# emonosuke/emoASR

Hardware: AMD Instinct MI355X
Metric: train frames/sec + decode RTF, Conformer-CTC 23M, 80-mel, 1/2/4/8 GPU (higher is better)
Workload: dtype bf16; 1 GPU; CTC(Conformer) 23M `L2`, bf16, SpecAugment on-GPU, synthetic LibriSpeech-shaped batches (2000 utts, lognormal lengths, ASRBatchSampler packing 30000 frames/50 utts per GPU), one step = accum_grad 5 micro-batches (the reference's accum_grad: 5, asr/train_asr.py:106-128, stacked through the engine in one pass) fwd+bwd, then all-reduce+clip+Adam; dropout 0.1; accum_grad=5, stacked_micro_batches=True, parallelism=dp1

## Files before the change

emoasr_amd/csrc/convfused.hip:

```cpp
#include <algorithm>
#include "common.h"
#include "../../include/emoasr_hip.h"

namespace {

constexpr int CF_TT = 32;
constexpr int CF_MAXK = 31;
constexpr int CF_CB = 256;
constexpr int CF_ROWS_P = 64;

typedef __attribute__((ext_vector_type(2))) float f2;
__device__ __forceinline__ f2 unpack2(unsigned u) { return f2{__uint_as_float(u << 16), __uint_as_float(u & 0xffff0000u)}; }
__device__ __forceinline__ unsigned pack2(f2 v) {
  const bf16 lo = (bf16)v[0], hi = (bf16)v[1];
  return (unsigned)__builtin_bit_cast(unsigned short, lo) | ((unsigned)__builtin_bit_cast(unsigned short, hi) << 16);
}
__device__ __forceinline__ unsigned lds_pair(const bf16* base, int row, int pair) {
  return *reinterpret_cast<const unsigned*>(base + row * CF_CB + 2 * pair);
}

__device__ __forceinline__ int ring_row(int u) { return (u & (CF_ROWS_P - 1)) * CF_CB; }

template <bool GLU>
__global__ __launch_bounds__(CF_CB) void cf_dwconv_kernel(int Tn, int C, int K, const bf16* __restrict__ x,
// ... 354 lines not shown
}

extern "C" int emoasr_conv_bwd_fused(int dtype, int B, int Tn, int C, int K, const void* ds, const void* cv,
                                     const float* mean, const float* var, const float* gamma, const float* beta, float eps,
                                     const float* tot, const void* g, const float* w, void* dg, float* dw, float* dbias,
                                     float* scratch, void* stream) {
  EMO_CHECK(dtype == EMO_BF16, "conv_bwd_fused: bf16 only");
  EMO_CHECK(K <= CF_MAXK && (K & 1) && C % 8 == 0, "conv_bwd_fused: K=%d (odd, <= %d), C=%d (multiple of 8)", K, CF_MAXK, C);
  EMO_CHECK((long)Tn * 2 * C * 2 < (1L << 32), "conv_bwd_fused: utterance larger than 4 GiB");
  EMO_CHECK(scratch != nullptr && tot != nullptr, "conv_bwd_fused: scratch and tot are required");
  if (B * Tn == 0) return 0;
  hipStream_t s = (hipStream_t)stream;
  if (bwd_lds_attr()) return 1;
  const int S = strip_tiles(1, &B, &Tn, cdiv(C, CF_CB));
  dim3 grid(cdiv(cdiv(Tn, CF_TT), S), cdiv(C, CF_CB), B);
  cf_conv_bwd_kernel<<<grid, CF_CB, CF_BWD_LDS, s>>>(Tn, C, K, (const bf16*)ds, (const bf16*)cv, mean, var, gamma, beta, eps, tot,
                                                   (const bf16*)g, w, (bf16*)dg, scratch, S, 1, RowSegs{});
  EMO_LAUNCH_CHECK();
  return emo_dwconv_bwd_w_reduce(cdiv(Tn, CF_TT) * B, C, K, scratch, dw, dbias, s);
}

int emo_bn_stats_finalize_seg(const RowSegs& sg, int C, float* part, float* mean, float* var, float* running_mean,
                              float* running_var, float momentum, long long* nbt, hipStream_t s);
int emo_bn_swish_fwd_seg(const RowSegs& sg, int C, const void* y, const float* mean, const float* var, const float* gamma,
                         const float* beta, float eps, void* z, hipStream_t s);
int emo_bn_swish_bwd_sums_seg(const RowSegs& sg, int C, const void* dz, const void* y, const float* mean, const float* var,
                              const float* gamma, const float* beta, float eps, float* dgamma, float* dbeta, float* scratch,
                              float** tot_out, hipStream_t s);

namespace {
bool row_segs(const emoasr_segments_t* seg, int C, RowSegs* out, int* tmax) {
  if (!seg || seg->n < 1 || seg->n > EMOASR_MAX_SEGMENTS) return false;
  RowSegs sg{};
  sg.n = seg->n;
  *tmax = 0;
  for (int i = 0; i < seg->n; ++i) {
    if (seg->B[i] <= 0 || seg->T[i] <= 0) return false;
    sg.b0[i + 1] = sg.b0[i] + seg->B[i];
    sg.T[i] = seg->T[i];
    sg.row[i + 1] = sg.row[i] + (long)seg->B[i] * seg->T[i];
    sg.part[i + 1] = sg.part[i] + emoasr_dwconv_stats_floats(seg->B[i], seg->T[i], C);
    sg.sums[i + 1] = sg.sums[i] + (emoasr_bn_swish_bwd_scratch_floats(seg->B[i] * seg->T[i], C) / (2 * C) - 1);
    *tmax = std::max(*tmax, seg->T[i]);
  }
  *out = sg;
  return true;
}
}

extern "C" int emoasr_conv_module_fwd_seg(int dtype, const emoasr_segments_t* seg, int C, int K, const void* g, const float* w,
                                          const float* bias, void* c, float* part, float* bmean, float* bvar, float* running_mean,
                                          float* running_var, float momentum, long long* num_batches_tracked, const float* gamma,
                                          const float* beta, float eps, void* z, int training, void* stream) {
  EMO_CHECK(dtype == EMO_BF16, "conv_module_fwd_seg: bf16 only");
  EMO_CHECK(K <= CF_MAXK && (K & 1) && C % 8 == 0, "conv_module_fwd_seg: K=%d (odd, <= %d), C=%d (multiple of 8)", K, CF_MAXK, C);
  RowSegs sg;
  int tmax = 0;
  EMO_CHECK(row_segs(seg, C, &sg, &tmax), "conv_module_fwd_seg: bad segment description");
  EMO_CHECK((long)tmax * 2 * C * 2 < (1L << 32) && sg.row[sg.n] * 2 * C * 2 < (1L << 46), "conv_module_fwd_seg: batch too large");
  EMO_CHECK(!training || (part && bmean && bvar), "conv_module_fwd_seg: training needs the BatchNorm buffers");
  hipStream_t s = (hipStream_t)stream;
  EmoTimerScope timer_(EMO_TIMER_CONV_MODULE, s, 0.0, 5.0 * (double)sg.row[sg.n] * C * 2.0);
  const int S = strip_tiles(seg->n, seg->B, seg->T, cdiv(C, CF_CB));
  dim3 grid(cdiv(cdiv(tmax, CF_TT), S), cdiv(C, CF_CB), sg.b0[sg.n]);
  cf_dwconv_kernel<true><<<grid, CF_CB, 0, s>>>(tmax, C, K, (const bf16*)g, w, bias, (bf16*)c, 0, training ? part : nullptr, S, sg);
  EMO_LAUNCH_CHECK();
  if (training) {
    if (emo_bn_stats_finalize_seg(sg, C, part, bmean, bvar, running_mean, running_var, momentum, num_batches_tracked, s)) return 1;
    return emo_bn_swish_fwd_seg(sg, C, c, bmean, bvar, gamma, beta, eps, z, s);
  }
  RowSegs one{};
  one.n = 1; one.b0[1] = sg.b0[sg.n]; one.row[1] = sg.row[sg.n];
  return emo_bn_swish_fwd_seg(one, C, c, running_mean, running_var, gamma, beta, eps, z, s);
}

extern "C" long emoasr_conv_module_bwd_seg_scratch_floats(const emoasr_segments_t* seg, int C, int K, int which) {
  RowSegs sg;
  int tmax = 0;
  if (!row_segs(seg, C, &sg, &tmax)) return 0;
  if (which == 0) return (sg.sums[sg.n] + 2 * sg.n) * 2 * C;
  return emoasr_dwconv_bwd_w_scratch_floats(sg.b0[sg.n], tmax, C, K);
}

extern "C" int emoasr_conv_module_bwd_seg(int dtype, const emoasr_segments_t* seg, int C, int K, const void* dz, const void* c,
                                          const float* bmean, const float* bvar, const float* gamma, const float* beta, float eps,
                                          float* dgamma, float* dbeta, const void* g, const float* w, void* dg, float* dw,
                                          float* dbias, float* bn_scratch, float* dw_scratch, void* stream) {
  EMO_CHECK(dtype == EMO_BF16, "conv_module_bwd_seg: bf16 only");
  EMO_CHECK(K <= CF_MAXK && (K & 1) && C % 8 == 0, "conv_module_bwd_seg: K=%d (odd, <= %d), C=%d (multiple of 8)", K, CF_MAXK, C);
  EMO_CHECK(bn_scratch && dw_scratch, "conv_module_bwd_seg: scratch required");
  RowSegs sg;
  int tmax = 0;
  EMO_CHECK(row_segs(seg, C, &sg, &tmax), "conv_module_bwd_seg: bad segment description");
  hipStream_t s = (hipStream_t)stream;
  EmoTimerScope timer_(EMO_TIMER_CONV_MODULE, s, 0.0, 8.0 * (double)sg.row[sg.n] * C * 2.0);
  float* tot = nullptr;
  if (emo_bn_swish_bwd_sums_seg(sg, C, dz, c, bmean, bvar, gamma, beta, eps, dgamma, dbeta, bn_scratch, &tot, s)) return 1;
  if (bwd_lds_attr()) return 1;
  const int S = strip_tiles(seg->n, seg->B, seg->T, cdiv(C, CF_CB));
  dim3 grid(cdiv(cdiv(tmax, CF_TT), S), cdiv(C, CF_CB), sg.b0[sg.n]);
  cf_conv_bwd_kernel<<<grid, CF_CB, CF_BWD_LDS, s>>>(tmax, C, K, (const bf16*)dz, (const bf16*)c, bmean, bvar, gamma, beta, eps, tot,
                                                   (const bf16*)g, w, (bf16*)dg, dw_scratch, S, 0, sg);
  EMO_LAUNCH_CHECK();
  return emo_dwconv_bwd_w_reduce((int)live_strips(seg->n, seg->B, seg->T, S), C, K, dw_scratch, dw, dbias, s);
}
```

emoasr_amd/csrc/convmodule.hip:

```cpp
#include <algorithm>
#include "common.h"
#include "../../include/emoasr_hip.h"

namespace {

constexpr int DW_TT = 32;
constexpr int DW_MAXK = 31;
constexpr int DW_WCHUNKS = 1;

template <typename T>
__global__ __launch_bounds__(256) void dwconv_kernel(int Tn, int C, int K, const T* __restrict__ x,
                                                     const float* __restrict__ w,
                                                     const float* __restrict__ bias, T* __restrict__ y,
                                                     int flip, float* __restrict__ part, const RowSegs sg) {
  const int c = blockIdx.y * 256 + threadIdx.x;
  if (c >= C) return;
  int b = blockIdx.z;
  if (sg.n > 1) {
    const int si = rowsegs_of_utt(sg, b);
    Tn = sg.T[si];
    x += sg.row[si] * C; y += sg.row[si] * C;
    if (part) part += sg.part[si];
    b -= sg.b0[si];
    if ((int)blockIdx.x * DW_TT >= Tn) return;
// ... 122 lines not shown
    tickets[blockIdx.x] = 0u;
    if (num_batches_tracked && blockIdx.x == 0) *num_batches_tracked += ns;
  }
}

template <typename T>
__global__ __launch_bounds__(256) void dwconv_bwd_w_kernel(int Tn, int C, int K, const T* __restrict__ dy,
                                                           const T* __restrict__ x, float* __restrict__ part, const RowSegs sg) {
  const int c = blockIdx.y * 256 + threadIdx.x;
  if (c >= C) return;
  int b = blockIdx.z;
  const int pad = (K - 1) / 2;
  if (sg.n > 1) {
    const int si = rowsegs_of_utt(sg, b);
    Tn = sg.T[si];
    x += sg.row[si] * C; dy += sg.row[si] * C;
    b -= sg.b0[si];
  }
  float acc[DW_MAXK];
#pragma unroll
  for (int j = 0; j < DW_MAXK; ++j) acc[j] = 0.f;
  float sb = 0.f;
  const __amdgpu_buffer_rsrc_t rsx = make_rsrc(x + (long)b * Tn * C), rsd = make_rsrc(dy + (long)b * Tn * C);
  for (int cc = 0; cc < DW_WCHUNKS; ++cc) {
    const int t0 = (blockIdx.x * DW_WCHUNKS + cc) * DW_TT;
    if (t0 >= Tn) break;
    float win[DW_TT + DW_MAXK - 1];
#pragma unroll
    for (int i = 0; i < DW_TT + DW_MAXK - 1; ++i) {
      const int t = t0 + i - pad;
      const bool ok = i < DW_TT + K - 1 && t >= 0 && t < Tn;
      win[i] = buf_load_f32<T>(rsx, ok ? (unsigned)(((long)t * C + c) * sizeof(T)) : EMO_OOB);
    }
    float dv[DW_TT];
#pragma unroll
    for (int i = 0; i < DW_TT; ++i)
      dv[i] = buf_load_f32<T>(rsd, t0 + i < Tn ? (unsigned)(((long)(t0 + i) * C + c) * sizeof(T)) : EMO_OOB);
#pragma unroll
    for (int i = 0; i < DW_TT; ++i) {
      const float d = dv[i];
      sb += d;
#pragma unroll
      for (int j = 0; j < DW_MAXK; ++j) acc[j] = emo_mac(d, win[i + j], acc[j]);
    }
  }
  const long blk = ((long)blockIdx.z * gridDim.x + blockIdx.x);
  float* p = part + blk * (K + 1) * C + c;
#pragma unroll
  for (int j = 0; j < DW_MAXK; ++j)
    if (j < K) p[(long)j * C] = acc[j];
  p[(long)K * C] = sb;
}

__global__ __launch_bounds__(256) void dwconv_bwd_w_reduce_kernel(int nblk, int C, int K,
                                                                  const float* __restrict__ part,
                                                                  float* __restrict__ dw,
                                                                  float* __restrict__ dbias) {
  __shared__ float red[4][64];
  const int lane = threadIdx.x & 63, wave = threadIdx.x >> 6;
  const int i = blockIdx.x * 64 + lane;
  const int n = (K + 1) * C;
  const int per = (nblk + gridDim.y - 1) / gridDim.y;
  const int b0 = blockIdx.y * per, b1 = min(nblk, b0 + per);
  float s = 0.f;
  if (i < n) {
#pragma unroll 8
    for (int b = b0 + wave; b < b1; b += 4) s += part[(long)b * n + i];
  }
  red[wave][lane] = s;
  __syncthreads();
  if (wave == 0 && i < n) {
    s = red[0][lane] + red[1][lane] + red[2][lane] + red[3][lane];
    const int j = i / C, c = i % C;
    if (gridDim.y == 1) {
      if (j < K) dw[c * K + j] += s;
      else if (dbias) dbias[c] += s;
    } else {
      if (j < K) atomicAdd(&dw[c * K + j], s);
      else if (dbias) atomicAdd(&dbias[c], s);
    }
  }
}

constexpr int BN_ROWS = 16;
constexpr int BN_STAT_ROWS = 64;
template <typename T>
__global__ __launch_bounds__(256) void bn_sum_kernel(int M, int C, const T* __restrict__ y,
                                                     float* __restrict__ sum) {
  const int c = blockIdx.x * 256 + threadIdx.x;
  if (c >= C) return;
  const int r0 = blockIdx.y * BN_STAT_ROWS, r1 = min(M, r0 + BN_STAT_ROWS);
  float s = 0.f;
  for (int r = r0; r < r1; ++r) s += to_f32(y[(long)r * C + c]);
  atomicAdd(&sum[c], s);
}
template <typename T>
__global__ __launch_bounds__(256) void bn_var_kernel(int M, int C, const T* __restrict__ y,
                                                     const float* __restrict__ sum,
                                                     float* __restrict__ sq) {
  const int c = blockIdx.x * 256 + threadIdx.x;
  if (c >= C) return;
  const float mu = sum[c] / M;
  const int r0 = blockIdx.y * BN_STAT_ROWS, r1 = min(M, r0 + BN_STAT_ROWS);
  float s = 0.f;
  for (int r = r0; r < r1; ++r) { const float d = to_f32(y[(long)r * C + c]) - mu; s += d * d; }
  atomicAdd(&sq[c], s);
}
__global__ void bn_finalize_kernel(int M, int C, float* mean, float* var, float* running_mean,
                                   float* running_var, float momentum) {
  const int c = blockIdx.x * 256 + threadIdx.x;
  if (c >= C) return;
  const float mu = mean[c] / M, vb = var[c] / M;
  mean[c] = mu; var[c] = vb;
  if (running_mean) running_mean[c] = (1.f - momentum) * running_mean[c] + momentum * mu;
  if (running_var) {
    const float vu = M > 1 ? var[c] * M / (M - 1) : vb;
    running_var[c] = (1.f - momentum) * running_var[c] + momentum * vu;
  }
}

template <typename T>
__global__ __launch_bounds__(256) void bn_swish_fwd_kernel(long n, int C, const T* __restrict__ y,
                                                           const float* __restrict__ mean,
                                                           const float* __restrict__ var,
                                                           const float* __restrict__ gamma,
                                                           const float* __restrict__ beta, float eps,
                                                           T* __restrict__ z, const RowSegs sg) {
  for (long i = (long)blockIdx.x * 256 + threadIdx.x; i < n; i += (long)gridDim.x * 256) {
    const int c = i % C;
    const long so = sg.n > 1 ? (long)rowsegs_of_row(sg, i / C) * C : 0;
    const float xh = (to_f32(y[i]) - mean[so + c]) * rsqrtf(var[so + c] + eps);
    z[i] = from_f32<T>(swish_t<T>(gamma[c] * xh + beta[c]));
  }
}
template <typename T>
__global__ __launch_bounds__(256) void bn_swish_fwd8_kernel(long n8, int C, const T* __restrict__ y,
                                                            const float* __restrict__ mean,
                                                            const float* __restrict__ var,
                                                            const float* __restrict__ gamma,
                                                            const float* __restrict__ beta, float eps,
                                                            T* __restrict__ z, const RowSegs sg) {
  const int cg = C / 8;
  for (long i = (long)blockIdx.x * 256 + threadIdx.x; i < n8; i += (long)gridDim.x * 256) {
    const long row = i / cg;
    const int c = (int)(i - row * cg) * 8;
    const long so = sg.n > 1 ? (long)rowsegs_of_row(sg, row) * C : 0;
    float v[8];
    load8<T>(y + i * 8, v);
#pragma unroll
    for (int j = 0; j < 8; ++j) {
      const float xh = (v[j] - mean[so + c + j]) * rsqrtf(var[so + c + j] + eps);
      v[j] = swish_t<T>(gamma[c + j] * xh + beta[c + j]);
    }
    store8<T>(z + i * 8, v);
  }
}

constexpr int BN_SUM_ROWS = 64;
constexpr int BN_APPLY_ROWS = 16;

template <typename T>
__global__ __launch_bounds__(256) void bn_bwd_sums_kernel(int M, int C, const T* __restrict__ dz,
                                                          const T* __restrict__ y,
                                                          const float* __restrict__ mean,
                                                          const float* __restrict__ var,
                                                          const float* __restrict__ gamma,
// ... 83 lines not shown
      raw[C + c] = b;
    }
  }
  if (ns == 1 || (!dbeta && !dgamma)) return;
  __syncthreads();
  if (threadIdx.x == 0) {
    __threadfence();
    s_last = atomicAdd(&tickets[64 + blockIdx.x], 1u) == (unsigned)ns - 1;
  }
  __syncthreads();
  if (!s_last) return;
  __threadfence();
  if (grp == 0 && c < C) {
    float da = 0.f, db = 0.f;
    const float* r0 = tot_ + (long)ns * 2 * C;
    for (int k = 0; k < ns; ++k) {
      da += __hip_atomic_load(r0 + (long)k * 2 * C + c, __ATOMIC_RELAXED, __HIP_MEMORY_SCOPE_AGENT);
      db += __hip_atomic_load(r0 + (long)k * 2 * C + C + c, __ATOMIC_RELAXED, __HIP_MEMORY_SCOPE_AGENT);
    }
    if (dbeta) dbeta[c] += da;
    if (dgamma) dgamma[c] += db;
  }
  if (threadIdx.x == 0) tickets[64 + blockIdx.x] = 0u;
}
template <typename T>
__global__ __launch_bounds__(256) void bn_bwd_apply_kernel(int M, int C, const T* __restrict__ dz,
                                                           const T* __restrict__ y,
                                                           const float* __restrict__ mean,
                                                           const float* __restrict__ var,
                                                           const float* __restrict__ gamma,
                                                           const float* __restrict__ beta, float eps,
                                                           const float* __restrict__ tot,
                                                           T* __restrict__ dy, const RowSegs sg) {
  const int hl = threadIdx.x & 31, rl = threadIdx.x >> 5;
  const int c = blockIdx.x * 256 + hl * 8;
  if (c >= C) return;
  if (sg.n > 1) {
    const int si = blockIdx.z;
    M = (int)(sg.row[si + 1] - sg.row[si]);
    if ((int)blockIdx.y * BN_APPLY_ROWS >= M) return;
    dz += sg.row[si] * C; y += sg.row[si] * C; dy += sg.row[si] * C;
    mean += (long)si * C; var += (long)si * C; tot += (long)si * 2 * C;
  }
  float mu[8], is[8], g[8], bt[8], m1[8], m2[8];
#pragma unroll
  for (int j = 0; j < 8; ++j) {
    mu[j] = mean[c + j]; is[j] = rsqrtf(var[c + j] + eps); g[j] = gamma[c + j]; bt[j] = beta[c + j];
    m1[j] = tot[c + j]; m2[j] = tot[C + c + j];
  }
  const __amdgpu_buffer_rsrc_t rsy = make_rsrc(y), rsd = make_rsrc(dz);
  const int r0 = blockIdx.y * BN_APPLY_ROWS;
#pragma unroll
  for (int it = 0; it < BN_APPLY_ROWS / 8; ++it) {
    const int r = r0 + rl + 8 * it;
    const bool ok = r < M;
    float yv[8], dv[8], o[8];
    buf_load8<T>(rsy, (long)r * C + c, ok, yv);
    buf_load8<T>(rsd, (long)r * C + c, ok, dv);
#pragma unroll
    for (int j = 0; j < 8; ++j) {
      const float xh = (yv[j] - mu[j]) * is[j];
      const float dbn = dv[j] * dswish_t<T>(g[j] * xh + bt[j]);
      o[j] = g[j] * is[j] * (dbn - m1[j] - xh * m2[j]);
    }
    if (ok) store8<T>(dy + (long)r * C + c, o);
  }
}

inline int ew_grid(long n) { long b = (n + 255) / 256; return (int)(b > 8192 ? 8192 : (b < 1 ? 1 : b)); }

}

int emo_dwconv_lds(int B, int Tn, int C, int K, const void* x, const float* w, const float* bias, void* y, int flip,
                   float* part, hipStream_t s);
static bool use_lds(int dtype, int Tn, int C) {
  return g_opt.dwconv_lds && dtype == EMO_BF16 && C % 8 == 0 && (long)Tn * C * 2 < (1L << 32);
}
int emo_dwconv_bwd_w_reduce(int nblk, int C, int K, const float* part, float* dw, float* dbias, hipStream_t s) {
  dwconv_bwd_w_reduce_kernel<<<dim3(cdiv((K + 1) * C, 64), nblk >= 1024 ? 4 : 1), 256, 0, s>>>(nblk, C, K, part, dw, dbias);
  EMO_LAUNCH_CHECK();
  return 0;
}

extern "C" int emoasr_dwconv_fwd(int dtype, int B, int Tn, int C, int K, const void* x, const float* w,
                                 const float* bias, void* y, void* stream) {
  EMO_CHECK(K <= DW_MAXK && (K & 1), "dwconv: K=%d unsupported (odd, <= %d)", K, DW_MAXK);
  if (B * Tn == 0) return 0;
  if (use_lds(dtype, Tn, C)) return emo_dwconv_lds(B, Tn, C, K, x, w, bias, y, 0, nullptr, (hipStream_t)stream);
  dim3 grid(cdiv(Tn, DW_TT), cdiv(C, 256), B);
  EMO_DISPATCH(dtype, (dwconv_kernel<T><<<grid, 256, 0, (hipStream_t)stream>>>(Tn, C, K, (const T*)x, w,
                                                                              bias, (T*)y, 0, nullptr, RowSegs{})));
  EMO_LAUNCH_CHECK();
  return 0;
}

extern "C" long emoasr_dwconv_stats_floats(int B, int Tn, int C) { return (long)B * cdiv(Tn, DW_TT) * 2 * C; }

extern "C" int emoasr_dwconv_fwd_stats(int dtype, int B, int Tn, int C, int K, const void* x, const float* w,
                                       const float* bias, void* y, float* part, void* stream) {
  EMO_CHECK(K <= DW_MAXK && (K & 1), "dwconv: K=%d unsupported", K);
  EMO_CHECK(part != nullptr && B * Tn > 0, "dwconv_fwd_stats: needs a non-empty batch and the partials buffer");
  if (use_lds(dtype, Tn, C)) return emo_dwconv_lds(B, Tn, C, K, x, w, bias, y, 0, part, (hipStream_t)stream);
  dim3 grid(cdiv(Tn, DW_TT), cdiv(C, 256), B);
  EMO_DISPATCH(dtype, (dwconv_kernel<T><<<grid, 256, 0, (hipStream_t)stream>>>(Tn, C, K, (const T*)x, w,
                                                                              bias, (T*)y, 0, part, RowSegs{})));
  EMO_LAUNCH_CHECK();
  return 0;
}

extern "C" int emoasr_bn_stats_finalize(int B, int Tn, int C, const float* part, float* mean, float* var,
                                        float* running_mean, float* running_var, float momentum,
                                        long long* num_batches_tracked, void* stream) {
  EMO_CHECK(B * Tn > 0, "bn_stats_finalize: empty batch");
  EMO_CHECK(cdiv(C, BNF_CH) <= 64, "bn_stats_finalize: C=%d too wide for the ticket table", C);
  EMO_BN_TICKETS(stream);
  bn_stats_finalize_kernel<<<cdiv(C, BNF_CH), 1024, 0, (hipStream_t)stream>>>(B, Tn, C, const_cast<float*>(part), mean, var, running_mean,
                                                                          running_var, momentum, num_batches_tracked, RowSegs{}, tickets_);
  EMO_LAUNCH_CHECK();
  return 0;
}
extern "C" int emoasr_dwconv_bwd_x(int dtype, int B, int Tn, int C, int K, const void* dy, const float* w,
                                   void* dx, void* stream) {
  EMO_CHECK(K <= DW_MAXK && (K & 1), "dwconv: K=%d unsupported", K);
  if (B * Tn == 0) return 0;
  if (use_lds(dtype, Tn, C)) return emo_dwconv_lds(B, Tn, C, K, dy, w, nullptr, dx, 1, nullptr, (hipStream_t)stream);
  dim3 grid(cdiv(Tn, DW_TT), cdiv(C, 256), B);
  EMO_DISPATCH(dtype, (dwconv_kernel<T><<<grid, 256, 0, (hipStream_t)stream>>>(Tn, C, K, (const T*)dy, w,
                                                                              nullptr, (T*)dx, 1, nullptr, RowSegs{})));
  EMO_LAUNCH_CHECK();
  return 0;
}
extern "C" long emoasr_dwconv_bwd_w_scratch_floats(int B, int Tn, int C, int K) {
  return (long)B * cdiv(Tn, DW_TT * DW_WCHUNKS) * (K + 1) * C;
}

extern "C" int emoasr_dwconv_bwd_w(int dtype, int B, int Tn, int C, int K, const void* dy, const void* x,
                                   float* dw, float* dbias, int accumulate, float* scratch, void* stream) {
  EMO_CHECK(K <= DW_MAXK && (K & 1), "dwconv: K=%d unsupported", K);
  hipStream_t s = (hipStream_t)stream;
  if (!accumulate) {
    hipMemsetAsync(dw, 0, sizeof(float) * C * K, s);
    if (dbias) hipMemsetAsync(dbias, 0, sizeof(float) * C, s);
  }
  if (B * Tn == 0) return 0;
  EMO_CHECK(scratch != nullptr, "dwconv_bwd_w: scratch of emoasr_dwconv_bwd_w_scratch_floats() floats required");
  dim3 grid(cdiv(Tn, DW_TT * DW_WCHUNKS), cdiv(C, 256), B);
  EMO_DISPATCH(dtype, (dwconv_bwd_w_kernel<T><<<grid, 256, 0, s>>>(Tn, C, K, (const T*)dy, (const T*)x, scratch, RowSegs{})));
  const int nblk = grid.x * B;
  dwconv_bwd_w_reduce_kernel<<<cdiv((K + 1) * C, 64), 256, 0, s>>>(nblk, C, K, scratch, dw, dbias);
  EMO_LAUNCH_CHECK();
  return 0;
}

extern "C" int emoasr_bn_stats(int dtype, int M, int C, const void* y, float* mean, float* var,
                               float* running_mean, float* running_var, float momentum, void* stream) {
  EMO_CHECK(M > 0, "bn_stats: empty batch");
  hipStream_t s = (hipStream_t)stream;
  hipMemsetAsync(mean, 0, sizeof(float) * C, s);
  hipMemsetAsync(var, 0, sizeof(float) * C, s);
  dim3 grid(cdiv(C, 256), cdiv(M, BN_STAT_ROWS));
  EMO_DISPATCH(dtype, (bn_sum_kernel<T><<<grid, 256, 0, s>>>(M, C, (const T*)y, mean)));
  EMO_DISPATCH(dtype, (bn_var_kernel<T><<<grid, 256, 0, s>>>(M, C, (const T*)y, mean, var)));
  bn_finalize_kernel<<<cdiv(C, 256), 256, 0, s>>>(M, C, mean, var, running_mean, running_var, momentum);
  EMO_LAUNCH_CHECK();
  return 0;
}
// ... 152 lines not shown
```

emoasr_amd/csrc/gemm.hip:

```cpp
#include <algorithm>
#include <type_traits>
#include <vector>
#include "mma.h"
#include "../../include/emoasr_hip.h"
#include "gemm_big_tn.h"

namespace {

struct ConvGeom {
  int T1, F1, T2, F2, C;
};
__device__ __forceinline__ long conv_row_base(const ConvGeom& g, int m) {
  const int per_b = g.T2 * g.F2;
  const int b = m / per_b, r = m - b * per_b;
  const int t2 = r / g.F2, f2 = r - t2 * g.F2;
  return (((long)b * g.T1 + 2 * t2) * g.F1 + 2 * f2) * g.C;
}
__device__ __forceinline__ int conv_k_off(const ConvGeom& g, int k) {
  const int p = k / g.C, c = k - p * g.C;
  const int kh = p / 3, kw = p - kh * 3;
  return (kh * g.F1 + kw) * g.C + c;
}

struct DgradGeom {
// ... 606 lines not shown
      }
    } else {
#pragma unroll
    for (int kk = 0; kk < BK; kk += M_::KSTEP) {
      typename M_::Frag af[TM], bfr[TN];
#pragma unroll
      for (int i = 0; i < TM; ++i) af[i] = M_::template load_km<TR>(As[buf], LDA, kk, w1 + i * 32, lane);
#pragma unroll
      for (int j = 0; j < TN; ++j) bfr[j] = M_::template load_km<TR>(Bs[buf], LDB, kk, w2 + j * 32, lane);
#pragma unroll
      for (int i = 0; i < TM; ++i)
#pragma unroll
        for (int j = 0; j < TN; ++j) acc[i][j] = M_::mma(af[i], bfr[j], acc[i][j]);
    }
    }
    store_tile(nxt, buf ^ 1);
    __syncthreads();
  };
  for (int kt = kt_begin; kt < kt_end; kt += 3) {
    step(kt, s1, s2);
    if (kt + 1 < kt_end) step(kt + 1, s2, s0);
    if (kt + 2 < kt_end) step(kt + 2, s0, s1);
  }

#pragma unroll
  for (int i = 0; i < TM; ++i)
#pragma unroll
    for (int j = 0; j < TN; ++j) {
      const int col = n2_0 + w2 + j * 32 + c_col(lane);
      if (col >= g.N2) continue;
#pragma unroll
      for (int r = 0; r < 16; ++r) {
        const int row = n1_0 + w1 + i * 32 + c_row(r, lane);
        if (row >= g.N1) continue;
        atomicAdd(&g.C[(long)row * g.ldc + col], g.alpha * acc[i][j][r]);
      }
    }
  if (do_colsum && n1_0 + tid < g.N1) atomicAdd(&g.colsum[n1_0 + tid], g.colsum_scale * csum);
}

template <typename T, int BN1, int BN2, int BMODE, bool TR, int KB, bool SP = false>
__global__ __launch_bounds__(256) void gemm_tn_kernel(const TnArgs g) {
  const int gx = gridDim.x, gy = gridDim.y;
  const int lin = xcd_remap((blockIdx.z * gy + blockIdx.y) * gx + blockIdx.x, gx * gy * gridDim.z);
  tn_block<T, BN1, BN2, BMODE, TR, KB, SP>(g, lin % gx, (lin / gx) % gy, lin / (gx * gy), gx);
}

constexpr int TN_PLACE_MAX = 24;
struct TnPlace {
  unsigned short start[8][TN_PLACE_MAX + 1];
  unsigned char prob[8][TN_PLACE_MAX], split[8][TN_PLACE_MAX];
  unsigned char cnt[8];
};
struct TnGroup {
  int n;
  int xcd;
  int start[EMOASR_TN_GROUP_MAX + 1];
  TnArgs p[EMOASR_TN_GROUP_MAX];
  TnPlace place;
};
template <typename T, bool TR, int KB, int BT, bool SP = false>
__global__ __launch_bounds__(256) void gemm_tn_grouped_kernel(const TnGroup G) {
  if (G.xcd == 1) {
    const int x = blockIdx.x & 7, slot = blockIdx.x >> 3, cnt = G.place.cnt[x];
    if (slot >= G.place.start[x][cnt]) return;
    int e = 0;
    while (e + 1 < cnt && slot >= G.place.start[x][e + 1]) ++e;
    const TnArgs& g = G.p[G.place.prob[x][e]];
    const int local = slot - G.place.start[x][e];
    const int tx = (g.N2 + BT - 1) / BT;
    tn_block<T, BT, BT, 0, TR, KB, SP>(g, local % tx, local / tx, G.place.split[x][e], tx);
    return;
  }
  const int bid = G.xcd ? xcd_remap(blockIdx.x, gridDim.x) : (int)blockIdx.x;
  int p = 0;
  while (p + 1 < G.n && bid >= G.start[p + 1]) ++p;
  const TnArgs& g = G.p[p];
  const int local = bid - G.start[p];
  const int tx = (g.N2 + BT - 1) / BT, ty = (g.N1 + BT - 1) / BT;
  tn_block<T, BT, BT, 0, TR, KB, SP>(g, local % tx, (local / tx) % ty, local / (tx * ty), tx);
}

template <typename T, int AMODE, bool BKM, bool TR, bool SP = false>
int launch_nt_(const NtArgs& a_in, hipStream_t s, int nz = 1) {
  NtArgs a = a_in;
  a.xcd = g_opt.gemm_xcd;
  if constexpr (SP) {
    const long t12864 = (long)cdiv(a.M, 128) * cdiv(a.N, 64) * nz, t128 = (long)cdiv(a.M, 128) * cdiv(a.N, 128) * nz;
    (void)t12864;
    int tile = (t128 >= g_opt.split_min128 && a.N % 128 == 0) ? 1 : 3;
    if (g_opt.split_tile == 1 && a.N % 128 == 0) tile = 1;
    else if (g_opt.split_tile >= 2) tile = g_opt.split_tile;
    const int kb = (g_opt.split_kb == 2 && a.K >= 512) ? 2 : 1;
#define EMO_SP_LAUNCH(BM_, BN_)                                                            \
  do {                                                                                     \
    dim3 grid(cdiv(a.N, BN_), cdiv(a.M, BM_), nz);                                         \
    if (kb == 2) gemm_nt_kernel<T, BM_, BN_, AMODE, BKM, TR, 2, true><<<grid, 256, 0, s>>>(a); \
    else gemm_nt_kernel<T, BM_, BN_, AMODE, BKM, TR, 1, true><<<grid, 256, 0, s>>>(a);      \
  } while (0)
    if (tile == 1) EMO_SP_LAUNCH(128, 128);
    else if (tile == 2) EMO_SP_LAUNCH(128, 64);
    else EMO_SP_LAUNCH(64, 64);
#undef EMO_SP_LAUNCH
    EMO_LAUNCH_CHECK();
    return 0;
  }
  const long t12864 = (long)cdiv(a.M, 128) * cdiv(a.N, 64) * nz;
  const bool stacked64 = AMODE == 0 && a.M >= 16384 && !(a.N >= (g_opt.gemm_wide128 ? 512 : 768));
  const int tile = g_opt.gemm_tile ? g_opt.gemm_tile : (stacked64 ? 3 : (t12864 >= 384 ? 2 : 3));
  const int kb = sizeof(T) == 2 ? (g_opt.gemm_kb ? g_opt.gemm_kb : (a.K >= 512 ? 2 : 1)) : 1;
#define EMO_NT_LAUNCH(BM_, BN_)                                                           \
  do {                                                                                    \
    dim3 grid(cdiv(a.N, BN_), cdiv(a.M, BM_), nz);                                        \
    if constexpr (sizeof(T) == 2) {                                                       \
      if (kb == 2) gemm_nt_kernel<T, BM_, BN_, AMODE, BKM, TR, 2><<<grid, 256, 0, s>>>(a); \
      else gemm_nt_kernel<T, BM_, BN_, AMODE, BKM, TR, 1><<<grid, 256, 0, s>>>(a);         \
    } else {                                                                              \
      gemm_nt_kernel<T, BM_, BN_, AMODE, BKM, TR, 1><<<grid, 256, 0, s>>>(a);              \
    }                                                                                     \
  } while (0)
  if constexpr (sizeof(T) == 2 && AMODE == 0 && !BKM) {
    if (g_opt.gemm_wholek && a.M <= 2048 && a.K % 256 == 0 && nz == 1) {
      dim3 grid(cdiv(a.N, 64), cdiv(a.M, 64), 1);
      gemm_nt_kernel<T, 64, 64, AMODE, BKM, TR, 8><<<grid, 256, 0, s>>>(a);
      EMO_LAUNCH_CHECK();
      return 0;
    }
  }
  if (tile == 1) EMO_NT_LAUNCH(128, 128);
  else if (tile == 2) EMO_NT_LAUNCH(128, 64);
  else EMO_NT_LAUNCH(64, 64);
#undef EMO_NT_LAUNCH
  EMO_LAUNCH_CHECK();
  return 0;
}
template <typename T> constexpr bool is_f32 = sizeof(T) == 4;
template <typename T, int AMODE>
int launch_nt(const NtArgs& a, hipStream_t s) {
  if constexpr (is_f32<T>) { if (t_f32_split) return launch_nt_<T, AMODE, false, true, true>(a, s); }
  return launch_nt_<T, AMODE, false, true>(a, s);
}
template <typename T>
int launch_nn(const NtArgs& a, hipStream_t s, int nz = 1) {
  if constexpr (is_f32<T>) { if (t_f32_split) return launch_nt_<T, 0, true, true, true>(a, s, nz); }
  return g_opt.tr_read ? launch_nt_<T, 0, true, true>(a, s, nz) : launch_nt_<T, 0, true, false>(a, s, nz);
}

inline int tn_split_cap(long N1, long N2, long K) {
  const long out_bytes = N1 * N2 * 4;
  const double est_s = 2.0 * (double)N1 * (double)N2 * (double)K / 300e12;
  const long cap_work = (long)(0.25 * est_s * 1.3e12 / (double)out_bytes);
  return (int)std::max(std::max(1L, (8L << 20) / out_bytes), cap_work);
}

template <typename T, int BMODE, bool SP = false>
int launch_tn(TnArgs a, hipStream_t s) {
  if constexpr (is_f32<T> && !SP) { if (t_f32_split) return launch_tn<T, BMODE, true>(a, s); }
  const bool big = (long)cdiv(a.N1, 128) * cdiv(a.N2, 128) >= 32 && a.N1 >= 128 && a.N2 >= 128;
  const int kb = sizeof(T) == 2 ? (g_opt.gemm_kb ? g_opt.gemm_kb : (a.K >= 512 && !big ? 2 : 1)) : 1;
  const int BK = (SP ? 32 : TileCfg<T>::BK) * kb;
  const int nk = cdiv(a.K, BK);
  const int bn = big ? 128 : 64;
  const long tiles = (long)cdiv(a.N1, bn) * cdiv(a.N2, bn);
  const long slots_ = g_opt.tn_group_blocks > 0 ? g_opt.tn_group_blocks : ((big && kb == 2) || (big && SP) ? 512 : 768);
  int splits = (int)std::max(1L, slots_ / tiles);
  const int cap = tn_split_cap(a.N1, a.N2, a.K);
  const int floor_splits = (int)std::min((long)splits, (128 + tiles - 1) / tiles);
  splits = std::max(floor_splits, std::min(splits, cap));
  splits = std::max(1, std::min(splits, nk / 4 > 0 ? nk / 4 : 1));
  a.k_tiles_per_split = cdiv(nk, splits);
  splits = cdiv(nk, a.k_tiles_per_split);
  dim3 grid(cdiv(a.N2, bn), cdiv(a.N1, bn), splits);
#define EMO_TN_LAUNCH(BN_, TR_)                                                     \
  do {                                                                              \
    if constexpr (sizeof(T) == 2) {                                                 \
      if (kb == 2) gemm_tn_kernel<T, BN_, BN_, BMODE, TR_, 2><<<grid, 256, 0, s>>>(a); \
      else gemm_tn_kernel<T, BN_, BN_, BMODE, TR_, 1><<<grid, 256, 0, s>>>(a);         \
    } else {                                                                        \
      gemm_tn_kernel<T, BN_, BN_, BMODE, TR_, 1, SP><<<grid, 256, 0, s>>>(a);          \
    }                                                                               \
  } while (0)
  if constexpr (SP) {
    if (big) EMO_TN_LAUNCH(128, true);
    else EMO_TN_LAUNCH(64, true);
  } else {
  if (big) {
    if (g_opt.tr_read) EMO_TN_LAUNCH(128, true);
    else EMO_TN_LAUNCH(128, false);
  } else {
    if (g_opt.tr_read) EMO_TN_LAUNCH(64, true);
    else EMO_TN_LAUNCH(64, false);
  }
  }
#undef EMO_TN_LAUNCH
  EMO_LAUNCH_CHECK();
  return 0;
}

}

bool emo_gemm_nt_big_wants(int M, int N, int K, long lda, long ldb, long ldc, const emoasr_epilogue_t& ep);
int emo_gemm_nt_big_ep(int M, int N, int K, const void* A, long lda, const void* B, long ldb, void* C, long ldc,
                       const emoasr_epilogue_t& ep, hipStream_t s);
int emo_conv2_fwd_big(int B, int T1, int F1, int C, const void* y1, const void* w, void* y2, const float* bias,
                      int relu, hipStream_t s);


static int check_vec(long ld, int dtype, const char* what) {
  const int vec = dtype == EMO_BF16 ? 8 : 4;
  if (ld % vec != 0) { emo_set_error("gemm: %s=%ld must be a multiple of %d elements", what, ld, vec); return 1; }
  return 0;
}

extern "C" int emoasr_gemm_nt(int dtype, int M, int N, int K, const void* A, long lda, const void* B,
                              long ldb, void* C, long ldc, const emoasr_epilogue_t* ep, void* stream) {
  SplitScope split_scope(dtype);
  EMO_CHECK(M > 0 && N > 0 && K > 0, "gemm_nt: empty problem %d %d %d", M, N, K);
  if (check_vec(lda, dtype, "lda") || check_vec(ldb, dtype, "ldb") || check_vec(K, dtype, "K")) return 1;
  NtArgs a{};
  a.M = M; a.N = N; a.K = K; a.A = A; a.lda = lda; a.B = B; a.ldb = ldb; a.C = C; a.ldc = ldc;
  if (ep) a.ep = *ep; else { a.ep = emoasr_epilogue_t{}; a.ep.alpha = 1.f; }
  const double esz_ = dtype == EMO_BF16 ? 2.0 : 4.0;
  EmoTimerScope timer_(EMO_TIMER_GEMM_NT_NN, (hipStream_t)stream, 2.0 * M * N * K,
                       ((double)M * K + (double)N * K + (double)M * N * (1 + (a.ep.residual ? 1 : 0) + (a.ep.pre_out ? 1 : 0))) * esz_);
  if (dtype == EMO_BF16 && emo_gemm_nt_big_wants(M, N, K, lda, ldb, ldc, a.ep))
    return emo_gemm_nt_big_ep(M, N, K, A, lda, B, ldb, C, ldc, a.ep, (hipStream_t)stream);
  EMO_DISPATCH(dtype, return (launch_nt<T, 0>(a, (hipStream_t)stream)));
}

extern "C" int emoasr_gemm_nn(int dtype, int M, int N, int K, const void* A, long lda, const void* B,
                              long ldb, void* C, long ldc, const emoasr_epilogue_t* ep, void* stream) {
  SplitScope split_scope(dtype);
  EMO_CHECK(M > 0 && N > 0 && K > 0, "gemm_nn: empty problem %d %d %d", M, N, K);
  if (check_vec(lda, dtype, "lda") || check_vec(ldb, dtype, "ldb") || check_vec(K, dtype, "K") ||
      check_vec(N, dtype, "N")) return 1;
  NtArgs a{};
  a.M = M; a.N = N; a.K = K; a.A = A; a.lda = lda; a.B = B; a.ldb = ldb; a.C = C; a.ldc = ldc;
  if (ep) a.ep = *ep; else { a.ep = emoasr_epilogue_t{}; a.ep.alpha = 1.f; }
  const double esz_ = dtype == EMO_BF16 ? 2.0 : 4.0;
  EmoTimerScope timer_(EMO_TIMER_GEMM_NT_NN, (hipStream_t)stream, 2.0 * M * N * K,
                       ((double)M * K + (double)N * K + (double)M * N * (1 + (a.ep.residual ? 1 : 0) + (a.ep.dact_pre ? 1 : 0))) * esz_);
  EMO_DISPATCH(dtype, return (launch_nn<T>(a, (hipStream_t)stream)));
  return 0;
}

extern "C" int emoasr_gemm_nn_batched(int dtype, int M, int N, int K, const void* A, long lda, long sa_b,
                                      long sa_h, const void* B, long ldb, long sb_b, long sb_h, void* C,
                                      long ldc, long sc_b, long sc_h, int nb, int nh, float alpha,
                                      int accumulate, void* stream) {
  SplitScope split_scope(dtype);
  EMO_CHECK(M > 0 && N > 0 && K > 0 && nb > 0 && nh > 0, "gemm_nn_batched: empty problem");
  if (check_vec(lda, dtype, "lda") || check_vec(ldb, dtype, "ldb") ||
      check_vec(N, dtype, "N") || check_vec(sa_b, dtype, "sa_b") || check_vec(sa_h, dtype, "sa_h") ||
      check_vec(sb_b, dtype, "sb_b") || check_vec(sb_h, dtype, "sb_h")) return 1;
  NtArgs a{};
  a.M = M; a.N = N; a.K = K; a.A = A; a.lda = lda; a.B = B; a.ldb = ldb; a.C = C; a.ldc = ldc;
  a.ep = emoasr_epilogue_t{}; a.ep.alpha = alpha;
  if (accumulate) { a.ep.residual = C; a.ep.ldr = (int)ldc; a.ep.res_scale = 1.f; }
  a.nh = nh; a.sa_b = sa_b; a.sa_h = sa_h; a.sb_b = sb_b; a.sb_h = sb_h; a.sc_b = sc_b; a.sc_h = sc_h;
  EMO_DISPATCH(dtype, return (launch_nn<T>(a, (hipStream_t)stream, nb * nh)));
  return 0;
}

static bool tn_big_takes(int dtype, int N1, int N2, int K, long lda, long ldb);
static void tn_big_splits(int n, const BigTnProblem* q, int* splits);

extern "C" int emoasr_gemm_tn(int dtype, int N1, int N2, int K, const void* A, long lda, const void* B,
                              long ldb, float* C, long ldc, float alpha, int accumulate, float* colsum,
                              float colsum_scale, void* stream) {
  SplitScope split_scope(dtype);
  EMO_CHECK(N1 > 0 && N2 > 0 && K > 0, "gemm_tn: empty problem");
  if (check_vec(lda, dtype, "lda") || check_vec(ldb, dtype, "ldb") || check_vec(N2, dtype, "N2")) return 1;
  EMO_CHECK(N1 % (dtype == EMO_BF16 ? 8 : 4) == 0 || lda >= (N1 + 7) / 8 * 8, "gemm_tn: ragged N1 needs padded lda");
  if (!accumulate) {
    if (ldc == N2) hipMemsetAsync(C, 0, sizeof(float) * (size_t)N1 * N2, (hipStream_t)stream);
    else hipMemset2DAsync(C, sizeof(float) * ldc, 0, sizeof(float) * N2, N1, (hipStream_t)stream);
    if (colsum) hipMemsetAsync(colsum, 0, sizeof(float) * N1, (hipStream_t)stream);
  }
  TnArgs a{};
  a.N1 = N1; a.N2 = N2; a.K = K; a.A = A; a.lda = lda; a.B = B; a.ldb = ldb; a.C = C; a.ldc = ldc;
  a.alpha = alpha; a.colsum = colsum; a.colsum_scale = colsum_scale;
  EmoTimerScope timer_(EMO_TIMER_GEMM_TN, (hipStream_t)stream, 2.0 * N1 * N2 * K,
                       ((double)K * N1 + (double)K * N2) * (dtype == EMO_BF16 ? 2.0 : 4.0) + 4.0 * N1 * N2);
  if (tn_big_takes(dtype, N1, N2, K, lda, ldb)) {
    const BigTnProblem q{N1, N2, K, A, lda, B, ldb, C, ldc, alpha, 0, colsum, colsum_scale};
    int splits = 1;
    tn_big_splits(1, &q, &splits);
    return emo_tn_big_launch(1, &q, &splits, (hipStream_t)stream);
  }
  EMO_DISPATCH(dtype, return (launch_tn<T, 0>(a, (hipStream_t)stream)));
}

static int tn_group_plan(int dtype, int n, const emoasr_tn_problem_t* probs, TnGroup& G, int& bt, int& kb) {
  EMO_CHECK(n > 0 && n <= EMOASR_TN_GROUP_MAX, "gemm_tn_grouped: n=%d outside 1..%d", n, EMOASR_TN_GROUP_MAX);
  G.n = n;
  long tiles = 0;
  bt = 128;
  for (int i = 0; i < n; ++i)
    if (probs[i].N1 < 128 || probs[i].N2 < 128) bt = 64;
  if (g_opt.gemm_tile == 3) bt = 64;
  kb = dtype == EMO_BF16 ? (g_opt.tn_group_kb ? g_opt.tn_group_kb : g_opt.gemm_kb ? g_opt.gemm_kb : (bt == 128 ? 1 : 2)) : 1;
  const bool split = dtype == EMO_F32X3;
  const int BK = (dtype == EMO_BF16 || split ? 32 : 16) * kb;
  for (int i = 0; i < n; ++i) {
    const emoasr_tn_problem_t& q = probs[i];
    EMO_CHECK(q.N1 > 0 && q.N2 > 0 && q.K > 0, "gemm_tn_grouped: empty problem %d", i);
    if (check_vec(q.lda, dtype, "lda") || check_vec(q.ldb, dtype, "ldb") || check_vec(q.N2, dtype, "N2")) return 1;
    EMO_CHECK(q.N1 % (dtype == EMO_BF16 ? 8 : 4) == 0 || q.lda >= (q.N1 + 7) / 8 * 8,
              "gemm_tn_grouped: ragged N1 needs padded lda");
    tiles += (long)cdiv(q.N1, bt) * cdiv(q.N2, bt);
  }
  const long slots = g_opt.tn_group_blocks > 0 ? g_opt.tn_group_blocks : ((bt == 128 && kb == 2) || (bt == 128 && split) ? 512 : 768);
// ... 223 lines not shown
```

emoasr_amd/csrc/layer.hip:

```cpp
#include <math.h>
#include <algorithm>
#include <map>
#include <mutex>
#include <utility>
#include "common.h"
#include "../../include/emoasr_hip.h"

void emo_attn_bwd_fused_extras(float* zero, long zn, const float* cast_src, void* cast_dst, long cn);
void emo_attn_bwd_defer_join(int v);
void emo_attn_bwd_join(void* stream);
int emo_attn_bwd_prelaunch(int dtype, const emoasr_attn_t* a, void* ws, size_t ws_bytes, float* zero, long zn, void* stream);

int emo_bn_stats_finalize_seg(const RowSegs& sg, int C, float* part, float* mean, float* var, float* running_mean,
                              float* running_var, float momentum, long long* nbt, hipStream_t s);
int emo_bn_swish_fwd_seg_dt(int dtype, const RowSegs& sg, int C, const void* y, const float* mean, const float* var,
                            const float* gamma, const float* beta, float eps, void* z, hipStream_t s);
int emo_bn_swish_bwd_sums_seg_dt(int dtype, const RowSegs& sg, int C, const void* dz, const void* y, const float* mean, const float* var,
                                 const float* gamma, const float* beta, float eps, float* dgamma, float* dbeta, float* scratch,
                                 float** tot_out, hipStream_t s);
int emo_bn_bwd_apply_seg(int dtype, const RowSegs& sg, int C, const void* dz, const void* y, const float* mean, const float* var,
                         const float* gamma, const float* beta, float eps, const float* tot, void* dy, hipStream_t s);
int emo_dwconv_seg(int dtype, const RowSegs& sg, int tmax, int C, int K, const void* x, const float* w, const float* bias, void* y,
                   int flip, float* part, hipStream_t s);
int emo_dwconv_bwd_w_seg(int dtype, const RowSegs& sg, int tmax, int C, int K, const void* dy, const void* x, float* dw, float* dbias,
                         float* scratch, hipStream_t s);

namespace {

emoasr_epilogue_t plain_ep() {
  emoasr_epilogue_t e{};
  e.alpha = 1.f;
  e.res_scale = 1.f;
  return e;
}

bool conv_fused_ok(int dtype, int d) { return g_opt.conv_fused && dtype == EMO_BF16 && d % 8 == 0; }

struct WgSide {
  hipStream_t side = nullptr;
  hipEvent_t fork = nullptr, done[2] = {nullptr, nullptr};
  bool pending[2] = {false, false};
  unsigned n = 0;
};
std::mutex g_wg_mu;
std::map<std::pair<int, hipStream_t>, WgSide> g_wg;

WgSide* wg_side_of(hipStream_t s, bool create) {
  hipStreamCaptureStatus cap = hipStreamCaptureStatusNone;
  if (hipStreamIsCapturing(s, &cap) != hipSuccess || cap != hipStreamCaptureStatusNone) return nullptr;
  int dev = 0;
  if (hipGetDevice(&dev) != hipSuccess) return nullptr;
  std::lock_guard<std::mutex> lk(g_wg_mu);
  auto it = g_wg.find({dev, s});
  if (it != g_wg.end()) return &it->second;
  if (!create) return nullptr;
  WgSide w;
  if (hipStreamCreateWithFlags(&w.side, hipStreamNonBlocking) != hipSuccess) return nullptr;
  if (hipEventCreateWithFlags(&w.fork, hipEventDisableTiming) != hipSuccess ||
      hipEventCreateWithFlags(&w.done[0], hipEventDisableTiming) != hipSuccess ||
      hipEventCreateWithFlags(&w.done[1], hipEventDisableTiming) != hipSuccess)
    return nullptr;
  return &(g_wg[{dev, s}] = w);
}

int ffn_fwd(int dtype, int M, int d, int F, const emoasr_ffn_params_t& p, const void* x, float res_scale,
            float p_enc, uint64_t s_in, uint64_t s_out, const emoasr_ffn_stash_t& st, void* stream) {
  if (emoasr_layernorm_fwd(dtype, M, d, x, p.ln_g, p.ln_b, 1e-5f, st.h, st.mean, st.rstd, stream)) return 1;
  emoasr_epilogue_t e1 = plain_ep();
  e1.bias = p.b1; e1.act = EMOASR_ACT_SWISH | (g_opt.ffn_save_dact ? EMOASR_ACT_SAVE_DACT : 0); e1.pre_out = st.u; e1.drop_p = p_enc; e1.seed = s_in;
  if (emoasr_gemm_nt(dtype, M, F, d, st.h, d, p.w1, d, st.a, F, &e1, stream)) return 1;
  emoasr_epilogue_t e2 = plain_ep();
  e2.bias = p.b2; e2.residual = x; e2.ldr = d; e2.res_scale = res_scale; e2.drop_p = p_enc; e2.seed = s_out;
  return emoasr_gemm_nt(dtype, M, d, F, st.a, F, p.w2, F, st.y, d, &e2, stream);
}

struct SegView {
  int n = 0, Btot = 0;
  int B[EMOASR_MAX_SEGMENTS], T[EMOASR_MAX_SEGMENTS], b0[EMOASR_MAX_SEGMENTS];
  long row[EMOASR_MAX_SEGMENTS + 1], prow[EMOASR_MAX_SEGMENTS + 1], part[EMOASR_MAX_SEGMENTS + 1];
  long M() const { return row[n]; }
  long R() const { return prow[n]; }
};

bool seg_view(const emoasr_conformer_fwd_t* io, int d, SegView* v) {
  const emoasr_segments_t& s = io->seg;
  if (s.n < 0 || s.n > EMOASR_MAX_SEGMENTS) return false;
  v->n = s.n > 0 ? s.n : 1;
  v->row[0] = v->prow[0] = v->part[0] = 0;
  v->Btot = 0;
  for (int i = 0; i < v->n; ++i) {
    v->B[i] = s.n > 0 ? s.B[i] : io->B;
    v->T[i] = s.n > 0 ? s.T[i] : io->T;
    if (v->B[i] <= 0 || v->T[i] <= 0) return false;
    v->b0[i] = v->Btot;
    v->Btot += v->B[i];
    v->row[i + 1] = v->row[i] + (long)v->B[i] * v->T[i];
    v->prow[i + 1] = v->prow[i] + 2L * v->T[i] - 1;
    v->part[i + 1] = v->part[i] + emoasr_dwconv_stats_floats(v->B[i], v->T[i], d);
  }
  return true;
}

RowSegs row_segs_of(const SegView& sv, int C) {
  RowSegs sg{};
  sg.n = sv.n;
  for (int i = 0; i < sv.n; ++i) {
    sg.b0[i + 1] = sg.b0[i] + sv.B[i];
    sg.T[i] = sv.T[i];
// ... 13 lines not shown
  a.B = nb; a.H = H; a.DK = d / H; a.Tq = tmax; a.Tk = tmax;
  a.ldq = a.ldk = a.ldv = 3 * d; a.ldo = d; a.ldp = d;
  a.q = base; a.k = base + (size_t)d * esz; a.v = base + (size_t)2 * d * esz;
  a.pos = (const char*)pp + (size_t)sv.prow[s0] * d * esz;
  a.klens = klens ? klens + sv.b0[s0] : nullptr;
  a.causal = 0; a.scale = 1.f / sqrtf((float)(d / H));
  a.seed = seed + 0x9E3779B97F4A7C15ull * (uint64_t)s0;
  a.nseg = 0;
  if (s1 - s0 > 1) {
    a.nseg = s1 - s0;
    for (int k = s0; k <= s1; ++k) {
      a.seg_b0[k - s0] = k < s1 ? sv.b0[k] - sv.b0[s0] : nb;
      a.seg_row[k - s0] = sv.row[k] - sv.row[s0];
      a.seg_prow[k - s0] = sv.prow[k] - sv.prow[s0];
      if (k < s1) a.seg_T[k - s0] = sv.T[k];
    }
  }
}

}

extern "C" int emoasr_wgrad_side_join(int keep, void* stream) {
  hipStream_t s = (hipStream_t)stream;
  WgSide* w = wg_side_of(s, false);
  if (!w) return 0;
  for (int back = 2; back > (keep > 0 ? 1 : 0); --back) {
    if (w->n < (unsigned)back) continue;
    const int slot = (w->n - back) & 1;
    if (!w->pending[slot]) continue;
    if (hipStreamWaitEvent(s, w->done[slot], 0) != hipSuccess) { emo_set_error("wgrad_side_join: hipStreamWaitEvent failed"); return 1; }
    w->pending[slot] = false;
  }
  return 0;
}

extern "C" int emoasr_conformer_attn_masks(int dtype, int nl, const emoasr_segments_t* seg, int B, int T, int H, int d, const int* klens,
                                           float p_att, const uint64_t* seeds, unsigned* masks, long layer_stride_words, int nw,
                                           void* stream) {
  EMO_CHECK(seg && seeds && masks && nl >= 0 && H > 0 && d % H == 0, "conformer_attn_masks: bad arguments");
  if (p_att <= 0.f) return 0;
  emoasr_conformer_fwd_t io{};
  io.B = B; io.T = T; io.seg = *seg;
  SegView sv;
  EMO_CHECK(seg_view(&io, d, &sv), "conformer_attn_masks: bad batch / segment shapes");
  const size_t esz = dtype == EMO_BF16 ? 2 : 4;
  const int astep = g_opt.stack_launch ? sv.n : 1;
  for (int l = 0; l < nl; ++l)
    for (int si = 0; si < sv.n; si += astep) {
      emoasr_attn_t am{};
      attn_args_for(am, sv, si, si + astep, H, d, esz, nullptr, nullptr, klens, seeds[l]);
      am.drop_p = p_att;
      if (emoasr_attn_dropmask(dtype, &am, masks + (size_t)l * layer_stride_words + (size_t)sv.row[si] * H * nw, nw, stream)) return 1;
    }
  return 0;
}

extern "C" int emoasr_conformer_layer_fwd(int dtype, const emoasr_conformer_layer_t* L,
                                          const emoasr_conformer_fwd_t* io, void* stream) {
  EMO_CHECK(L && io && io->x && io->pos_t, "conformer_layer_fwd: missing arguments");
  const int d = L->d, H = L->H, F = L->F;
  EMO_CHECK(d > 0 && H > 0 && d % H == 0, "conformer_layer_fwd: bad dims d=%d H=%d", d, H);
  SegView sv;
  EMO_CHECK(seg_view(io, d, &sv), "conformer_layer_fwd: bad batch / segment shapes (B=%d T=%d segments=%d)", io->B, io->T, io->seg.n);
  const int M = (int)sv.M(), R = (int)sv.R();
  const size_t esz = dtype == EMO_BF16 ? 2 : 4;
  const float p_enc = io->p_enc;
  const bool att_bits = g_opt.attn_mask_bits && io->att_mask && io->training && io->p_att > 0.f && dtype == EMO_BF16;
  const int astep_m = g_opt.stack_launch ? sv.n : 1;
  for (int si = 0; si < sv.n && att_bits && !io->att_mask_ready; si += astep_m) {
    emoasr_attn_t am{};
    attn_args_for(am, sv, si, si + astep_m, H, d, esz, io->qkv, io->pp, io->klens, io->seed[2]);
    am.drop_p = io->p_att;
    if (emoasr_attn_dropmask(dtype, &am, io->att_mask + (size_t)sv.row[si] * H * io->att_mask_nw, io->att_mask_nw, stream)) return 1;
  }
  if (ffn_fwd(dtype, M, d, F, L->ffm, io->x, 0.5f, p_enc, io->seed[0], io->seed[1], io->ffm, stream)) return 1;
  const void* x1 = io->ffm.y;
  if (emoasr_layernorm_fwd(dtype, M, d, x1, L->att_ln_g, L->att_ln_b, 1e-5f, io->at_h, io->at_mean, io->at_rstd, stream))
    return 1;
  {
    emoasr_epilogue_t e = plain_ep();
    e.bias = L->bqkv;
    if (emoasr_gemm_nt(dtype, M, 3 * d, d, io->at_h, d, L->wqkv, d, io->qkv, 3 * d, &e, stream)) return 1;
    emoasr_epilogue_t ep = plain_ep();
    if (emoasr_gemm_nt(dtype, R, d, d, io->pos_t, d, L->wpos, d, io->pp, d, &ep, stream)) return 1;
    const int astep = g_opt.stack_launch ? sv.n : 1;
    for (int si = 0; si < sv.n; si += astep) {
      const size_t ro = (size_t)sv.row[si];
      emoasr_attn_t a{};
      attn_args_for(a, sv, si, si + astep, H, d, esz, io->qkv, io->pp, io->klens, io->seed[2]);
      a.bias_u = L->bias_u; a.bias_v = L->bias_v; a.drop_p = io->p_att;
      a.out = (char*)io->o + ro * d * esz; a.lse = io->lse + ro * H;
      if (att_bits) { a.keep_mask = io->att_mask + ro * H * io->att_mask_nw; a.keep_nw = io->att_mask_nw; }
      if (emoasr_attn_fwd(dtype, &a, stream)) return 1;
    }
    emoasr_epilogue_t eo = plain_ep();
    eo.bias = L->bout; eo.residual = x1; eo.ldr = d; eo.drop_p = p_enc; eo.seed = io->seed[3];
    if (emoasr_gemm_nt(dtype, M, d, d, io->o, d, L->wout, d, io->at_y, d, &eo, stream)) return 1;
  }
  const void* x2 = io->at_y;
  if (emoasr_layernorm_fwd(dtype, M, d, x2, L->cv_ln_g, L->cv_ln_b, 1e-5f, io->cv_h, io->cv_mean, io->cv_rstd, stream))
    return 1;
  {
    emoasr_epilogue_t e = plain_ep();
    e.bias = L->pw1_b;
    if (emoasr_gemm_nt(dtype, M, 2 * d, d, io->cv_h, d, L->pw1, d, io->g, 2 * d, &e, stream)) return 1;
    const bool fused = conv_fused_ok(dtype, d);
    if (!fused && emoasr_glu_fwd(dtype, M, d, io->g, io->gl, stream)) return 1;
    if (io->training) EMO_CHECK(io->bn_part && io->bmean && io->bvar, "conformer_layer_fwd: training needs the BatchNorm buffers");
    const bool conv_one_launch = fused && sv.n > 1 && g_opt.stack_launch;
    if (conv_one_launch &&
        emoasr_conv_module_fwd_seg(dtype, &io->seg, d, L->K, io->g, L->dw_w, L->dw_b, io->c, io->bn_part, io->bmean, io->bvar,
                                   L->bn_rm, L->bn_rv, 0.1f, L->bn_nbt, L->bn_g, L->bn_b, 1e-5f, io->z, io->training, stream))
      return 1;
    const bool bn_one_launch = !fused && io->training && sv.n > 1 && g_opt.stack_launch;
    if (bn_one_launch) {
      const RowSegs sg = row_segs_of(sv, d);
      int tmax = 0;
      for (int si = 0; si < sv.n; ++si) tmax = std::max(tmax, sv.T[si]);
      if (emo_dwconv_seg(dtype, sg, tmax, d, L->K, io->gl, L->dw_w, L->dw_b, io->c, 0, io->bn_part, (hipStream_t)stream)) return 1;
      if (emo_bn_stats_finalize_seg(sg, d, io->bn_part, io->bmean, io->bvar, L->bn_rm, L->bn_rv, 0.1f, L->bn_nbt, (hipStream_t)stream))
        return 1;
      if (emo_bn_swish_fwd_seg_dt(dtype, sg, d, io->c, io->bmean, io->bvar, L->bn_g, L->bn_b, 1e-5f, io->z, (hipStream_t)stream)) return 1;
    }
    for (int si = 0; si < sv.n && !conv_one_launch && !bn_one_launch; ++si) {
      const size_t ro = (size_t)sv.row[si];
      const int B = sv.B[si], T = sv.T[si];
      const char* g = (const char*)io->g + ro * 2 * d * esz;
      const char* gl = io->gl ? (const char*)io->gl + ro * d * esz : nullptr;
      char* c = (char*)io->c + ro * d * esz;
      const float *bmean = L->bn_rm, *bvar = L->bn_rv;
      if (io->training) {
        float* part = io->bn_part + sv.part[si];
        if (fused) {
          if (emoasr_glu_dwconv_fwd(dtype, B, T, d, L->K, g, L->dw_w, L->dw_b, c, part, stream)) return 1;
        } else if (emoasr_dwconv_fwd_stats(dtype, B, T, d, L->K, gl, L->dw_w, L->dw_b, c, part, stream)) {
          return 1;
        }
        if (emoasr_bn_stats_finalize(B, T, d, part, io->bmean + (size_t)si * d, io->bvar + (size_t)si * d, L->bn_rm, L->bn_rv, 0.1f,
                                     L->bn_nbt, stream))
          return 1;
        bmean = io->bmean + (size_t)si * d; bvar = io->bvar + (size_t)si * d;
      } else if (fused) {
        if (emoasr_glu_dwconv_fwd(dtype, B, T, d, L->K, g, L->dw_w, L->dw_b, c, nullptr, stream)) return 1;
      } else if (emoasr_dwconv_fwd(dtype, B, T, d, L->K, gl, L->dw_w, L->dw_b, c, stream)) {
        return 1;
      }
      if (emoasr_bn_swish_fwd(dtype, B * T, d, c, bmean, bvar, L->bn_g, L->bn_b, 1e-5f, (char*)io->z + ro * d * esz, stream)) return 1;
    }
    emoasr_epilogue_t eo = plain_ep();
    eo.bias = L->pw2_b; eo.residual = x2; eo.ldr = d; eo.drop_p = p_enc; eo.seed = io->seed[4];
    if (emoasr_gemm_nt(dtype, M, d, d, io->z, d, L->pw2, d, io->cv_y, d, &eo, stream)) return 1;
  }
  if (ffn_fwd(dtype, M, d, F, L->ff, io->cv_y, 0.5f, p_enc, io->seed[5], io->seed[6], io->ff, stream)) return 1;
  return emoasr_layernorm_fwd(dtype, M, d, io->ff.y, L->fin_ln_g, L->fin_ln_b, 1e-5f, io->y, io->fin_mean, io->fin_rstd, stream);
}

namespace {

struct BwdLayout {
  size_t off = 0;
  size_t take(size_t bytes) { const size_t o = off; off += (bytes + 255) / 256 * 256; return o; }
};

struct BwdBufs {
  size_t dx1, dx2, dx3, dx4, pre1, pre2, pre3, pre4, dh, du_ff, du_ffm, dz, dc, dgl, dg, dout, dqkv, dpos_t;
  size_t dpos, delta, bn_scr, dw_scr, attn_ws, attn_ws_bytes, total;
  size_t img[EMOASR_MAX_SEGMENTS + 1];
};

BwdBufs bwd_layout(int dtype, const SegView& sv, int d, int H, int F, int K) {
  const size_t esz = dtype == EMO_BF16 ? 2 : 4, M = (size_t)sv.M(), R = (size_t)sv.R();
  BwdLayout L;
  BwdBufs b{};
  b.dx1 = L.take(M * d * esz); b.dx2 = L.take(M * d * esz); b.dx3 = L.take(M * d * esz); b.dx4 = L.take(M * d * esz);
  b.pre1 = L.take(M * d * esz); b.pre2 = L.take(M * d * esz); b.pre3 = L.take(M * d * esz); b.pre4 = L.take(M * d * esz);
  b.dh = L.take(M * d * esz);
  b.du_ff = L.take(M * F * esz); b.du_ffm = L.take(M * F * esz);
  b.dz = L.take(M * d * esz); b.dc = L.take(M * d * esz); b.dgl = L.take(M * d * esz); b.dg = L.take(M * 2 * d * esz);
  b.dout = L.take(M * d * esz); b.dqkv = L.take(M * 3 * d * esz); b.dpos_t = L.take(R * d * esz);
  b.dpos = L.take(R * d * 4); b.delta = L.take(M * H * 4);
  size_t bn_scr = 0, dw_scr = 0, attn_ws = 0;
  int tmax = 0;
  for (int i = 0; i < sv.n; ++i) {
    bn_scr = std::max(bn_scr, (size_t)emoasr_bn_swish_bwd_scratch_floats(sv.B[i] * sv.T[i], d) * 4);
    dw_scr = std::max(dw_scr, (size_t)emoasr_dwconv_bwd_w_scratch_floats(sv.B[i], sv.T[i], d, K) * 4);
    attn_ws = std::max(attn_ws, dtype == EMO_BF16 ? emoasr_attn_bwd_fused_ws_bytes(dtype, sv.B[i], H, sv.T[i], sv.T[i], 1)
                                                  : emoasr_attn_bwd_mat_bytes(dtype, sv.B[i], H, sv.T[i], sv.T[i], 1, 1));
    tmax = std::max(tmax, sv.T[i]);
    b.img[i + 1] = b.img[i] + (dtype == EMO_BF16 ? 0 : emoasr_attn_bwd_mat_bytes(dtype, sv.B[i], H, sv.T[i], sv.T[i], 1, 0));
  }
  if (dtype == EMO_BF16)
    attn_ws = std::max(attn_ws, emoasr_attn_bwd_fused_ws_bytes_rows(dtype, (long)M, H, tmax, 1));
  if (sv.n > 1) {
    emoasr_segments_t sg{};
    sg.n = sv.n;
    for (int i = 0; i < sv.n; ++i) { sg.B[i] = sv.B[i]; sg.T[i] = sv.T[i]; }
    bn_scr = std::max(bn_scr, (size_t)emoasr_conv_module_bwd_seg_scratch_floats(&sg, d, K, 0) * 4);
    dw_scr = std::max(dw_scr, (size_t)emoasr_conv_module_bwd_seg_scratch_floats(&sg, d, K, 1) * 4);
  }
  b.bn_scr = L.take(bn_scr);
  b.dw_scr = L.take(dw_scr);
  b.attn_ws_bytes = attn_ws;
  b.attn_ws = L.take(b.attn_ws_bytes);
  b.total = L.off;
  return b;
}

}

extern "C" size_t emoasr_conformer_layer_bwd_ws_bytes_seg(int dtype, const emoasr_segments_t* seg, int d, int H, int F, int K) {
  emoasr_conformer_fwd_t io{};
  if (!seg) return 0;
  io.seg = *seg;
  SegView sv;
  if (seg->n < 1 || !seg_view(&io, d, &sv)) return 0;
  return bwd_layout(dtype, sv, d, H, F, K).total;
}

extern "C" size_t emoasr_conformer_layer_bwd_img_bytes_seg(int dtype, const emoasr_segments_t* seg, int d, int H) {
  emoasr_conformer_fwd_t io{};
  if (!seg || dtype == EMO_BF16) return 0;
  io.seg = *seg;
  SegView sv;
  if (seg->n < 1 || !seg_view(&io, d, &sv)) return 0;
  return bwd_layout(dtype, sv, d, H, 4 * d, 1).img[sv.n];
}

extern "C" size_t emoasr_conformer_layer_bwd_ws_bytes(int dtype, int B, int T, int d, int H, int F, int K) {
  emoasr_segments_t seg{};
  seg.n = 1; seg.B[0] = B; seg.T[0] = T;
  return emoasr_conformer_layer_bwd_ws_bytes_seg(dtype, &seg, d, H, F, K);
}

extern "C" int emoasr_conformer_layer_bwd(int dtype, const emoasr_conformer_layer_t* L, const emoasr_conformer_layer_t* G,
                                          const emoasr_conformer_fwd_t* st, const emoasr_conformer_bwd_t* io, void* stream) {
  EMO_CHECK(L && G && st && io && io->dy && io->dx && io->ws && io->ln_part, "conformer_layer_bwd: missing arguments");
  const int d = L->d, H = L->H, F = L->F, K = L->K;
  SegView sv;
  EMO_CHECK(seg_view(st, d, &sv), "conformer_layer_bwd: bad batch / segment shapes");
  const int M = (int)sv.M(), R = (int)sv.R();
  const BwdBufs bb = bwd_layout(dtype, sv, d, H, F, K);
  EMO_CHECK(io->ws_bytes >= bb.total, "conformer_layer_bwd: workspace %zu < %zu bytes", io->ws_bytes, bb.total);
  char* ws = static_cast<char*>(io->ws);
  const size_t esz = dtype == EMO_BF16 ? 2 : 4;
  EMO_CHECK(dtype == EMO_BF16 || (io->attn_img && io->attn_img_bytes >= bb.img[sv.n]),
            "conformer_layer_bwd: f32 needs the zero-filled attention image area (%zu bytes, emoasr_conformer_layer_bwd_img_bytes_seg)",
            bb.img[sv.n]);
  const float p = st->p_enc;
  hipStream_t s = (hipStream_t)stream;
  emoasr_tn_problem_t pr[EMOASR_TN_GROUP_MAX];
  int npr = 0;
  WgSide* wgs = g_opt.wgrad_side ? wg_side_of(s, true) : nullptr;
  if (wgs && wgs->pending[wgs->n & 1]) {
    if (hipStreamWaitEvent(s, wgs->done[wgs->n & 1], 0) != hipSuccess) return 1;
    wgs->pending[wgs->n & 1] = false;
  }
  auto wgrad = [&](const void* dy, long lddy, int N1, const void* x, long ldx, int N2, int Kred, const void* gw, float alpha,
                   const void* gb) {
    pr[npr++] = emoasr_tn_problem_t{N1, N2, Kred, dy, lddy, x, ldx, (float*)gw, (long)N2, alpha, (float*)gb, alpha};
  };
  auto ln_bwd = [&](int slot, const void* dh, const void* x, const float* gamma, const float* mean, const float* rstd,
                    const void* dres, void* dx, const void* ggam, const void* gbet, void* pre, float scale, uint64_t seed) {
    emoasr_ln_bwd_opts_t o{};
    if (pre && p > 0.f) { o.dy2 = pre; o.scale2 = scale; o.drop_p2 = p; o.seed2 = seed; }
    o.defer_finalize = 1;
    return emoasr_layernorm_bwd_ex(dtype, M, d, dh, x, gamma, mean, rstd, dres, dx, (float*)ggam, (float*)gbet,
                                   io->ln_part + (long)slot * io->ln_part_stride, &o, stream);
  };
  auto dgrad = [&](int n_out, const void* dy_, const void* W, const void* Wt, void* dx_) {
    emoasr_epilogue_t e_ = plain_ep();
    if (Wt) return emoasr_gemm_nt(dtype, M, d, n_out, dy_, n_out, Wt, n_out, dx_, d, &e_, stream);
    return emoasr_gemm_nn(dtype, M, d, n_out, dy_, n_out, W, d, dx_, d, &e_, stream);
  };
  auto ffn_bwd = [&](const emoasr_ffn_params_t& P, const emoasr_ffn_params_t& Gp, const emoasr_ffn_stash_t& S, const void* x_in,
                     const void* dx_in, const void* pre_in, void* du, uint64_t s_in, const void* w1t, const void* w2t) {
    const void* dy = p > 0.f ? pre_in : dx_in;
    const float alpha = p > 0.f ? 1.f : 0.5f;
    wgrad(dy, d, d, S.a, F, F, M, Gp.w2, alpha, Gp.b2);
    emoasr_epilogue_t e = plain_ep();
    e.alpha = alpha; e.dact_pre = S.u; e.seed = s_in;
    if (g_opt.ffn_save_dact) { e.dact = EMOASR_DACT_MUL; e.drop_p = 0.f; }
    else { e.dact = EMOASR_ACT_SWISH; e.drop_p = p; }
    if (w2t ? emoasr_gemm_nt(dtype, M, F, d, dy, d, w2t, d, du, F, &e, stream)
            : emoasr_gemm_nn(dtype, M, F, d, dy, d, P.w2, F, du, F, &e, stream)) return 1;
    wgrad(du, F, F, S.h, d, d, M, Gp.w1, 1.f, Gp.b1);
    return dgrad(F, du, P.w1, w1t, ws + bb.dh);
  };

  if (g_opt.stack_launch && dtype == EMO_BF16) {
    emoasr_attn_t am{};
    attn_args_for(am, sv, 0, sv.n, H, d, esz, st->qkv, st->pp, st->klens, st->seed[2]);
    am.bias_u = L->bias_u; am.bias_v = L->bias_v; am.drop_p = st->p_att;
    if (g_opt.attn_mask_bits && st->att_mask && st->p_att > 0.f) { am.keep_mask = st->att_mask; am.keep_nw = st->att_mask_nw; }
    if (emo_attn_bwd_prelaunch(dtype, &am, ws + bb.attn_ws, bb.attn_ws_bytes, (float*)(ws + bb.dpos), (long)sv.R() * d, stream)) return 1;
  }
  if (ln_bwd(0, io->dy, st->ff.y, L->fin_ln_g, st->fin_mean, st->fin_rstd, nullptr, ws + bb.dx1, G->fin_ln_g, G->fin_ln_b,
             ws + bb.pre1, 0.5f, st->seed[6])) return 1;
  if (ffn_bwd(L->ff, G->ff, st->ff, st->cv_y, ws + bb.dx1, ws + bb.pre1, ws + bb.du_ff, st->seed[5], L->ff_w1t, L->ff_w2t)) return 1;
  if (ln_bwd(1, ws + bb.dh, st->cv_y, L->ff.ln_g, st->ff.mean, st->ff.rstd, ws + bb.dx1, ws + bb.dx2, G->ff.ln_g, G->ff.ln_b,
             ws + bb.pre2, 1.f, st->seed[4])) return 1;
  {
    const void* dy = p > 0.f ? ws + bb.pre2 : ws + bb.dx2;
    wgrad(dy, d, d, st->z, d, d, M, G->pw2, 1.f, G->pw2_b);
    emoasr_epilogue_t e = plain_ep();
    if (L->pw2_t ? emoasr_gemm_nt(dtype, M, d, d, dy, d, L->pw2_t, d, ws + bb.dz, d, &e, stream)
                 : emoasr_gemm_nn(dtype, M, d, d, dy, d, L->pw2, d, ws + bb.dz, d, &e, stream)) return 1;
    if (conv_fused_ok(dtype, d)) {
      const bool conv_one_launch = sv.n > 1 && g_opt.stack_launch;
      if (conv_one_launch &&
          emoasr_conv_module_bwd_seg(dtype, &st->seg, d, K, ws + bb.dz, st->c, st->bmean, st->bvar, L->bn_g, L->bn_b, 1e-5f,
                                     (float*)G->bn_g, (float*)G->bn_b, st->g, L->dw_w, ws + bb.dg, (float*)G->dw_w, (float*)G->dw_b,
                                     (float*)(ws + bb.bn_scr), (float*)(ws + bb.dw_scr), stream))
        return 1;
      for (int si = 0; si < sv.n && !conv_one_launch; ++si) {
        const size_t ro = (size_t)sv.row[si];
        const float *bmean = st->bmean + (size_t)si * d, *bvar = st->bvar + (size_t)si * d;
        const char* c = (const char*)st->c + ro * d * esz;
        float* tot = nullptr;
        if (emoasr_bn_swish_bwd_sums(dtype, sv.B[si] * sv.T[si], d, ws + bb.dz + ro * d * esz, c, bmean, bvar, L->bn_g, L->bn_b, 1e-5f,
                                     (float*)G->bn_g, (float*)G->bn_b, (float*)(ws + bb.bn_scr), &tot, stream)) return 1;
        if (emoasr_conv_bwd_fused(dtype, sv.B[si], sv.T[si], d, K, ws + bb.dz + ro * d * esz, c, bmean, bvar, L->bn_g, L->bn_b, 1e-5f,
                                  tot, (const char*)st->g + ro * 2 * d * esz, L->dw_w, ws + bb.dg + ro * 2 * d * esz, (float*)G->dw_w,
                                  (float*)G->dw_b, (float*)(ws + bb.dw_scr), stream)) return 1;
      }
    } else {
      const bool bn_one_launch = sv.n > 1 && g_opt.stack_launch;
      if (bn_one_launch) {
        const RowSegs sg = row_segs_of(sv, d);
        int tmax = 0;
        for (int si = 0; si < sv.n; ++si) tmax = std::max(tmax, sv.T[si]);
        float* tot = nullptr;
        if (emo_bn_swish_bwd_sums_seg_dt(dtype, sg, d, ws + bb.dz, st->c, st->bmean, st->bvar, L->bn_g, L->bn_b, 1e-5f, (float*)G->bn_g,
                                         (float*)G->bn_b, (float*)(ws + bb.bn_scr), &tot, s)) return 1;
        if (emo_bn_bwd_apply_seg(dtype, sg, d, ws + bb.dz, st->c, st->bmean, st->bvar, L->bn_g, L->bn_b, 1e-5f, tot, ws + bb.dc, s)) return 1;
        if (emo_dwconv_seg(dtype, sg, tmax, d, K, ws + bb.dc, L->dw_w, nullptr, ws + bb.dgl, 1, nullptr, s)) return 1;
        if (emo_dwconv_bwd_w_seg(dtype, sg, tmax, d, K, ws + bb.dc, st->gl, (float*)G->dw_w, (float*)G->dw_b, (float*)(ws + bb.dw_scr), s))
          return 1;
      }
      for (int si = 0; si < sv.n && !bn_one_launch; ++si) {
        const size_t ro = (size_t)sv.row[si];
        const int B = sv.B[si], T = sv.T[si];
        const float *bmean = st->bmean + (size_t)si * d, *bvar = st->bvar + (size_t)si * d;
        if (emoasr_bn_swish_bwd(dtype, B * T, d, ws + bb.dz + ro * d * esz, (const char*)st->c + ro * d * esz, bmean, bvar, L->bn_g,
                                L->bn_b, 1e-5f, ws + bb.dc + ro * d * esz, (float*)G->bn_g, (float*)G->bn_b,
                                (float*)(ws + bb.bn_scr), stream)) return 1;
        if (emoasr_dwconv_bwd_x(dtype, B, T, d, K, ws + bb.dc + ro * d * esz, L->dw_w, ws + bb.dgl + ro * d * esz, stream)) return 1;
        if (emoasr_dwconv_bwd_w(dtype, B, T, d, K, ws + bb.dc + ro * d * esz, (const char*)st->gl + ro * d * esz, (float*)G->dw_w,
                                (float*)G->dw_b, 1, (float*)(ws + bb.dw_scr), stream)) return 1;
      }
      if (emoasr_glu_bwd(dtype, M, d, st->g, ws + bb.dgl, ws + bb.dg, stream)) return 1;
    }
    wgrad(ws + bb.dg, 2 * d, 2 * d, st->cv_h, d, d, M, G->pw1, 1.f, G->pw1_b);
    if (dgrad(2 * d, ws + bb.dg, L->pw1, L->pw1_t, ws + bb.dh)) return 1;
    if (ln_bwd(2, ws + bb.dh, st->at_y, L->cv_ln_g, st->cv_mean, st->cv_rstd, ws + bb.dx2, ws + bb.dx3, G->cv_ln_g, G->cv_ln_b,
               ws + bb.pre3, 1.f, st->seed[3])) return 1;
  }
  {
    const void* dy = p > 0.f ? ws + bb.pre3 : ws + bb.dx3;
    wgrad(dy, d, d, st->o, d, d, M, G->wout, 1.f, G->bout);
    emoasr_epilogue_t e = plain_ep();
    if (L->wout_t ? emoasr_gemm_nt(dtype, M, d, d, dy, d, L->wout_t, d, ws + bb.dout, d, &e, stream)
                  : emoasr_gemm_nn(dtype, M, d, d, dy, d, L->wout, d, ws + bb.dout, d, &e, stream)) return 1;
    if (dtype != EMO_BF16) {
      if (hipMemsetAsync(ws + bb.dpos, 0, (size_t)R * d * 4, s) != hipSuccess) return 1;
      for (int si = 0; si < sv.n; ++si) {
        const size_t ro = (size_t)sv.row[si], po = (size_t)sv.prow[si];
        char* dqkv = ws + bb.dqkv + ro * 3 * d * esz;
        emoasr_attn_t a{};
        attn_args_for(a, sv, si, si + 1, H, d, esz, st->qkv, st->pp, st->klens, st->seed[2]);
        a.bias_u = L->bias_u; a.bias_v = L->bias_v; a.drop_p = st->p_att;
        a.out = (char*)st->o + ro * d * esz; a.lse = st->lse + ro * H;
        a.dout = ws + bb.dout + ro * d * esz; a.delta = (float*)(ws + bb.delta) + ro * H;
        a.dq = dqkv; a.dk = dqkv + (size_t)d * esz; a.dv = dqkv + (size_t)2 * d * esz;
        a.dpos = (float*)(ws + bb.dpos) + po * d; a.dbias_u = (float*)G->bias_u; a.dbias_v = (float*)G->bias_v;
        if (emoasr_attn_bwd_mat_bind(dtype, &a, (char*)io->attn_img + bb.img[si], ws + bb.attn_ws)) return 1;
        if (emoasr_attn_bwd(dtype, &a, stream)) return 1;
      }
    }
    const int astep = g_opt.stack_launch ? sv.n : 1;
    for (int si = 0; si < sv.n && dtype == EMO_BF16; si += astep) {
      const size_t ro = (size_t)sv.row[si], po = (size_t)sv.prow[si];
      const long Rs = sv.prow[si + astep] - sv.prow[si];
      char* dqkv = ws + bb.dqkv + ro * 3 * d * esz;
      emoasr_attn_t a{};
      attn_args_for(a, sv, si, si + astep, H, d, esz, st->qkv, st->pp, st->klens, st->seed[2]);
      a.bias_u = L->bias_u; a.bias_v = L->bias_v; a.drop_p = st->p_att;
      a.out = (char*)st->o + ro * d * esz; a.lse = st->lse + ro * H;
      if (g_opt.attn_mask_bits && st->att_mask && st->p_att > 0.f) { a.keep_mask = st->att_mask + ro * H * st->att_mask_nw; a.keep_nw = st->att_mask_nw; }
      a.dout = ws + bb.dout + ro * d * esz; a.delta = (float*)(ws + bb.delta) + ro * H;
      a.dq = dqkv; a.dk = dqkv + (size_t)d * esz; a.dv = dqkv + (size_t)2 * d * esz;
      float* dpos = (float*)(ws + bb.dpos) + po * d;
      a.dpos = dpos; a.dbias_u = (float*)G->bias_u; a.dbias_v = (float*)G->bias_v;
      emo_attn_bwd_fused_extras(dpos, Rs * d, dpos, ws + bb.dpos_t + po * d * esz, Rs * d);
      emo_attn_bwd_defer_join(astep == sv.n);
      if (emoasr_attn_bwd_fused(dtype, &a, ws + bb.attn_ws, bb.attn_ws_bytes, stream)) return 1;
// ... 24 lines not shown
```

emoasr_amd/engine/encoder.py:

```python
import math
import os

import torch

from .. import ops
from ..ops import ACT_RELU, ACT_SWISH
from .arena import AttnStash, ConvStash, FFNStash, LayerRecord, ParamArena, _Stash, _cfg, h2d_i32, h2d_pack, sinusoid
from .las import LASDecoder
from .rnn_encoder import RNNEncoder
from .rnnt import RNNTDecoder
from .transformer_decoder import TransformerDecoder


class CTCEngine(TransformerDecoder, RNNTDecoder, RNNEncoder, LASDecoder):

    def __init__(self, cfg, module, compute_dtype=torch.bfloat16, bn_buffers=None, f32_split=False, arena=None):
        self.cfg = cfg
        self.split = bool(f32_split) and compute_dtype == torch.float32
        self.d = cfg.enc_hidden_size
        self.h = _cfg(cfg, "enc_num_attention_heads", 0)
        self.nl = cfg.enc_num_layers
        self.conformer = cfg.encoder_type == "conformer"
        self.rnn_enc = cfg.encoder_type == "rnn"
        self.rel = _cfg(cfg, "pos_encode_type", "abs") == "rel"
        self.embed_in = _cfg(cfg, "input_layer", "conv2d") == "embed"
        inter_on = (_cfg(cfg, "mtl_inter_ctc_weight", 0) or 0) > 0 or (_cfg(cfg, "mtl_phone_ctc_weight", 0) or 0) > 0
        self.inter_layer = int(cfg.inter_ctc_layer_id) if inter_on else 0
        self.eouts_inter = None
        self._implicit_dgrad = os.environ.get("EMOASR_CONV2_DGRAD", "implicit") == "implicit"
        self._conv1_fold = os.environ.get("EMOASR_CONV1_FOLD", "1") != "0"
        from .. import lib as _lib
        self._conv_fused = _lib.get_option("conv_fused") != 0
        self._ffn_save_dact = _lib.get_option("ffn_save_dact") != 0
        self._conv_big = _lib.get_option("conv_big") != 0
        self.p_enc = float(_cfg(cfg, "dropout_enc_rate", 0.0))
        self.p_att = float(_cfg(cfg, "dropout_attn_rate", 0.0))
        self.dtype = compute_dtype
        self.module = module
        self._own_arena = arena is None
        self.arena = ParamArena(module, compute_dtype) if arena is None else arena
        self._tables = {}
        self._scratch_cache = {}
        self._group_wgrads = os.environ.get("EMOASR_WGRAD_GROUP", "1") != "0"
        self._defer_wgrads = False
        self._wq = []
        self._ln_deferred = []
        self.grad_hook = None
        self._layer_lo = None
        self._cpp_layers = os.environ.get("EMOASR_CPP_LAYER", "1") != "0"
        self._layer_rt = None
        self.mask_padding = False
        self._conv_lens = None
        self._side_wgrads = os.environ.get("EMOASR_WGRAD_SIDE", "0") != "0"
        self._side, self._inflight = None, []
        self.attn_store_scores = os.environ.get("EMOASR_ATTN_STORED", "0") == "1"
        self.attn_fused = os.environ.get("EMOASR_ATTN_FUSED", "1") != "0"
        self._bufs = {}
        self.f32_head = os.environ.get("EMOASR_F32_HEAD", "1") != "0"
        self.seed = 0x5EED
        if _cfg(cfg, "decoder_type", "ctc") == "transformer":
            self._dec_init()
        if _cfg(cfg, "decoder_type", "ctc") == "rnn_transducer":
            self._rnnt_init()
        if _cfg(cfg, "decoder_type", "ctc") == "las":
            self._las_init()
        self.step_count = 0

    def ensure_bound(self):
        if not self.arena.bound():
            assert self._own_arena, "emoasr_amd: the parameters left the shared arena; its owner re-binds them and rebuilds this engine"
            self.arena = ParamArena(self.module, self.dtype)
            self._layer_lo = None
            self._layer_rt = None
            self._bufs = {}
            self._scratch_cache = {}

    def _pos_table(self, T, device, max_len=5000):
        max_len = max(max_len, T)
        key = (self.rel, max_len, str(device))
        if key not in self._tables:
            if self.rel:
                tab = sinusoid(torch.arange(max_len - 1, -max_len, -1), self.d, device)
            else:
                tab = sinusoid(torch.arange(max_len), self.d, device)
            self._tables[key] = tab
        tab = self._tables[key]
        if self.rel:
            return tab[max_len - T: max_len - 1 + T]
        return tab[:T]

    def _seed(self, site):
        return (self.seed * 1000003 + self.step_count * 4099 + site) & 0xFFFFFFFFFFFF

    def _apply_mode(self):
        ops.split_products(self.split)

    def _scope(self):
        return ops.stream_scope(self.split)

    def _buffers(self, name):
        b = self._bufs.get(name)
        if b is None or not b.is_cuda:
            self._bufs = dict(self.module.named_buffers())
            b = self._bufs[name]
        return b

    def forward(self, xs, xlens_host, training, stash=None):
        with self._scope():
            if self.rnn_enc:
                return self._rnn_enc_forward(xs, xlens_host, training, stash)
            return self._forward(xs, xlens_host, training, stash)

    def _forward(self, xs, xlens_host, training, stash):
        self.ensure_bound()
        A, d, dt = self.arena, self.d, self.dtype
        A.refresh_shadow()
        stash = training if stash is None else stash
        self._keep = stash
        st = _Stash() if stash else None
        p_enc = self.p_enc if training else 0.0
        p_att = self.p_att if training else 0.0
        B, T = xs.shape[:2]
        dev = xs.device
        xlens_host = [int(v) for v in xlens_host]
        if self.embed_in:
            return self._forward_embed(xs, xlens_host, training, stash, st)
        elens_host = [((v - 1) // 2 - 1) // 2 for v in xlens_host]
        elens = h2d_i32(elens_host, dev)
        x, y1, y2, w2r, wlr = self._frontend_fwd(xs)
        T2, F2 = y2.shape[1], y2.shape[2]
        M = B * T2
        tab = self._pos_table(T2, dev)
        scale = math.sqrt(d)
# ... 150 lines not shown
    def _layer_fwd(self, li, x, B, T, elens, pos_t, p_enc, p_att, training):
        name = f"encoder.transformers.{li}"
        site = 100 + li * 20
        A = self.arena
        if self.conformer:
            x, s_ffm = self._ffn_fwd(name + ".feed_forward_macaron", x, 0.5, ACT_SWISH, name + ".norm_ff_macaron", 1e-5,
                                     p_enc, site, training)
            if self.rel:
                x, s_att = self._attn_fwd(name + ".self_attn", x, B, T, elens, pos_t, name + ".norm_self_attn", 1e-5,
                                          p_enc, p_att, site + 2, training)
                x, s_conv = self._conv_fwd(name + ".conv", x, B, T, name + ".norm_conv", p_enc, site + 4, training)
            else:
                x, s_conv = self._conv_fwd(name + ".conv", x, B, T, name + ".norm_conv", p_enc, site + 4, training)
                x, s_att = self._attn_fwd(name + ".self_attn", x, B, T, elens, None, name + ".norm_self_attn", 1e-5,
                                          p_enc, p_att, site + 2, training)
            x, s_ff = self._ffn_fwd(name + ".feed_forward", x, 0.5, ACT_SWISH, name + ".norm_ff", 1e-5, p_enc, site + 6,
                                    training)
            y, mean, rstd = ops.layernorm_fwd(x, A.p(name + ".norm_final.weight"), A.p(name + ".norm_final.bias"), 1e-5,
                                              self._keep)
            return y, LayerRecord(s_ffm, s_att, s_conv, s_ff, (x, mean, rstd))
        x, s_att = self._attn_fwd(name + ".self_attn", x, B, T, elens, None, name + ".norm1", 1e-12, p_enc, p_att,
                                  site + 2, training)
        x, s_ff = self._ffn_fwd(name + ".feed_forward", x, 1.0, ACT_RELU, name + ".norm2", 1e-12, p_enc, site + 6, training)
        return x, LayerRecord(None, s_att, None, s_ff, None)

    def head_logits(self, eouts, head="decoder.output", out_f32=False):
        self._apply_mode()
        B, T, d = eouts.shape
        A = self.arena
        w = A.w(head + ".weight")
        V = w.shape[0]
        out = None
        if V % 8:
            out = torch.empty(B * T, (V + 7) // 8 * 8, device=eouts.device, dtype=eouts.dtype)[:, :V]
            out_f32 = False
        if out_f32 and eouts.dtype != torch.float32:
            logits = ops.gemm_nt(eouts.reshape(B * T, d), w, bias=A.p(head + ".bias"), out_f32=True)
        else:
            logits = ops.gemm_nt(eouts.reshape(B * T, d), w, out=out, bias=A.p(head + ".bias"))
        return logits.view(B, T, V)

    def ctc_loss(self, logits, elens, ys_host, ylens_host, blank, want_grad, gscale_over_b=None):
        self._apply_mode()
        B, T, V = logits.shape
        dev = logits.device
        ylens_host = [int(v) for v in ylens_host]
        Lmax = max(max(ylens_host), 1)
        labels = torch.as_tensor(ys_host)[:, :Lmax].to(torch.int32)
        if labels.shape[1] < Lmax:
            labels = torch.nn.functional.pad(labels, (0, Lmax - labels.shape[1]))
        labels = h2d_i32(labels.contiguous(), dev)
        ylens = h2d_i32(ylens_host, dev)
        lse = ops.row_lse(logits.view(B * T, V))
        lp, alpha, beta, nll = ops.ctc_forward(logits, lse, labels, elens, ylens, blank)
        loss = torch.where(torch.isfinite(nll), nll, torch.zeros_like(nll)).sum() / B
        ctx = (logits, lse, labels, elens, ylens, blank, lp, alpha, beta, nll) if want_grad else None
        return loss, ctx

    def ctc_grad(self, ctx, gscale, gscale_dev=None):
        self._apply_mode()
        logits, lse, labels, elens, ylens, blank, lp, alpha, beta, nll = ctx
        return ops.ctc_grad(logits, lse, labels, elens, ylens, blank, lp, alpha, beta, nll, gscale / logits.shape[0],
                            gscale_dev)

    def greedy(self, logits, elens, blank):
        best, hyp, hyplen = ops.ctc_greedy(logits, elens, blank)
        return best, hyp, hyplen

    def stacked_ok(self):
        cfg = self.cfg
        return (self.encoder_stacked_ok() and _cfg(cfg, "decoder_type", "ctc") == "ctc"
                and not (_cfg(cfg, "kd_weight", 0) or 0) > 0)

    def ctc_train_stacked(self, batches, blank, scales=None, head="decoder.output"):
        assert self.stacked_ok(), "ctc_train_stacked: unsupported configuration (see stacked_ok)"
        self._defer_wgrads = self._group_wgrads
        try:
            with self._scope():
                return self._ctc_train_stacked(batches, blank, scales, head)
        finally:
            self._defer_wgrads = False
            self._wq = []
            self._ln_deferred = []

    def _stack_dtype_ok(self, single=False):
        if self.dtype == torch.bfloat16:
            return True
        if os.environ.get("EMOASR_F32_CPP_BWD", "1") == "0":
            return False
        return single or os.environ.get("EMOASR_F32_STACKED", "1") != "0"

    def encoder_stacked_ok(self):
        return (self.conformer and self.rel and self._stack_dtype_ok() and self._cpp_layers and self.attn_fused
                and not self.attn_store_scores and not self._side_wgrads and self.inter_layer == 0
                and os.environ.get("EMOASR_CPP_BWD", "1") != "0" and self._implicit_dgrad and self._conv_big
                and self.d % 256 == 0 and os.environ.get("EMOASR_STACKED", "1") != "0")

    def _encoder_fwd_stacked(self, xs_list, xlens_list, elens_dev=None):
        from .. import lib
        self.ensure_bound()
        A, d, dt = self.arena, self.d, self.dtype
        A.refresh_shadow()
        A.attach_grads()
        self.step_count += 1
        self._keep = True
        n = len(xs_list)
        assert 1 <= n <= lib.MAX_SEGMENTS
        dev = xs_list[0].device
        p_enc, p_att = self.p_enc, self.p_att
        pre = "encoder.conv."
        C = d
        w1 = A.p(pre + "conv.0.weight").view(C, 9)
        w2r = ops.strided_copy(A.p(pre + "conv.2.weight").permute(0, 2, 3, 1), out_dtype=dt).view(C, 9 * C)
        y1s, segs, xlens_all = [], [], []
        for xs, xlens in zip(xs_list, xlens_list):
            B, T, Fd = xs.shape
            T1, F1 = (T - 3) // 2 + 1, (Fd - 3) // 2 + 1
            T2, F2 = (T1 - 3) // 2 + 1, (F1 - 3) // 2 + 1
            segs.append((B, T2))
            xlens_all += [int(v) for v in xlens]
        rows = [0]
        for b, t in segs:
            rows.append(rows[-1] + b * t)
        M = rows[-1]
        elens_host = [((v - 1) // 2 - 1) // 2 for v in xlens_all]
        elens = elens_dev if elens_dev is not None else h2d_i32(elens_host, dev)
        if self._layer_rt is None:
            from ..layer_rt import ConformerLayerRuntime
            self._layer_rt = ConformerLayerRuntime(self)
        Btot, Tmax = sum(b for b, _ in segs), max(t for _, t in segs)
        masks = None
        if p_att > 0 and dt == torch.bfloat16 and os.environ.get("EMOASR_MASKS_UPFRONT", "1") != "0":
            masks = self._layer_rt.hash_attn_masks(self.nl, Btot, Tmax, elens, p_att, tuple(segs))
        y2 = torch.empty(M, F2 * C, device=dev, dtype=dt)
        for k, xs in enumerate(xs_list):
            y1 = ops.conv1_fwd(xs, w1, A.p(pre + "conv.0.bias"), dt)
            ops.conv2_fwd(y1, w2r, out=y2[rows[k]:rows[k + 1]], bias=A.p(pre + "conv.2.bias"), act=ACT_RELU)
            y1s.append(y1)
        wl = A.p(pre + "output.weight")
        wlr = ops.strided_copy(wl.view(d, C, F2).permute(0, 2, 1), out_dtype=dt).view(d, F2 * C)
        x = ops.gemm_nt(y2, wlr, bias=A.p(pre + "output.bias"))
        s_pe = self._seed(1)
        x = ops.posenc(x.view(1, M, d), None, math.sqrt(d), p_enc, s_pe).view(M, d)
        tab = torch.cat([self._pos_table(t, dev) for _, t in segs], 0)
        pos_t = ops.strided_copy(tab, out_dtype=dt)
        if p_enc > 0:
            pos_t = ops.scale_dropout(pos_t, 1.0, p_enc, self._seed(2))
        cur, layers = x, []
        for li in range(self.nl):
            cur = self._layer_rt.forward(li, cur, Btot, Tmax, elens, pos_t, p_enc, p_att, True, True, segs=tuple(segs),
                                         att_mask=None if masks is None else masks[li])
            layers.append(cur)
        x_final = cur.tv("y")
        eouts, fin_mean, fin_rstd = ops.layernorm_fwd(x_final, A.p("encoder.norm.weight"), A.p("encoder.norm.bias"), 1e-12, True)
        st = _Stash()
        st.xs_list, st.y1s, st.y2, st.wlr, st.segs, st.rows, st.M, st.F2 = xs_list, y1s, y2, wlr, segs, rows, M, F2
        st.elens, st.elens_host, st.s_pe, st.layers = elens, elens_host, s_pe, layers
        st.pos_t = pos_t
        st.att_masks = masks
        st.x_final, st.fin_mean, st.fin_rstd, st.Btot, st.Tmax = x_final, fin_mean, fin_rstd, Btot, Tmax
        return eouts, st

    def _encoder_bwd_stacked(self, st, deouts):
        A, d, dt = self.arena, self.d, self.dtype
        dev = deouts.device
        M, F2, C, rows = st.M, st.F2, self.d, st.rows
        pre = "encoder.conv."
        dx, _ = self._ln_bwd(deouts, st.x_final, "encoder.norm", st.fin_mean, st.fin_rstd, None, None)
        lnf = ops.lib.size_query("emoasr_layernorm_bwd_scratch_floats", d)
        ln_parts = torch.empty(self.nl, 5, lnf, device=dev, dtype=torch.float32)
        dx_bufs = [torch.empty(M, d, device=dev, dtype=dt) for _ in range(2)]
        for li in reversed(range(self.nl)):
            out = dx_bufs[li & 1]
            self._layer_rt.backward(li, st.layers[li], dx, out, ln_parts[li], self._ln_deferred)
            dx = out
            if self.grad_hook is not None:
                self._flush_wgrads()
                ops.layernorm_bwd_finalize(self._ln_deferred)
                self._hook_after_layer(li)
        self._flush_wgrads()
        self._layer_rt.join_wgrads()
        ops.layernorm_bwd_finalize(self._ln_deferred)
        if self.grad_hook is not None and self._layer_rt.wgrad_side:
            self.grad_hook(self._layer_offset(0))
        dlin = ops.scale_dropout(dx, math.sqrt(d), self.p_enc, st.s_pe)
        dwl = torch.zeros(d, F2 * C, device=dev, dtype=torch.float32)
        ops.gemm_tn(dlin, st.y2, out=dwl, accumulate=True, colsum=A.g(pre + "output.bias"))
        ops.strided_copy(dwl.view(d, F2, C).permute(0, 2, 1), out=A.g(pre + "output.weight").view(d, C, F2), accumulate=True)
        dy2 = ops.gemm_nn(dlin, st.wlr, dact_pre=st.y2, dact=ACT_RELU)
        dw2 = torch.zeros(C, 9 * C, device=dev, dtype=torch.float32)
        kc = dt == torch.bfloat16
        if kc:
            wt = ops.strided_copy(A.p(pre + "conv.2.weight").permute(1, 2, 3, 0), out_dtype=dt).view(C, 9 * C)
        else:
            w2r = ops.strided_copy(A.p(pre + "conv.2.weight").permute(0, 2, 3, 1), out_dtype=dt).view(C, 9 * C)
        dw1, db1 = A.g(pre + "conv.0.weight").view(C, 9), A.g(pre + "conv.0.bias")
        seg_wgrad = kc and C % 256 == 0 and len(st.xs_list) <= ops.lib.CONV2_WGRAD_SEGMENTS
        if seg_wgrad:
            ops.conv2_wgrad_seg([(dy2[rows[k]:rows[k + 1]].view(-1, C), st.y1s[k]) for k in range(len(st.xs_list))], dw2,
                                dbias=A.g(pre + "conv.2.bias"))
        for k, xs in enumerate(st.xs_list):
            dy2_k = dy2[rows[k]:rows[k + 1]].view(-1, C)
            if not seg_wgrad:
                ops.conv2_wgrad(dy2_k, st.y1s[k], dw2, dbias=A.g(pre + "conv.2.bias"), accumulate=True)
            if kc and self._conv1_fold:
                ops.conv2_dgrad_w1(dy2_k, wt, st.y1s[k], xs, dw1, db1, accumulate=True)
                continue
            dy1 = ops.conv2_dgrad_kc(dy2_k, wt, st.y1s[k]) if kc else ops.conv2_dgrad(dy2_k, w2r, st.y1s[k])
            ops.conv1_wgrad(xs, dy1, dw1, db1, accumulate=True)
        ops.strided_copy(dw2.view(C, 3, 3, C).permute(0, 3, 1, 2), out=A.g(pre + "conv.2.weight"), accumulate=True)

    def encoder_forward_stacked(self, xs_list, xlens_list):
        assert self.encoder_stacked_ok(), "encoder_forward_stacked: unsupported configuration (see encoder_stacked_ok)"
        with self._scope():
            return self._encoder_fwd_stacked(xs_list, xlens_list)

    def encoder_backward_stacked(self, st, deouts):
        self._defer_wgrads = self._group_wgrads
        try:
            with self._scope():
                self._encoder_bwd_stacked(st, deouts)
        finally:
            self._defer_wgrads = False
            self._wq = []
            self._ln_deferred = []

    def _ctc_train_stacked(self, batches, blank, scales, head):
        A = self.arena
        n = len(batches)
        scales = [1.0 / n] * n if scales is None else [float(v) for v in scales]
        dev = batches[0][0].device
        segs_h, rows_h = [], [0]
        for xs, _, _, _ in batches:
            Bk, Tk, Fd = xs.shape
            T1 = (Tk - 3) // 2 + 1
            segs_h.append((Bk, (T1 - 3) // 2 + 1))
            rows_h.append(rows_h[-1] + Bk * segs_h[-1][1])
        elens_h = [((int(v) - 1) // 2 - 1) // 2 for b in batches for v in b[1]]
        ylens_all = [int(v) for _, _, _, yl in batches for v in yl]
        Lmax = max(max(ylens_all), 1)
        lab = torch.zeros(sum(b for b, _ in segs_h), Lmax, dtype=torch.int32)
        row0, tpad, uscale, b0 = [], [], [], 0
        segw = torch.zeros(n, sum(b for b, _ in segs_h), dtype=torch.float32)
        for k, (_, _, ys, ylens) in enumerate(batches):
            B, T2 = segs_h[k]
            yk = torch.as_tensor(ys)[:, :Lmax].to(torch.int32)
            lab[b0:b0 + B, : yk.shape[1]] = yk
            row0 += [rows_h[k] + b * T2 for b in range(B)]
            tpad += [T2] * B
            uscale += [scales[k] / B] * B
            segw[k, b0:b0 + B] = 1.0 / B
            b0 += B
        elens_d, labels, yl, row0_d, tpad_d, uscale_d, segw_d = h2d_pack(
            [torch.tensor(elens_h, dtype=torch.int32), lab, torch.tensor(ylens_all, dtype=torch.int32),
             torch.tensor(row0, dtype=torch.int64), torch.tensor(tpad, dtype=torch.int32),
             torch.tensor(uscale, dtype=torch.float32), segw], dev)
        eouts, st = self._encoder_fwd_stacked([b[0] for b in batches], [b[1] for b in batches], elens_dev=elens_d)
        segs, rows, elens, Btot, Tmax = st.segs, st.rows, st.elens, st.Btot, st.Tmax
        assert list(segs) == segs_h and list(rows) == rows_h
        w = A.w(head + ".weight")
        V = w.shape[0]
        assert V % 8 == 0, "ctc_train_stacked: vocabulary must be a multiple of 8"
        logits, lse = ops.gemm_nt_lse(eouts, w, A.p(head + ".bias"))
        Vp = (V + 63) // 64 * 64
        dlp = torch.empty(logits.shape[0], Vp, device=dev, dtype=logits.dtype)
        if Vp > V:
            dlp[:, V:].zero_()
        dlogits = dlp[:, :V]
        lp, alpha, beta, nll = ops.ctc_forward_rows(logits, lse, labels, elens, yl, blank, row0_d, Tmax)
        losses = (segw_d * torch.nan_to_num(nll, nan=0.0, posinf=0.0, neginf=0.0)).sum(1)
        ops.ctc_grad_rows(logits, lse, labels, elens, yl, blank, lp, alpha, beta, nll, 1.0, row0_d, tpad_d, uscale_d, dlogits)
        if self.dtype == torch.bfloat16 and os.environ.get("EMOASR_HEAD_NT", "1") != "0":
            self._wgrad(dlogits, eouts, A.g(head + ".weight", tuple(w.shape)), 1.0, A.g(head + ".bias"), 1.0)
            w_t = torch.zeros(w.shape[1], Vp, device=dev, dtype=w.dtype)
            w_t[:, :V].copy_(w.t())
            deouts = ops.gemm_nt(dlp, w_t)
        else:
            deouts = self._lin_bwd(dlogits, eouts, head + ".weight", head + ".bias")
        if self.grad_hook is not None:
            self._flush_wgrads()
            self.grad_hook(A.offsets[head + ".weight"])
        self._encoder_bwd_stacked(st, deouts)
        return losses

    def _lin_bwd(self, dy, x_in, wname, bname, alpha=1.0, **epi):
        A = self.arena
        w = A.w(wname)
        w2 = w.view(w.shape[0], -1)
        self._wgrad(dy, x_in, A.g(wname, tuple(w2.shape)), alpha, A.g(bname), alpha)
        return ops.gemm_nn(dy, w2, alpha=alpha, **epi)

    def _wgrad(self, dy, x_in, out, alpha=1.0, colsum=None, colsum_scale=1.0):
        if self._defer_wgrads:
            self._wq.append((dy, x_in, out, alpha, colsum, colsum_scale))
        else:
            ops.gemm_tn(dy, x_in, out=out, alpha=alpha, accumulate=True, colsum=colsum, colsum_scale=colsum_scale)

    def _hook_after_layer(self, li):
        if not self._layer_rt.wgrad_side:
            self.grad_hook(self._layer_offset(li))
            return
        self._layer_rt.join_wgrads(keep=1)
        if li + 1 < self.nl:
            self.grad_hook(self._layer_offset(li + 1))

    def _layer_offset(self, li):
        if self._layer_lo is None:
            lo = {}
# ... 275 lines not shown
```

emoasr_amd/layer_rt.py:

```python
import ctypes
import os

import torch

from . import lib, ops
from .engine.arena import AttnStash, ConvStash, FFNStash, LayerRecord

_ALIGN_T, _ALIGN_F = 64, 16


def _round(n, a):
    return (n + a - 1) // a * a


class _Layout:

    def __init__(self, B, T, d, H, F, segs=None):
        self.segs = segs
        if segs is None:
            M, R = B * T, 2 * T - 1
            qkv_shape, o_shape, lse_shape, nstat = (B, T, 3 * d), (B, T, d), (B, H, T), 1
            npart = lib.size_query("emoasr_dwconv_stats_floats", B, T, d)
        else:
            M, R = sum(b * t for b, t in segs), sum(2 * t - 1 for _, t in segs)
            qkv_shape, o_shape, lse_shape, nstat = (M, 3 * d), (M, d), (H * M,), len(segs)
            npart = sum(lib.size_query("emoasr_dwconv_stats_floats", b, t, d) for b, t in segs)
        self.M, self.R = M, R
        self.mask_nw = lib.size_query("emoasr_attn_dropmask_words", T if segs is None else max(t for _, t in segs))
        t_fields = [("ffm_h", (M, d)), ("ffm_u", (M, F)), ("ffm_a", (M, F)), ("ffm_y", (M, d)),
                    ("at_h", (M, d)), ("qkv", qkv_shape), ("pp", (R, d)), ("o", o_shape), ("at_y", (M, d)),
                    ("cv_h", (M, d)), ("g", (M, 2 * d)), ("gl", (M, d)), ("c", (M, d)), ("z", (M, d)), ("cv_y", (M, d)),
                    ("ff_h", (M, d)), ("ff_u", (M, F)), ("ff_a", (M, F)), ("ff_y", (M, d)), ("y", (M, d))]
        f_fields = [("ffm_mean", (M,)), ("ffm_rstd", (M,)), ("lse", lse_shape), ("at_mean", (M,)), ("at_rstd", (M,)),
                    ("bmean", (nstat * d,)), ("bvar", (nstat * d,)), ("bn_part", (npart,)),
                    ("cv_mean", (M,)), ("cv_rstd", (M,)), ("ff_mean", (M,)), ("ff_rstd", (M,)),
                    ("fin_mean", (M,)), ("fin_rstd", (M,)), ("att_mask", (M * H * self.mask_nw,))]
        self.t, self.f = {}, {}
        off = 0
        for name, shape in t_fields:
            n = 1
            for s in shape:
                n *= s
            self.t[name] = (off, n, shape)
            off += _round(n, _ALIGN_T)
        self.nt = off
        off = 0
        for name, shape in f_fields:
            n = 1
            for s in shape:
                n *= s
            self.f[name] = (off, n, shape)
            off += _round(n, _ALIGN_F)
        self.nf = off


class LayerStash:
    __slots__ = ("wt", "wf", "lay", "x_in", "seeds", "_tup", "io", "B", "T", "sweep")

    def __init__(self, wt, wf, lay, x_in, seeds):
        self.wt, self.wf, self.lay, self.x_in, self.seeds, self._tup = wt, wf, lay, x_in, seeds, None
        self.io = None

    def tv(self, name):
        o, n, shape = self.lay.t[name]
        return self.wt[o:o + n].view(shape)

    def fv(self, name):
        o, n, shape = self.lay.f[name]
        return self.wf[o:o + n].view(shape)

    def input(self):
        x = self.x_in
        if isinstance(x, LayerStash):
            x = self.x_in = x.tv("y")
        return x

    def __iter__(self):
        if self.lay.segs is not None:
            raise RuntimeError("a stacked layer pass is differentiated by emoasr_conformer_layer_bwd only (no per-kernel path)")
        if self._tup is None:
            tv, fv, s = self.tv, self.fv, self.seeds
            x0 = self.input()
            x1, x2, x3, x4 = tv("ffm_y"), tv("at_y"), tv("cv_y"), tv("ff_y")
            s_ffm = FFNStash(x0, fv("ffm_mean"), fv("ffm_rstd"), tv("ffm_h"), tv("ffm_u"), tv("ffm_a"), s[0], s[1])
            s_att = AttnStash(x1, fv("at_mean"), fv("at_rstd"), tv("at_h"), tv("qkv"), tv("pp"), tv("o"), fv("lse"), s[2], s[3],
                              None)
            s_conv = ConvStash(x2, fv("cv_mean"), fv("cv_rstd"), tv("cv_h"), tv("g"), tv("gl"), tv("c"), fv("bmean"), fv("bvar"),
                               tv("z"), s[4])
            s_ff = FFNStash(x3, fv("ff_mean"), fv("ff_rstd"), tv("ff_h"), tv("ff_u"), tv("ff_a"), s[5], s[6])
            self._tup = LayerRecord(s_ffm, s_att, s_conv, s_ff, (x4, fv("fin_mean"), fv("fin_rstd")))
        return iter(self._tup)

    def __getitem__(self, i):
        return tuple(self)[i]


class ConformerLayerRuntime:
    def __init__(self, eng):
        self.eng = eng
        self.params = {}
        self.grads = {}
        self.layouts = {}
        self.bwd_ws = [None, None]
        self.wgrad_side = os.environ.get("EMOASR_CPP_WGRAD_SIDE", "0") != "0"
        lib.set_option("wgrad_side", int(self.wgrad_side))
        self.calls = 0
        self.attn_img, self.attn_img_key = None, None
        self.sweeps = 0

    def _layer_params(self, li):
        eng, A = self.eng, self.eng.arena
        name = f"encoder.transformers.{li}"
        bn = name + ".conv.batch_norm"
        rm = eng._buffers(bn + ".running_mean")
        guard = (A.flat.data_ptr(), A.shadow.data_ptr(), rm.data_ptr())
        hit = self.params.get(li)
        if hit is not None and hit[1] == guard:
            return hit[0]
        d = eng.d
        L = lib.ConformerLayer()
        L.d, L.H = d, eng.h
        w1 = A.w(name + ".feed_forward.w1.weight")
        L.F = w1.shape[0]
        wd = A.p(name + ".conv.depthwise_conv.weight")
        L.K = wd.shape[-1]

        def ffn(dst, pre, norm):
            dst.ln_g, dst.ln_b = A.p(norm + ".weight").data_ptr(), A.p(norm + ".bias").data_ptr()
            dst.w1, dst.b1 = A.w(pre + ".w1.weight").data_ptr(), A.p(pre + ".w1.bias").data_ptr()
            dst.w2, dst.b2 = A.w(pre + ".w2.weight").data_ptr(), A.p(pre + ".w2.bias").data_ptr()

        ffn(L.ffm, name + ".feed_forward_macaron", name + ".norm_ff_macaron")
        ffn(L.ff, name + ".feed_forward", name + ".norm_ff")
        sa = name + ".self_attn"
        L.att_ln_g, L.att_ln_b = A.p(name + ".norm_self_attn.weight").data_ptr(), A.p(name + ".norm_self_attn.bias").data_ptr()
        L.wqkv = A.w_span(sa + ".linear_q.weight", sa + ".linear_v.weight", (3 * d, d)).data_ptr()
        L.bqkv = A.p_span(sa + ".linear_q.bias", sa + ".linear_v.bias", (3 * d,)).data_ptr()
        L.wpos = A.w(sa + ".linear_pos.weight").data_ptr()
        L.bias_u, L.bias_v = A.p(sa + ".pos_bias_u").data_ptr(), A.p(sa + ".pos_bias_v").data_ptr()
        L.wout, L.bout = A.w(sa + ".linear_out.weight").data_ptr(), A.p(sa + ".linear_out.bias").data_ptr()
        cv = name + ".conv"
        L.cv_ln_g, L.cv_ln_b = A.p(name + ".norm_conv.weight").data_ptr(), A.p(name + ".norm_conv.bias").data_ptr()
        L.pw1, L.pw1_b = A.w(cv + ".pointwise_conv1.weight", (2 * d, d)).data_ptr(), A.p(cv + ".pointwise_conv1.bias").data_ptr()
        L.dw_w, L.dw_b = wd.data_ptr(), A.p(cv + ".depthwise_conv.bias").data_ptr()
        L.bn_g, L.bn_b = A.p(bn + ".weight").data_ptr(), A.p(bn + ".bias").data_ptr()
        L.bn_rm, L.bn_rv = rm.data_ptr(), eng._buffers(bn + ".running_var").data_ptr()
        L.bn_nbt = eng._buffers(bn + ".num_batches_tracked").data_ptr()
        L.pw2, L.pw2_b = A.w(cv + ".pointwise_conv2.weight", (d, d)).data_ptr(), A.p(cv + ".pointwise_conv2.bias").data_ptr()
        L.fin_ln_g, L.fin_ln_b = A.p(name + ".norm_final.weight").data_ptr(), A.p(name + ".norm_final.bias").data_ptr()
        if A.shadow.dtype == torch.bfloat16 and os.environ.get("EMOASR_DGRAD_NT", "1") != "0":
            L.ffm_w1t = A.transposed(name + ".feed_forward_macaron.w1.weight").data_ptr()
            L.ff_w1t = A.transposed(name + ".feed_forward.w1.weight").data_ptr()
            L.wqkv_t = A.transposed(sa + ".linear_q.weight", sa + ".linear_v.weight", (3 * d, d)).data_ptr()
            L.pw1_t = A.transposed(cv + ".pointwise_conv1.weight", None, (2 * d, d)).data_ptr()
            if os.environ.get("EMOASR_DGRAD_NT2", "0") != "0":
                L.ffm_w2t = A.transposed(name + ".feed_forward_macaron.w2.weight").data_ptr()
                L.ff_w2t = A.transposed(name + ".feed_forward.w2.weight").data_ptr()
                L.wout_t = A.transposed(sa + ".linear_out.weight").data_ptr()
                L.pw2_t = A.transposed(cv + ".pointwise_conv2.weight", None, (d, d)).data_ptr()
        self.params[li] = (L, guard)
        return L

    def hash_attn_masks(self, nl, B, T, elens, p_att, segs):
        eng = self.eng
        lay = self._layout(B, T, self._layer_params(0).F, segs)
        masks = torch.empty(nl, lay.M * eng.h * lay.mask_nw, device=elens.device, dtype=torch.int32)
        seeds = (ctypes.c_uint64 * nl)(*[eng._seed(100 + li * 20 + 2) for li in range(nl)])
        seg = lib.Segments()
        seg.n = len(segs)
        for k, (sb, stt) in enumerate(segs):
            seg.B[k], seg.T[k] = sb, stt
        lib.call("emoasr_conformer_attn_masks", lib.BF16, nl, ctypes.byref(seg), B, T, eng.h, eng.d, elens.data_ptr(), p_att, seeds,
                 masks.data_ptr(), masks.stride(0), lay.mask_nw, ops._stream())
        return masks

    def _layout(self, B, T, F, segs):
        key = (B, T) if segs is None else tuple(segs)
        lay = self.layouts.get(key)
        if lay is None:
            if len(self.layouts) > 64:
                self.layouts.clear()
            lay = self.layouts[key] = _Layout(B, T, self.eng.d, self.eng.h, F, segs)
        return lay

    def forward(self, li, x, B, T, elens, pos_t, p_enc, p_att, training, keep, segs=None, att_mask=None):
        eng = self.eng
        L = self._layer_params(li)
        lay = self._layout(B, T, L.F, segs)
        dev = pos_t.device
        wt = torch.empty(lay.nt, device=dev, dtype=eng.dtype)
        wf = torch.empty(lay.nf, device=dev, dtype=torch.float32)
        site = 100 + li * 20
        seeds = tuple(eng._seed(site + k) for k in (0, 1, 2, 3, 4, 6, 7))
        st = LayerStash(wt, wf, lay, x, seeds)
        if isinstance(x, LayerStash):
            st.sweep = x.sweep
        else:
            self.sweeps += 1
            st.sweep = self.sweeps
        esz = wt.element_size()
        tb, fb = wt.data_ptr(), wf.data_ptr()
        t, f = lay.t, lay.f
        io = lib.ConformerFwd()
        io.B, io.T = B, T
        if segs is not None:
            assert len(segs) <= lib.MAX_SEGMENTS, f"at most {lib.MAX_SEGMENTS} stacked micro-batches"
            io.seg.n = len(segs)
            for k, (sb, stt) in enumerate(segs):
                io.seg.B[k], io.seg.T[k] = sb, stt
        io.x = tb_prev(x, esz)
        io.pos_t, io.klens = pos_t.data_ptr(), elens.data_ptr()
        io.training, io.p_enc, io.p_att = int(training), p_enc, p_att
        io.seed[:] = seeds
        io.ffm.h, io.ffm.u, io.ffm.a, io.ffm.y = (tb + t["ffm_h"][0] * esz, tb + t["ffm_u"][0] * esz if keep else None,
                                                  tb + t["ffm_a"][0] * esz, tb + t["ffm_y"][0] * esz)
        io.ff.h, io.ff.u, io.ff.a, io.ff.y = (tb + t["ff_h"][0] * esz, tb + t["ff_u"][0] * esz if keep else None,
                                              tb + t["ff_a"][0] * esz, tb + t["ff_y"][0] * esz)
        for k in ("at_h", "qkv", "pp", "o", "at_y", "cv_h", "g", "gl", "c", "z", "cv_y", "y"):
            setattr(io, k, tb + t[k][0] * esz)
        io.lse = fb + f["lse"][0] * 4
        if training and p_att > 0 and wt.dtype == torch.bfloat16:
            if att_mask is not None:
                io.att_mask, io.att_mask_nw, io.att_mask_ready = att_mask.data_ptr(), lay.mask_nw, 1
            else:
                io.att_mask, io.att_mask_nw = fb + f["att_mask"][0] * 4, lay.mask_nw
        io.bmean, io.bvar, io.bn_part = fb + f["bmean"][0] * 4, fb + f["bvar"][0] * 4, fb + f["bn_part"][0] * 4
        if keep:
            io.ffm.mean, io.ffm.rstd = fb + f["ffm_mean"][0] * 4, fb + f["ffm_rstd"][0] * 4
            io.ff.mean, io.ff.rstd = fb + f["ff_mean"][0] * 4, fb + f["ff_rstd"][0] * 4
            io.at_mean, io.at_rstd = fb + f["at_mean"][0] * 4, fb + f["at_rstd"][0] * 4
            io.cv_mean, io.cv_rstd = fb + f["cv_mean"][0] * 4, fb + f["cv_rstd"][0] * 4
            io.fin_mean, io.fin_rstd = fb + f["fin_mean"][0] * 4, fb + f["fin_rstd"][0] * 4
        lib.call("emoasr_conformer_layer_fwd", ops.dt(wt), ctypes.byref(L), ctypes.byref(io), ops._stream())
        st.io, st.B, st.T = io, B, T
        return st

    def _layer_grads(self, li):
        eng, A = self.eng, self.eng.arena
        guard = A.grad.data_ptr()
        hit = self.grads.get(li)
        if hit is not None and hit[1] == guard:
            return hit[0]
        name = f"encoder.transformers.{li}"
        d = eng.d
        G = lib.ConformerLayer()

        def gp(n):
            return A.g(n).data_ptr()

        def ffn(dst, pre, norm):
            dst.ln_g, dst.ln_b = gp(norm + ".weight"), gp(norm + ".bias")
            dst.w1, dst.b1, dst.w2, dst.b2 = gp(pre + ".w1.weight"), gp(pre + ".w1.bias"), gp(pre + ".w2.weight"), gp(pre + ".w2.bias")

        ffn(G.ffm, name + ".feed_forward_macaron", name + ".norm_ff_macaron")
        ffn(G.ff, name + ".feed_forward", name + ".norm_ff")
        sa, cv, bn = name + ".self_attn", name + ".conv", name + ".conv.batch_norm"
        G.att_ln_g, G.att_ln_b = gp(name + ".norm_self_attn.weight"), gp(name + ".norm_self_attn.bias")
        G.wqkv = A.g_span(sa + ".linear_q.weight", sa + ".linear_v.weight", (3 * d, d)).data_ptr()
        G.bqkv = A.g_span(sa + ".linear_q.bias", sa + ".linear_v.bias", (3 * d,)).data_ptr()
        G.wpos = gp(sa + ".linear_pos.weight")
        G.bias_u, G.bias_v = gp(sa + ".pos_bias_u"), gp(sa + ".pos_bias_v")
        G.wout, G.bout = gp(sa + ".linear_out.weight"), gp(sa + ".linear_out.bias")
        G.cv_ln_g, G.cv_ln_b = gp(name + ".norm_conv.weight"), gp(name + ".norm_conv.bias")
        G.pw1, G.pw1_b = gp(cv + ".pointwise_conv1.weight"), gp(cv + ".pointwise_conv1.bias")
        G.dw_w, G.dw_b = gp(cv + ".depthwise_conv.weight"), gp(cv + ".depthwise_conv.bias")
        G.bn_g, G.bn_b = gp(bn + ".weight"), gp(bn + ".bias")
        G.pw2, G.pw2_b = gp(cv + ".pointwise_conv2.weight"), gp(cv + ".pointwise_conv2.bias")
        G.fin_ln_g, G.fin_ln_b = gp(name + ".norm_final.weight"), gp(name + ".norm_final.bias")
        self.grads[li] = (G, guard)
        return G

    def backward(self, li, st, dy, dx, ln_part, deferred):
        eng, A = self.eng, self.eng.arena
        L, G = self._layer_params(li), self._layer_grads(li)
        B, T = st.B, st.T
        if st.lay.segs is None:
            nb = lib.size_query("emoasr_conformer_layer_bwd_ws_bytes", ops.dt(st.wt), B, T, eng.d, eng.h, L.F, L.K)
        else:
            nb = lib.ws_bytes_seg(ops.dt(st.wt), st.io.seg, eng.d, eng.h, L.F, L.K)
        k = (self.calls & 1) if self.wgrad_side else 0
        self.calls += 1
        if self.bwd_ws[k] is None or self.bwd_ws[k].numel() < nb:
            self.join_wgrads()
            self.bwd_ws[k] = torch.empty(int(nb * 1.1) + 256, device=dy.device, dtype=torch.uint8)
        io = lib.ConformerBwd()
        io.dy, io.dx = dy.data_ptr(), dx.data_ptr()
        io.ws, io.ws_bytes = self.bwd_ws[k].data_ptr(), self.bwd_ws[k].numel()
        if st.wt.dtype != torch.bfloat16:
            seg = st.io.seg
            if st.lay.segs is None:
                seg = lib.Segments()
                seg.n, seg.B[0], seg.T[0] = 1, B, T
            ni = lib.img_bytes_seg(ops.dt(st.wt), seg, eng.d, eng.h)
            key = st.sweep
            if self.attn_img is None or self.attn_img.numel() < ni:
                self.attn_img, self.attn_img_key = torch.empty(int(ni * 1.1) + 256, device=dy.device, dtype=torch.uint8), None
            if self.attn_img_key != key:
                self.attn_img[:ni].zero_()
                self.attn_img_key = key
            io.attn_img, io.attn_img_bytes = self.attn_img.data_ptr(), self.attn_img.numel()
        io.ln_part, io.ln_part_stride = ln_part.data_ptr(), ln_part.stride(0)
        lib.call("emoasr_conformer_layer_bwd", ops.dt(st.wt), ctypes.byref(L), ctypes.byref(G), ctypes.byref(st.io),
                 ctypes.byref(io), ops._stream())
        name = f"encoder.transformers.{li}"
        M = st.lay.M
        for k, norm in enumerate(("norm_final", "norm_ff", "norm_conv", "norm_self_attn", "norm_ff_macaron")):
            deferred.append((M, eng.d, ln_part[k], A.g(f"{name}.{norm}.weight"), A.g(f"{name}.{norm}.bias")))

    def join_wgrads(self, keep=0):
        if self.wgrad_side:
            lib.call("emoasr_wgrad_side_join", int(keep), ops._stream())


def tb_prev(x, esz):
    if isinstance(x, LayerStash):
        return x.wt.data_ptr() + x.lay.t["y"][0] * esz
    return x.data_ptr()
```

emoasr_amd/lib.py:

```python
import contextlib
import ctypes
import os
from ctypes import (POINTER, Structure, c_char_p, c_float, c_int, c_long, c_uint64,
                    c_void_p)

_HERE = os.path.dirname(os.path.abspath(__file__))
LIB_PATH = os.environ.get("EMOASR_HIP_LIB") or os.path.join(_HERE, "libemoasr_hip.so")

F32, BF16, F32X3 = 0, 1, 2
ACT_NONE, ACT_RELU, ACT_SWISH, ACT_GELU = 0, 1, 2, 3


class Epilogue(Structure):
    _fields_ = [("bias", c_void_p), ("residual", c_void_p), ("pre_out", c_void_p),
                ("dact_pre", c_void_p), ("alpha", c_float), ("res_scale", c_float),
                ("act", c_int), ("dact", c_int), ("ldr", c_int), ("out_f32", c_int),
                ("drop_p", c_float), ("seed", c_uint64)]


class AttnArgs(Structure):
    _fields_ = [("B", c_int), ("H", c_int), ("DK", c_int), ("Tq", c_int), ("Tk", c_int),
                ("ldq", c_long), ("ldk", c_long), ("ldv", c_long), ("ldo", c_long), ("ldp", c_long),
                ("q", c_void_p), ("k", c_void_p), ("v", c_void_p), ("pos", c_void_p),
                ("bias_u", c_void_p), ("bias_v", c_void_p), ("klens", c_void_p),
# ... 88 lines not shown
                ("len_weight", ctypes.c_double), ("vals", c_void_p), ("cands", c_void_p), ("lm_at", c_void_p), ("psi", c_void_p),
                ("score", c_void_p), ("score_ctc", c_void_p),
                ("n_ids", c_void_p), ("n_parent", c_void_p), ("n_pcand", c_void_p), ("n_last", c_void_p),
                ("n_outlen", c_void_p), ("n_klens", c_void_p), ("hist_parent", c_void_p), ("hist_token", c_void_p),
                ("res_score", c_void_p), ("res_step", c_void_p), ("res_parent", c_void_p), ("state", c_void_p),
                ("host_mirror", c_void_p)]


class JointStep(Structure):
    _fields_ = [("dec_nl", c_int), ("dec_layers", POINTER(DecoderLayer)), ("dec", DecoderStep),
                ("lm_nl", c_int), ("lm_layers", POINTER(BertLayer)), ("lm", BertStep),
                ("dec_k_prev", c_void_p), ("dec_v_prev", c_void_p), ("lm_k_prev", c_void_p), ("lm_v_prev", c_void_p),
                ("parent", c_void_p), ("scores_pre", c_void_p), ("ctc_x", c_void_p), ("T", c_int), ("blank", c_int),
                ("states_prev", c_void_p), ("states_cur", c_void_p), ("upd", BeamUpdate)]


class BeamUpdateBatch(Structure):
    _fields_ = [("u", BeamUpdate), ("S", c_int), ("max_pos", c_int), ("pos", c_void_p), ("ctl", c_void_p)]


class DecoderStepGroup(Structure):
    _fields_ = [("d", DecoderStep), ("S", c_int), ("W", c_int), ("moff", c_void_p)]


class JointBatchStep(Structure):
    _fields_ = [("dec_nl", c_int), ("dec_layers", POINTER(DecoderLayer)), ("dec", DecoderStepGroup),
                ("lm_nl", c_int), ("lm_layers", POINTER(BertLayer)), ("lm", BertStep),
                ("dec_k_prev", c_void_p), ("dec_v_prev", c_void_p), ("lm_k_prev", c_void_p), ("lm_v_prev", c_void_p),
                ("parent", c_void_p), ("ctc_x", c_void_p), ("Tmax", c_int), ("blank", c_int),
                ("states_prev", c_void_p), ("states_cur", c_void_p), ("upd", BeamUpdateBatch)]


class JointGridStep(Structure):
    _fields_ = [("js", JointBatchStep), ("U", c_int), ("n_groups", c_int), ("group_rows", c_int),
                ("sutt", c_void_p), ("groups", c_void_p), ("mu", c_void_p), ("mu_row", c_void_p)]


class FfnParams(Structure):
    _fields_ = [("ln_g", c_void_p), ("ln_b", c_void_p), ("w1", c_void_p), ("b1", c_void_p),
                ("w2", c_void_p), ("b2", c_void_p)]


class ConformerLayer(Structure):
    _fields_ = [("d", c_int), ("H", c_int), ("F", c_int), ("K", c_int), ("ffm", FfnParams), ("ff", FfnParams),
                ("att_ln_g", c_void_p), ("att_ln_b", c_void_p), ("wqkv", c_void_p), ("bqkv", c_void_p),
                ("wpos", c_void_p), ("bias_u", c_void_p), ("bias_v", c_void_p), ("wout", c_void_p), ("bout", c_void_p),
                ("cv_ln_g", c_void_p), ("cv_ln_b", c_void_p), ("pw1", c_void_p), ("pw1_b", c_void_p),
                ("dw_w", c_void_p), ("dw_b", c_void_p), ("bn_g", c_void_p), ("bn_b", c_void_p),
                ("bn_rm", c_void_p), ("bn_rv", c_void_p), ("bn_nbt", c_void_p), ("pw2", c_void_p), ("pw2_b", c_void_p),
                ("fin_ln_g", c_void_p), ("fin_ln_b", c_void_p),
                ("ffm_w1t", c_void_p), ("ff_w1t", c_void_p), ("wqkv_t", c_void_p), ("pw1_t", c_void_p),
                ("ffm_w2t", c_void_p), ("ff_w2t", c_void_p), ("wout_t", c_void_p), ("pw2_t", c_void_p)]


class TcItem(Structure):
    _fields_ = [("src", c_void_p), ("dst", c_void_p), ("rows", c_int), ("cols", c_int), ("ld_dst", c_long)]


TC_MAX = 64


class FfnStash(Structure):
    _fields_ = [("h", c_void_p), ("u", c_void_p), ("a", c_void_p), ("y", c_void_p), ("mean", c_void_p),
                ("rstd", c_void_p)]


MAX_SEGMENTS = 8


class Segments(Structure):
    _fields_ = [("n", c_int), ("B", c_int * MAX_SEGMENTS), ("T", c_int * MAX_SEGMENTS)]


class ConformerFwd(Structure):
    _fields_ = [("B", c_int), ("T", c_int), ("x", c_void_p), ("pos_t", c_void_p), ("klens", c_void_p),
                ("training", c_int), ("p_enc", c_float), ("p_att", c_float), ("seed", c_uint64 * 7),
                ("ffm", FfnStash), ("ff", FfnStash),
                ("at_h", c_void_p), ("qkv", c_void_p), ("pp", c_void_p), ("o", c_void_p), ("at_y", c_void_p),
                ("lse", c_void_p), ("at_mean", c_void_p), ("at_rstd", c_void_p),
                ("cv_h", c_void_p), ("g", c_void_p), ("gl", c_void_p), ("c", c_void_p), ("z", c_void_p),
                ("cv_y", c_void_p), ("bmean", c_void_p), ("bvar", c_void_p), ("bn_part", c_void_p),
                ("cv_mean", c_void_p), ("cv_rstd", c_void_p),
                ("y", c_void_p), ("fin_mean", c_void_p), ("fin_rstd", c_void_p), ("seg", Segments),
                ("att_mask", c_void_p), ("att_mask_nw", c_int), ("att_mask_ready", c_int)]

class ConformerBwd(Structure):
    _fields_ = [("dy", c_void_p), ("dx", c_void_p), ("ws", c_void_p), ("ws_bytes", ctypes.c_size_t),
                ("ln_part", c_void_p), ("ln_part_stride", c_long), ("attn_img", c_void_p), ("attn_img_bytes", ctypes.c_size_t)]


class LasAttend(Structure):
    _fields_ = [("B", c_int), ("T", c_int), ("A", c_int), ("D", c_int),
                ("pk", c_void_p), ("pk_bstride", c_long), ("pq", c_void_p), ("aw_prev", c_void_p),
                ("filt", c_void_p), ("w_conv", c_void_p), ("b_conv", c_void_p), ("w_score", c_void_p),
                ("eouts", c_void_p), ("eo_bstride", c_long), ("elens", c_void_p),
                ("drop_p", c_float), ("seed", c_uint64), ("step", c_int),
                ("scores", c_void_p), ("aw", c_void_p), ("lse", c_void_p), ("ctx", c_void_p), ("ctx_ld", c_long),
                ("dctx", c_void_p), ("dctx_ld", c_long), ("daw", c_void_p),
                ("dpq", c_void_p), ("daw_prev", c_void_p), ("dpk", c_void_p), ("deouts", c_void_p),
                ("dw_score", c_void_p), ("dw_conv", c_void_p), ("db_conv", c_void_p), ("dfilt", c_void_p)]


class LasAttendGroup(Structure):
    _fields_ = [("S", c_int), ("W", c_int), ("A", c_int), ("D", c_int), ("Tmax", c_int), ("rows", c_int),
                ("pk", c_void_p), ("eouts", c_void_p), ("moff", c_void_p), ("pq", c_void_p), ("aw_src", c_void_p),
                ("parent", c_void_p), ("state", c_void_p),
                ("filt", c_void_p), ("w_conv", c_void_p), ("b_conv", c_void_p), ("w_score", c_void_p),
                ("scores", c_void_p), ("aw_dst", c_void_p), ("ctx", c_void_p), ("ctx_ld", c_long)]


LAS_GATHER_MAX = 16


class LasGatherItem(Structure):
    _fields_ = [("src", c_void_p), ("dst", c_void_p), ("row_bytes", c_long)]


class LasStateGather(Structure):
    _fields_ = [("S", c_int), ("W", c_int), ("n", c_int), ("parent", c_void_p), ("state", c_void_p),
                ("item", LasGatherItem * LAS_GATHER_MAX)]


P, I, L, F, U64 = c_void_p, c_int, c_long, c_float, c_uint64

SIGNATURES = {
    "emoasr_gemm_nt": [I, I, I, I, P, L, P, L, P, L, POINTER(Epilogue), P],
    "emoasr_gemm_nn": [I, I, I, I, P, L, P, L, P, L, POINTER(Epilogue), P],
    "emoasr_gemm_tn": [I, I, I, I, P, L, P, L, P, L, F, I, P, F, P],
    "emoasr_gemm_nn_batched": [I, I, I, I, P, L, L, L, P, L, L, L, P, L, L, L, I, I, F, I, P],
    "emoasr_gemm_tn_grouped": [I, I, POINTER(TnProblem), P],
    "emoasr_gemm_tn_grouped_plan": [I, I, POINTER(TnProblem), POINTER(c_int), POINTER(c_int), POINTER(c_int)],
    "emoasr_colsum": [I, I, I, P, L, P, F, I, P],
    "emoasr_conv1_fwd": [I, I, I, I, I, P, P, P, P, P],
    "emoasr_conv1_wgrad": [I, I, I, I, I, P, P, P, P, I, P, P],
    "emoasr_conv2_fwd": [I, I, I, I, I, P, P, P, POINTER(Epilogue), P],
    "emoasr_conv2_wgrad": [I, I, I, I, I, P, P, P, P, I, P],
    "emoasr_conv2_wgrad_seg": [I, I, POINTER(Conv2WgradSeg), I, I, P, P, P],
    "emoasr_conv2_col2im": [I, I, I, I, I, P, P, P, P],
    "emoasr_conv2_dgrad": [I, I, I, I, I, P, P, P, P, P],
    "emoasr_conv2_dgrad_kc": [I, I, I, I, I, P, P, P, P, P],
    "emoasr_conv2_dgrad_w1": [I, I, I, I, I, P, P, P, P, P, P, I, P, P],
    "emoasr_gemm_nt_big": [I, I, I, I, P, L, P, L, P, L, P, I, P],
    "emoasr_layernorm_fwd": [I, I, I, P, P, P, F, P, P, P, P],
    "emoasr_layernorm_bwd": [I, I, I, P, P, P, P, P, P, P, P, P, P, P],
    "emoasr_layernorm_bwd_ex": [I, I, I, P, P, P, P, P, P, P, P, P, P, POINTER(LnBwdOpts), P],
    "emoasr_layernorm_bwd_finalize": [I, POINTER(LnFinalizeItem), P],
    "emoasr_conformer_layer_fwd": [I, POINTER(ConformerLayer), POINTER(ConformerFwd), P],
    "emoasr_conformer_attn_masks": [I, I, POINTER(Segments), I, I, I, I, P, F, P, P, L, I, P],
    "emoasr_conformer_layer_bwd": [I, POINTER(ConformerLayer), POINTER(ConformerLayer), POINTER(ConformerFwd),
                                   POINTER(ConformerBwd), P],
    "emoasr_transformer_decoder_infer": [I, I, POINTER(DecoderLayer), POINTER(DecoderInfer), P],
    "emoasr_bert_lm_infer": [I, I, POINTER(BertLayer), POINTER(BertInfer), P],
    "emoasr_transformer_decoder_step": [I, I, POINTER(DecoderLayer), POINTER(DecoderStep), P],
    "emoasr_bert_lm_step": [I, I, POINTER(BertLayer), POINTER(BertStep), P],
    "emoasr_beam_cache_gather": [I, I, I, I, I, P, P, P, P, P, P, P],
    "emoasr_beam_update": [POINTER(BeamUpdate), P],
    "emoasr_beam_scores_topk": [I, I, I, I, P, L, P, L, F, P, P, P, P],
    "emoasr_rowlin": [I, I, I, P, L, P, P, F, P, P, I, P, L, P, P, F, P, I, L, P],
    "emoasr_attn_step": [I, I, I, I, P, P, P, P, P, P],
    "emoasr_joint_beam_step": [I, POINTER(JointStep), P, P],
    "emoasr_joint_beam_step_parts": [I, POINTER(JointStep), I, P],
    "emoasr_joint_beam_graph_build": [I, POINTER(JointStep), I, I, P],
    "emoasr_joint_beam_graph_launch": [I, I, P],
    "emoasr_attn_step_group": [I, I, I, I, I, P, P, P, P, P],
    "emoasr_group_offsets_check": [I, POINTER(c_int)],
    "emoasr_beam_update_batch": [POINTER(BeamUpdateBatch), P],
    "emoasr_ctc_prefix_init_ragged": [I, I, P, P, I, P, L, P],
    "emoasr_ctc_prefix_score_ragged": [I, I, I, I, I, P, P, P, I, P, P, P, P, P, I, I, P, P, P],
    "emoasr_transformer_decoder_step_group": [I, I, POINTER(DecoderLayer), POINTER(DecoderStepGroup), P],
    "emoasr_joint_beam_batch_step": [I, POINTER(JointBatchStep), P],
    "emoasr_attn_step_cells": [I, I, I, I, I, I, I, P, P, P, P, P, P],
    "emoasr_cell_groups_check": [I, POINTER(c_int), I, I, I],
    "emoasr_beam_scores_topk_rows": [I, I, I, I, P, L, P, L, P, P, P, P, P],
    "emoasr_ctc_prefix_init_cells": [I, I, I, P, P, P, I, P, L, P],
    "emoasr_ctc_prefix_score_cells": [I, I, I, I, I, P, P, P, P, I, P, P, P, P, P, I, I, P, P, P],
    "emoasr_beam_update_cells": [POINTER(BeamUpdateBatch), P, P],
    "emoasr_joint_beam_grid_step": [I, POINTER(JointGridStep), P],
    "emoasr_attn_dropmask": [I, POINTER(AttnArgs), P, I, P],
    "emoasr_attn_fwd": [I, POINTER(AttnArgs), P],
    "emoasr_attn_bwd": [I, POINTER(AttnArgs), P],
    "emoasr_attn_bwd_fused": [I, POINTER(AttnArgs), P, ctypes.c_size_t, P],
    "emoasr_glu_fwd": [I, I, I, P, P, P],
    "emoasr_glu_fwd_masked": [I, I, I, I, P, P, P, P],
    "emoasr_glu_bwd": [I, I, I, P, P, P, P],
    "emoasr_dwconv_fwd": [I, I, I, I, I, P, P, P, P, P],
    "emoasr_dwconv_bwd_x": [I, I, I, I, I, P, P, P, P],
    "emoasr_dwconv_fwd_stats": [I, I, I, I, I, P, P, P, P, P, P],
    "emoasr_bn_stats_finalize": [I, I, I, P, P, P, P, P, F, P, P],
    "emoasr_dwconv_bwd_w": [I, I, I, I, I, P, P, P, P, I, P, P],
    "emoasr_bn_stats": [I, I, I, P, P, P, P, P, F, P],
    "emoasr_bn_swish_fwd": [I, I, I, P, P, P, P, P, F, P, P],
    "emoasr_bn_swish_bwd": [I, I, I, P, P, P, P, P, P, F, P, P, P, P, P],
    "emoasr_glu_dwconv_fwd": [I, I, I, I, I, P, P, P, P, P, P],
    "emoasr_bn_swish_bwd_sums": [I, I, I, P, P, P, P, P, P, F, P, P, P, P, P],
    "emoasr_conv_bwd_fused": [I, I, I, I, I, P, P, P, P, P, P, F, P, P, P, P, P, P, P, P],
    "emoasr_strided_copy": [I, I, P, P, I, I, I, I, L, L, L, L, I, P],
    "emoasr_transpose_cast_batched": [I, I, P, P],
    "emoasr_scale_dropout": [I, L, P, P, F, F, U64, P],
    "emoasr_posenc": [I, I, I, I, P, P, F, F, U64, P, P],
    "emoasr_add": [I, L, P, P, P, P],
    "emoasr_row_lse": [I, I, I, P, L, P, P],
    "emoasr_gemm_nt_lse": [I, I, I, I, P, L, P, L, P, L, P, P, P, P],
    "emoasr_ctc_forward": [I, I, I, I, I, P, L, P, P, P, P, I, P, P, P, P, P],
    "emoasr_ctc_grad": [I, I, I, I, I, P, L, P, P, P, P, I, P, P, P, P, F, P, P, L, P],
    "emoasr_rnnt_greedy": [I, I, I, I, I, I, I, I, I, P, P, P, P, P, P, P, P, P, P, P, P, P, L, P, P, P, P],
    "emoasr_wgrad_side_join": [I, P],
    "emoasr_rnnt_beam_lstm": [I, I, I, I, P, L, P, P, P, P, P, P, P, P, P, P, I, P],
    "emoasr_rnnt_beam_joint": [I, I, I, I, I, P, P, P, P, P, P, P, P],
    "emoasr_rnnt_beam_pick": [I, I, I, I, I, P, L, P, L, P],
    "emoasr_rnnt_beam_lstm_rows": [I, I, I, I, P, L, L, P, P, P, P, P, P, L, P, P, P, P],
    "emoasr_rnnt_beam_joint_rows": [I, I, I, I, I, P, L, P, P, P, P, P, P, P, P],
    "emoasr_rnnt_beam_start": [I, I, I, I, I, P, P, P, L, P, P],
    "emoasr_rnnt_beam_book": [I, I, I, I, I, P, P, L, P, P, L, P, P],
    "emoasr_rnnt_beam_finish": [I, I, I, I, I, P, I, P, P, P, P, P, L, P, P],
    "emoasr_rnnt_beam_pick_lm": [I, I, I, I, I, I, I, P, L, P, L, P, P, P, L, P],
    "emoasr_rnnt_beam_gather_rows": [I, I, I, P, L, P, P, P, P],
    "emoasr_rnnlm_step": [I, I, I, I, I, I, I, P, P, P, P, P, P, P, P, P, P, P, P, L, I, P, P, L, P],
    "emoasr_las_attend_fwd": [I, POINTER(LasAttend), P],
    "emoasr_las_attend_bwd": [I, POINTER(LasAttend), P],
    "emoasr_las_dropmask": [POINTER(LasAttend), P, P],
    "emoasr_las_attend_group": [I, POINTER(LasAttendGroup), P],
    "emoasr_las_state_gather": [POINTER(LasStateGather), P],
    "emoasr_mlm_expand": [I, I, I, P, P, P, I, I, I, I, P, P, P, P, P],
    "emoasr_sample_rows": [I, I, I, P, L, P, P, U64, L, P, P, P, P],
    "emoasr_gumbel_noise": [I, I, U64, L, P, L, P],
    "emoasr_electra_corrupt": [I, I, P, P, P, P, P, P, P, P],
    "emoasr_bce_head_fwd": [I, I, I, P, L, P, P, P, P, P, P, P, P],
    "emoasr_bce_head_bwd": [I, I, I, P, L, P, P, P, P, F, P, P, L, P, P, P],
    "emoasr_ctc_token_conf": [I, I, I, I, P, L, P, P, P, I, P, P, P, P],
# ... 67 lines not shown

ENV_ALIASES = {
    "EMOASR_CONV_FUSED": _off("conv_fused", "dwconv_lds"),
    "EMOASR_FFN_SAVE_DACT": _off("ffn_save_dact"),
    "EMOASR_CONV_BIG": _off("conv_big"),
    "EMOASR_BIG_MIN_TILES": lambda value: [("big_min_tiles", int(value))],
    "EMOASR_DECODE_COOP": lambda value: [("decode_coop", int(value))],
}


def load():
    global _lib
    if _lib is not None:
        return _lib
    if not os.path.exists(LIB_PATH):
        raise EmoasrHipError(
            f"{LIB_PATH} not found: build it with `python -m emoasr_amd.build` "
            "(hipcc --offload-arch=gfx950).  There is no CPU fallback.")
    import torch
    lib = ctypes.CDLL(LIB_PATH)
    lib.emoasr_last_error.restype = c_char_p
    lib.emoasr_last_error.argtypes = []
    lib.emoasr_version.restype = c_int
    lib.emoasr_set_option.argtypes = [c_char_p, c_int]
    lib.emoasr_set_option.restype = c_int
    lib.emoasr_get_option.argtypes = [c_char_p, POINTER(c_int), POINTER(c_int)]
    lib.emoasr_get_option.restype = c_int
    lib.emoasr_option_count.argtypes = []
    lib.emoasr_option_count.restype = c_int
    lib.emoasr_option_name.argtypes = [c_int]
    lib.emoasr_option_name.restype = c_char_p
    for name, args in SIGNATURES.items():
        fn = getattr(lib, name)
        fn.argtypes = args
        fn.restype = c_int
    _lib = lib
    pairs = []
    for var, to_pairs in ENV_ALIASES.items():
        if os.environ.get(var):
            pairs += [(var, n, v) for n, v in to_pairs(os.environ[var])]
    for item in filter(None, os.environ.get("EMOASR_OPTIONS", "").split(",")):
        name, _, value = item.partition("=")
        pairs.append(("EMOASR_OPTIONS", name.strip(), int(value)))
    for var, name, value in pairs:
        if lib.emoasr_set_option(name.encode(), value) != 0:
            raise EmoasrHipError(f"{var}: {lib.emoasr_last_error().decode()}")
    return lib


_FN = {}

def call(name, *args):
    fn = _FN.get(name)
    if fn is None:
        fn = _FN[name] = getattr(load(), name)
    rc = fn(*args)
    if rc != 0:
        raise EmoasrHipError(f"{name} failed ({rc}): {load().emoasr_last_error().decode()}")


_SIZE_FN = {}


def size_query(name, *ints):
    fn = _SIZE_FN.get(name)
    if fn is None:
        fn = getattr(load(), name)
        fn.restype = ctypes.c_long
        fn.argtypes = [c_int] * len(ints)
        _SIZE_FN[name] = fn
    return int(fn(*[int(v) for v in ints]))


def ws_bytes_seg(dtype_code, seg, d, H, F, K):
    fn = load().emoasr_conformer_layer_bwd_ws_bytes_seg
    fn.restype = ctypes.c_size_t
    fn.argtypes = [c_int, POINTER(Segments), c_int, c_int, c_int, c_int]
    n = int(fn(dtype_code, ctypes.byref(seg), d, H, F, K))
    if n == 0:
        raise EmoasrHipError("emoasr_conformer_layer_bwd_ws_bytes_seg: bad segment description")
    return n


def img_bytes_seg(dtype_code, seg, d, H):
    fn = load().emoasr_conformer_layer_bwd_img_bytes_seg
    fn.restype = ctypes.c_size_t
    fn.argtypes = [c_int, POINTER(Segments), c_int, c_int]
    return int(fn(dtype_code, ctypes.byref(seg), d, H))


def timer_read(name, reset=True):
    lib = load()
    calls, ms = c_int(0), ctypes.c_double(0.0)
    lib.emoasr_timer_read.argtypes = [c_char_p, POINTER(c_int), POINTER(ctypes.c_double), c_int]
    lib.emoasr_timer_read.restype = c_int
    if lib.emoasr_timer_read(name.encode(), ctypes.byref(calls), ctypes.byref(ms), int(reset)) != 0:
        raise EmoasrHipError(lib.emoasr_last_error().decode())
    return calls.value, ms.value


TIMER_FAMILIES = ("attn_bwd_fused_kernel", "attn_bwd_dpos_kernel", "attn_fwd_kernel", "gemm_tn_grouped_kernel", "gemm_nt_nn",
                  "gemm_tn", "layernorm", "conv_module")


def timer_mask(*names):
    m = 0
    for n in names:
        m |= 1 << (TIMER_FAMILIES.index(n) + 1)
    return m


def timer_read_ex(name, reset=True):
    lib = load()
    calls, ms, fl, by = c_int(0), ctypes.c_double(0.0), ctypes.c_double(0.0), ctypes.c_double(0.0)
    fn = lib.emoasr_timer_read_ex
    fn.argtypes = [c_char_p, POINTER(c_int)] + [POINTER(ctypes.c_double)] * 3 + [c_int]
    fn.restype = c_int
    if fn(name.encode(), ctypes.byref(calls), ctypes.byref(ms), ctypes.byref(fl), ctypes.byref(by), int(reset)) != 0:
        raise EmoasrHipError(lib.emoasr_last_error().decode())
    return calls.value, ms.value, fl.value, by.value


def set_option(name, value):
    lib = load()
    if lib.emoasr_set_option(name.encode(), int(value)) != 0:
        raise EmoasrHipError(lib.emoasr_last_error().decode())


def _get_option(name):
    lib = load()
    value, default = c_int(0), c_int(0)
    if lib.emoasr_get_option(name.encode(), ctypes.byref(value), ctypes.byref(default)) != 0:
        raise EmoasrHipError(lib.emoasr_last_error().decode())
    return value.value, default.value


def get_option(name):
    return _get_option(name)[0]


def option_default(name):
    return _get_option(name)[1]


def option_names():
    lib = load()
    return [lib.emoasr_option_name(i).decode() for i in range(lib.emoasr_option_count())]


@contextlib.contextmanager
def options(**values):
    saved = []
    try:
        for name, value in values.items():
            saved.append((name, get_option(name)))
            set_option(name, value)
        yield
    finally:
        for name, value in reversed(saved):
            set_option(name, value)
```

emoasr_amd/ops.py:

```python
import ctypes
from ctypes import byref, c_void_p

import os
import threading
from types import SimpleNamespace

import torch

from . import lib
from .lib import ACT_GELU, ACT_NONE, ACT_RELU, ACT_SWISH, BF16, F32, F32X3, AttnArgs, Epilogue

_DT = {torch.float32: F32, torch.bfloat16: BF16}


def dt(t):
    if t.dtype == torch.float32 and split_products():
        return F32X3
    return _DT[t.dtype]


def _p(t):
    return None if t is None else c_void_p(t.data_ptr())


# ... 164 lines not shown
    if out is None:
        y2 = torch.empty(B, T2, F2, C, device=y1.device, dtype=y1.dtype)
    else:
        assert out.is_contiguous() and out.numel() == B * T2 * F2 * C and out.dtype == y1.dtype
        y2 = out.view(B, T2, F2, C)
    ep = make_epilogue(**epi)
    lib.call("emoasr_conv2_fwd", dt(y1), B, T1, F1, C, _p(y1), _p(_chk(w, y1.dtype)), _p(y2), byref(ep),
             _stream())
    return y2


def conv2_wgrad(dy2, y1, dw, dbias=None, accumulate=False):
    B, T1, F1, C = y1.shape
    lib.call("emoasr_conv2_wgrad", dt(y1), B, T1, F1, C, _p(dy2), _p(y1), _p(_chk(dw, torch.float32)),
             _p(dbias), int(accumulate), _stream())


def conv2_wgrad_seg(segs, dw, dbias=None):
    assert 1 <= len(segs) <= lib.CONV2_WGRAD_SEGMENTS
    _, _, F1, C = segs[0][1].shape
    arr = (lib.Conv2WgradSeg * len(segs))()
    for q, (dy2, y1) in zip(arr, segs):
        B, T1, f1, c = y1.shape
        assert (f1, c) == (F1, C) and y1.dtype == segs[0][1].dtype
        _chk(dy2, y1.dtype)
        q.dy2, q.y1, q.B, q.T1 = dy2.data_ptr(), _chk(y1).data_ptr(), B, T1
    lib.call("emoasr_conv2_wgrad_seg", dt(segs[0][1]), len(segs), arr, F1, C, _p(_chk(dw, torch.float32)), _p(dbias), _stream())


def conv2_dgrad(dy2, w, y1):
    B, T1, F1, C = y1.shape
    dy1 = torch.empty_like(y1)
    lib.call("emoasr_conv2_dgrad", dt(y1), B, T1, F1, C, _p(_chk(dy2, y1.dtype)), _p(_chk(w, y1.dtype)), _p(y1), _p(dy1),
             _stream())
    return dy1


def conv2_dgrad_kc(dy2, wt, y1):
    B, T1, F1, C = y1.shape
    dy1 = torch.empty_like(y1)
    lib.call("emoasr_conv2_dgrad_kc", dt(y1), B, T1, F1, C, _p(_chk(dy2, y1.dtype)), _p(_chk(wt, y1.dtype)), _p(y1), _p(dy1),
             _stream())
    return dy1


def conv2_dgrad_w1(dy2, wt, y1, x, dw1, db1, accumulate=False):
    B, T1, F1, C = y1.shape
    Bx, T, Fd = x.shape
    assert Bx == B and (T - 3) // 2 + 1 == T1 and (Fd - 3) // 2 + 1 == F1, (x.shape, y1.shape)
    scratch = torch.empty(lib.size_query("emoasr_conv2_dgrad_w1_scratch_floats", B, T, Fd, C), device=x.device,
                          dtype=torch.float32)
    lib.call("emoasr_conv2_dgrad_w1", dt(y1), B, T, Fd, C, _p(_chk(dy2, y1.dtype)), _p(_chk(wt, y1.dtype)), _p(y1),
             _p(_chk(x, torch.float32)), _p(_chk(dw1, torch.float32)), _p(_chk(db1, torch.float32)), int(accumulate),
             _p(scratch), _stream())


def gemm_nt_big(a, b, out=None, bias=None, relu=False):
    M, K, lda = _rows(_chk(a, torch.bfloat16))
    N, Kb, ldb = _rows(_chk(b, a.dtype))
    assert K == Kb, (a.shape, b.shape)
    if out is None:
        out = torch.empty(M, N, device=a.device, dtype=a.dtype)
    lib.call("emoasr_gemm_nt_big", dt(a), M, N, K, _p(a), lda, _p(b), ldb, _p(out), out.stride(0), _p(bias), int(relu),
             _stream())
    return out


def conv2_col2im(dcol, y1):
    B, T1, F1, C = y1.shape
    dy1 = torch.empty_like(y1)
    lib.call("emoasr_conv2_col2im", dt(y1), B, T1, F1, C, _p(dcol), _p(y1), _p(dy1), _stream())
    return dy1


def layernorm_fwd(x, gamma, beta, eps, want_stats=True):
    M, N, ld = _rows(_chk(x))
    assert ld == N
    y = torch.empty_like(x)
    mean = torch.empty(M, device=x.device, dtype=torch.float32) if want_stats else None
    rstd = torch.empty(M, device=x.device, dtype=torch.float32) if want_stats else None
    lib.call("emoasr_layernorm_fwd", dt(x), M, N, _p(x), _p(gamma), _p(beta), eps, _p(y), _p(mean), _p(rstd),
             _stream())
    return y, mean, rstd


def layernorm_bwd(dy, x, gamma, mean, rstd, dres, dgamma, dbeta, branch=None, deferred=None):
    M, N, ld = _rows(_chk(x))
    dx = torch.empty_like(x)
    scratch = None
    if dgamma is not None or dbeta is not None:
        scratch = torch.empty(lib.size_query("emoasr_layernorm_bwd_scratch_floats", N), device=x.device, dtype=torch.float32)
    if branch is None and deferred is None:
        lib.call("emoasr_layernorm_bwd", dt(x), M, N, _p(dy), _p(x), _p(gamma), _p(mean), _p(rstd), _p(dres), _p(dx),
                 _p(dgamma), _p(dbeta), _p(scratch), _stream())
        return dx
    o = lib.LnBwdOpts()
    dy2 = None
    if branch is not None:
        dy2 = torch.empty_like(x)
        o.dy2, o.scale2, o.drop_p2, o.seed2 = dy2.data_ptr(), branch[0], branch[1], branch[2]
    if deferred is not None and scratch is not None:
        o.defer_finalize = 1
        deferred.append((M, N, scratch, dgamma, dbeta))
    lib.call("emoasr_layernorm_bwd_ex", dt(x), M, N, _p(dy), _p(x), _p(gamma), _p(mean), _p(rstd), _p(dres), _p(dx),
             _p(dgamma), _p(dbeta), _p(scratch), byref(o), _stream())
    return dx if branch is None else (dx, dy2)


def layernorm_bwd_finalize(deferred):
    for i0 in range(0, len(deferred), lib.LN_FINALIZE_MAX):
        chunk = deferred[i0:i0 + lib.LN_FINALIZE_MAX]
        arr = (lib.LnFinalizeItem * len(chunk))()
        for it, (M, N, scratch, dgamma, dbeta) in zip(arr, chunk):
            it.M, it.N, it.part = M, N, scratch.data_ptr()
            it.dgamma = None if dgamma is None else dgamma.data_ptr()
            it.dbeta = None if dbeta is None else dbeta.data_ptr()
        lib.call("emoasr_layernorm_bwd_finalize", len(chunk), arr, _stream())
    del deferred[:]


def _attn_args(q, k, v, H, pos, bias_u, bias_v, klens, causal, scale, drop_p, seed):
    B, Tq, D = q.shape
    Tk = k.shape[1]
    a = AttnArgs()
    a.B, a.H, a.DK, a.Tq, a.Tk = B, H, D // H, Tq, Tk
    assert q.stride(2) == 1 and k.stride(2) == 1 and v.stride(2) == 1
    assert q.stride(0) == Tq * q.stride(1) and k.stride(0) == Tk * k.stride(1) and v.stride(0) == Tk * v.stride(1)
    a.ldq, a.ldk, a.ldv = q.stride(1), k.stride(1), v.stride(1)
    a.q, a.k, a.v = q.data_ptr(), k.data_ptr(), v.data_ptr()
    if pos is not None:
        a.pos, a.ldp = pos.data_ptr(), pos.stride(0)
    a.bias_u = None if bias_u is None else bias_u.data_ptr()
    a.bias_v = None if bias_v is None else bias_v.data_ptr()
    a.klens = None if klens is None else klens.data_ptr()
    a.causal = int(causal)
    a.scale, a.drop_p, a.seed = scale, drop_p, seed
    return a


def attn_dropmask(q, k, H, klens=None, drop_p=0.0, seed=0):
    B, Tq, _ = q.shape
    nw = lib.size_query("emoasr_attn_dropmask_words", k.shape[1])
    a = _attn_args(q, k, k, H, None, None, None, klens, False, 1.0, drop_p, seed)
    mask = torch.zeros(B * Tq, H, nw, device=q.device, dtype=torch.int32)
    lib.call("emoasr_attn_dropmask", dt(q), byref(a), mask.data_ptr(), nw, _stream())
    return mask


def attn_fwd(q, k, v, H, scale, pos=None, bias_u=None, bias_v=None, klens=None, causal=False, drop_p=0.0,
             seed=0, store_scores=False, keep_mask=None):
    B, Tq, D = q.shape
    a = _attn_args(q, k, v, H, pos, bias_u, bias_v, klens, causal, scale, drop_p, seed)
    out = torch.empty(B, Tq, D, device=q.device, dtype=q.dtype)
    lse = torch.empty(B, H, Tq, device=q.device, dtype=torch.float32)
    a.out, a.ldo, a.lse = out.data_ptr(), D, lse.data_ptr()
    if keep_mask is not None:
        a.keep_mask, a.keep_nw = keep_mask.data_ptr(), keep_mask.shape[-1]
    st = None
    if store_scores:
        st = torch.empty(B, H, k.shape[1], (Tq + 7) // 8 * 8, device=q.device, dtype=torch.float32)
        a.st, a.ldst = st.data_ptr(), st.shape[-1]
    lib.call("emoasr_attn_fwd", dt(q), byref(a), _stream())
    return (out, lse, st) if store_scores else (out, lse)


class AttnScratch:
# ... 1442 lines not shown
```

include/emoasr_hip.h:

```cpp
#ifndef EMOASR_HIP_H
#define EMOASR_HIP_H
#include <stddef.h>
#include <stdint.h>
#ifdef __cplusplus
extern "C" {
#endif

enum { EMOASR_F32 = 0, EMOASR_BF16 = 1, EMOASR_F32X3 = 2 };
enum { EMOASR_ACT_NONE = 0, EMOASR_ACT_RELU = 1, EMOASR_ACT_SWISH = 2,
       EMOASR_DACT_MUL = 6 };
#define EMOASR_ACT_SAVE_DACT 0x100

const char* emoasr_last_error(void);
int emoasr_version(void);
int emoasr_set_option(const char* name, int value);
int emoasr_get_option(const char* name, int* value, int* default_value);
int emoasr_option_count(void);
const char* emoasr_option_name(int index);
int emoasr_timer_read(const char* name, int* calls, double* ms, int reset);
int emoasr_timer_read_ex(const char* name, int* calls, double* ms, double* flops, double* bytes, int reset);

typedef struct {
  const float* bias;
  const void* residual;
// ... 358 lines not shown

int emoasr_sample_rows(int dtype, int M, int V, const void* logits, long ld, const int* labels, const float* w, uint64_t seed,
                       long row0, float* loss, float* lse, int* sample, void* stream);
int emoasr_gumbel_noise(int M, int V, uint64_t seed, long row0, float* out, long ldo, void* stream);
int emoasr_electra_corrupt(int BN, int M, const int* ids, const int* sel, const int* labels, const int* samples, int* generated,
                           float* replaced, int* counters, void* stream);
int emoasr_bce_head_fwd(int dtype, int M, int H, const void* h, long ldh, const void* wp, const float* bp, const float* y,
                        const float* w, float* z, float* loss, float* sig, void* stream);
int emoasr_bce_head_bwd(int dtype, int M, int H, const void* h, long ldh, const void* wp, const float* z, const float* y,
                        const float* w, float gscale, const float* gscale_dev, void* dh, long lddh, float* dwp, float* dbp,
                        void* stream);

int emoasr_ctc_token_conf(int dtype, int B, int T, int V, const void* logits, long ld, const float* lse, const int* best,
                          const int* elens, int blank, int* frame, float* conf, int* ntok, void* stream);
int emoasr_correct_fuse(int dtype_asr, int dtype_lm, int n, int V_asr, int V_lm, int n_cols, const void* asr, long ld_asr,
                        const float* asr_lse, const int* asr_rows, long asr_nrows, const void* lm, long ld_lm, float w,
                        int* out_id, float* out_val, void* stream);
#define EMO_CORRECT_MAX_WEIGHTS 16
int emoasr_correct_mask_grid(int B, int T, int NT, const int* hyp, const int* ntok, const float* conf, const int* frame,
                             const float* ths, int mask_id, int pad_id, int* ys, int* num_masked, int* lm_rows, int* asr_rows,
                             void* stream);
int emoasr_correct_fuse_grid(int dtype_asr, int dtype_lm, int n, int V_asr, int V_lm, int n_cols, const void* asr, long ld_asr,
                             const float* asr_lse, const int* asr_rows, long asr_nrows, const void* lm, long ld_lm,
                             const float* weights, int NW, int* out_id, float* out_val, void* stream);

#define EMOASR_EDIT_MAX_LEN 4096
#define EMOASR_EDIT_LDS_WORDS 4096
enum { EMOASR_ALIGN_NONE = 0, EMOASR_ALIGN_SI = 1, EMOASR_ALIGN_SID = 2 };
long emoasr_edit_align_lds_words(void);
long emoasr_edit_align_ws_words(int ref_len, int hyp_len);
int emoasr_edit_align(int P, int n_ref, int max_hyp_len, int max_ref_len, const int* hyp, const int* hyp_off, const int* ref,
                      const int* ref_off, const int* ref_idx, int label_mode, int* counts, unsigned char* ops,
                      const long* ops_off, unsigned char* labels, void* ws, const long* ws_off, int* status, void* stream);
int emoasr_rescore_grid(int N, int U, int G1, int G2, const double* score_asr, const double* score_lm, const int* ylen,
                        const int* utt_off, const int* counts, const double* lm_w, const double* len_w, int* best,
                        long long* totals, void* stream);

typedef struct emoasr_ffn_params {
  const float *ln_g, *ln_b;
  const void* w1; const float* b1;
  const void* w2; const float* b2;
} emoasr_ffn_params_t;
typedef struct emoasr_conformer_layer {
  int d, H, F, K;
  emoasr_ffn_params_t ffm, ff;
  const float *att_ln_g, *att_ln_b;
  const void* wqkv; const float* bqkv;
  const void* wpos;
  const float *bias_u, *bias_v;
  const void* wout; const float* bout;
  const float *cv_ln_g, *cv_ln_b;
  const void* pw1; const float* pw1_b;
  const float *dw_w, *dw_b;
  const float *bn_g, *bn_b;
  float *bn_rm, *bn_rv; long long* bn_nbt;
  const void* pw2; const float* pw2_b;
  const float *fin_ln_g, *fin_ln_b;
  const void *ffm_w1t, *ff_w1t, *wqkv_t, *pw1_t;
  const void *ffm_w2t, *ff_w2t, *wout_t, *pw2_t;
} emoasr_conformer_layer_t;
typedef struct emoasr_ffn_stash {
  void *h, *u, *a, *y;
  float *mean, *rstd;
} emoasr_ffn_stash_t;
typedef struct emoasr_segments {
  int n;
  int B[EMOASR_MAX_SEGMENTS], T[EMOASR_MAX_SEGMENTS];
} emoasr_segments_t;
typedef struct emoasr_conformer_fwd {
  int B, T;
  const void* x;
  const void* pos_t;
  const int* klens;
  int training;
  float p_enc, p_att;
  uint64_t seed[7];
  emoasr_ffn_stash_t ffm, ff;
  void *at_h, *qkv, *pp, *o, *at_y; float *lse, *at_mean, *at_rstd;
  void *cv_h, *g, *gl, *c, *z, *cv_y; float *bmean, *bvar, *bn_part, *cv_mean, *cv_rstd;
  void* y; float *fin_mean, *fin_rstd;
  emoasr_segments_t seg;
  unsigned* att_mask; int att_mask_nw;
  int att_mask_ready;
} emoasr_conformer_fwd_t;
int emoasr_conformer_attn_masks(int dtype, int nl, const emoasr_segments_t* seg, int B, int T, int H, int d, const int* klens,
                                float p_att, const uint64_t* seeds, unsigned* masks, long layer_stride_words, int nw, void* stream);
int emoasr_conformer_layer_fwd(int dtype, const emoasr_conformer_layer_t* layer,
                               const emoasr_conformer_fwd_t* io, void* stream);
typedef struct emoasr_conformer_bwd {
  const void* dy;
  void* dx;
  void* ws; size_t ws_bytes;
  float* ln_part; long ln_part_stride;
  void* attn_img; size_t attn_img_bytes;
} emoasr_conformer_bwd_t;
size_t emoasr_conformer_layer_bwd_ws_bytes(int dtype, int B, int T, int d, int H, int F, int K);
int emoasr_conv_module_fwd_seg(int dtype, const emoasr_segments_t* seg, int C, int K, const void* g, const float* w,
                               const float* bias, void* c, float* part, float* bmean, float* bvar, float* running_mean,
                               float* running_var, float momentum, long long* num_batches_tracked, const float* gamma,
                               const float* beta, float eps, void* z, int training, void* stream);
long emoasr_conv_module_bwd_seg_scratch_floats(const emoasr_segments_t* seg, int C, int K, int which);
int emoasr_conv_module_bwd_seg(int dtype, const emoasr_segments_t* seg, int C, int K, const void* dz, const void* c,
                               const float* bmean, const float* bvar, const float* gamma, const float* beta, float eps,
                               float* dgamma, float* dbeta, const void* g, const float* w, void* dg, float* dw, float* dbias,
                               float* bn_scratch, float* dw_scratch, void* stream);
size_t emoasr_conformer_layer_bwd_ws_bytes_seg(int dtype, const emoasr_segments_t* seg, int d, int H, int F, int K);
int emoasr_wgrad_side_join(int keep, void* stream);
size_t emoasr_conformer_layer_bwd_img_bytes_seg(int dtype, const emoasr_segments_t* seg, int d, int H);
int emoasr_conformer_layer_bwd(int dtype, const emoasr_conformer_layer_t* layer, const emoasr_conformer_layer_t* grads,
                               const emoasr_conformer_fwd_t* st, const emoasr_conformer_bwd_t* io, void* stream);

typedef struct emoasr_lin { const void* w; const float* b; } emoasr_lin_t;
typedef struct emoasr_lnp { const float *g, *b; } emoasr_lnp_t;
typedef struct emoasr_decoder_layer {
  emoasr_lnp_t ln1, ln2, ln3;
  emoasr_lin_t qkv, out;
  emoasr_lin_t q2, out2;
  emoasr_lin_t w1, w2;
} emoasr_decoder_layer_t;
typedef struct emoasr_decoder_infer {
  int nb, L, T, dd, H, F, V;
  const int* ids;
  const void* embed; const float* pe; float emb_scale;
  const int *kself, *kmem;
  const void* const* kv;
  emoasr_lnp_t ln_out; emoasr_lin_t out;
  void* logits_last;
  void* ws; size_t ws_bytes;
} emoasr_decoder_infer_t;
typedef struct emoasr_bert_layer {
  emoasr_lin_t qkv, attn_out; emoasr_lnp_t ln_attn;
  emoasr_lin_t inter, out; emoasr_lnp_t ln_out;
} emoasr_bert_layer_t;
typedef struct emoasr_bert_infer {
  int nb, L, d, H, F, V;
  const int* ids; const void* word_emb; const float* pe;
  emoasr_lnp_t ln_emb;
  const int* klens;
  emoasr_lin_t transform; emoasr_lnp_t ln_transform; const float* out_bias;
  float* logp;
  void* ws; size_t ws_bytes;
} emoasr_bert_infer_t;
size_t emoasr_decode_ws_bytes(int dtype, int nb, int L, int d, int H, int F, int V);
int emoasr_transformer_decoder_infer(int dtype, int nl, const emoasr_decoder_layer_t* layers,
                                     const emoasr_decoder_infer_t* io, void* stream);
int emoasr_bert_lm_infer(int dtype, int nl, const emoasr_bert_layer_t* layers, const emoasr_bert_infer_t* io,
                         void* stream);

typedef struct emoasr_decoder_step {
  int nb, Lmax, T, dd, H, F, V;
  const int* ids; const int* pos; const int* klens;
  const void* embed; const float* pe; float emb_scale;
  const int* kmem; const void* const* kv;
  void* kcache; void* vcache;
  emoasr_lnp_t ln_out; emoasr_lin_t out;
  void* logits_last;
  void* ws; size_t ws_bytes;
} emoasr_decoder_step_t;
typedef struct emoasr_bert_step {
  int nb, Lmax, d, H, F, V;
  const int* ids; const int* pos; const int* klens;
  const void* word_emb; const float* pe; emoasr_lnp_t ln_emb;
  void* kcache; void* vcache;
  emoasr_lin_t transform; emoasr_lnp_t ln_transform; const float* out_bias;
  float* logp;
  int raw_logits;
  void* ws; size_t ws_bytes;
} emoasr_bert_step_t;
size_t emoasr_decode_step_ws_bytes(int dtype, int nb, int d, int H, int F, int V);
int emoasr_transformer_decoder_step(int dtype, int nl, const emoasr_decoder_layer_t* layers, const emoasr_decoder_step_t* io,
                                    void* stream);
int emoasr_bert_lm_step(int dtype, int nl, const emoasr_bert_layer_t* layers, const emoasr_bert_step_t* io, void* stream);
int emoasr_rowlin(int M, int N, int K, const void* x, long ldx, const float* lna_g, const float* lna_b, float lna_eps,
                  const void* w, const float* bias, int act, const void* res, long ldres, const float* lnr_g,
                  const float* lnr_b, float lnr_eps, void* y, int out_f32, long ldy, void* stream);
int emoasr_attn_step(int nb, int d, int H, int Lmax, const void* qkv, void* kcache, void* vcache, const int* pos, void* out,
                     void* stream);
long emoasr_decode_coop_status(void);
// ... 162 lines not shown
```

Before: 6.083 million frames/s.

## Batch per-layer positional projections and defer depthwise-conv weight-grad reductions into grouped launches

Computes the relative positional projection for all layers in one strided batched GEMM before the layer loop instead of one small GEMM per layer. Also defers each layer's depthwise-conv weight-gradient reduction into a per-layer partial table and reduces all layers together in a single grouped kernel at the end of backward. Both are meant to cut kernel-launch count and small-kernel tail cost. In exchange, every layer now allocates a separate fp32 partial table, which raises memory use, and the all-layer positional buffer is allocated on each forward.

```diff
diff --git a/emoasr_amd/csrc/convfused.hip b/emoasr_amd/csrc/convfused.hip
--- a/emoasr_amd/csrc/convfused.hip
+++ b/emoasr_amd/csrc/convfused.hip
@@ -460,10 +460,10 @@
   return emoasr_dwconv_bwd_w_scratch_floats(sg.b0[sg.n], tmax, C, K);
 }
 
-extern "C" int emoasr_conv_module_bwd_seg(int dtype, const emoasr_segments_t* seg, int C, int K, const void* dz, const void* c,
-                                          const float* bmean, const float* bvar, const float* gamma, const float* beta, float eps,
-                                          float* dgamma, float* dbeta, const void* g, const float* w, void* dg, float* dw,
-                                          float* dbias, float* bn_scratch, float* dw_scratch, void* stream) {
+int emo_conv_module_bwd_seg(int dtype, const emoasr_segments_t* seg, int C, int K, const void* dz, const void* c, const float* bmean,
+                            const float* bvar, const float* gamma, const float* beta, float eps, float* dgamma, float* dbeta,
+                            const void* g, const float* w, void* dg, float* dw, float* dbias, float* bn_scratch, float* dw_scratch,
+                            int defer_reduce, void* stream) {
   EMO_CHECK(dtype == EMO_BF16, "conv_module_bwd_seg: bf16 only");
   EMO_CHECK(K <= CF_MAXK && (K & 1) && C % 8 == 0, "conv_module_bwd_seg: K=%d (odd, <= %d), C=%d (multiple of 8)", K, CF_MAXK, C);
   EMO_CHECK(bn_scratch && dw_scratch, "conv_module_bwd_seg: scratch required");
@@ -480,5 +480,21 @@
   cf_conv_bwd_kernel<<<grid, CF_CB, CF_BWD_LDS, s>>>(tmax, C, K, (const bf16*)dz, (const bf16*)c, bmean, bvar, gamma, beta, eps, tot,
                                                    (const bf16*)g, w, (bf16*)dg, dw_scratch, S, 0, sg);
   EMO_LAUNCH_CHECK();
+  if (defer_reduce) return 0;
   return emo_dwconv_bwd_w_reduce((int)live_strips(seg->n, seg->B, seg->T, S), C, K, dw_scratch, dw, dbias, s);
 }
+
+extern "C" int emoasr_conv_module_bwd_seg(int dtype, const emoasr_segments_t* seg, int C, int K, const void* dz, const void* c,
+                                          const float* bmean, const float* bvar, const float* gamma, const float* beta, float eps,
+                                          float* dgamma, float* dbeta, const void* g, const float* w, void* dg, float* dw,
+                                          float* dbias, float* bn_scratch, float* dw_scratch, void* stream) {
+  return emo_conv_module_bwd_seg(dtype, seg, C, K, dz, c, bmean, bvar, gamma, beta, eps, dgamma, dbeta, g, w, dg, dw, dbias,
+                                 bn_scratch, dw_scratch, 0, stream);
+}
+
+extern "C" long emoasr_conv_module_bwd_seg_rows(const emoasr_segments_t* seg, int C) {
+  RowSegs sg;
+  int tmax = 0;
+  if (!row_segs(seg, C, &sg, &tmax)) return 0;
+  return live_strips(seg->n, seg->B, seg->T, strip_tiles(seg->n, seg->B, seg->T, cdiv(C, CF_CB)));
+}
diff --git a/emoasr_amd/csrc/convmodule.hip b/emoasr_amd/csrc/convmodule.hip
--- a/emoasr_amd/csrc/convmodule.hip
+++ b/emoasr_amd/csrc/convmodule.hip
@@ -228,6 +228,46 @@
   }
 }
 
+constexpr int DW_GROUP_MAX = 32;
+struct DwReduceGroup {
+  int rows[DW_GROUP_MAX];
+  const float* part[DW_GROUP_MAX];
+  float* dw[DW_GROUP_MAX];
+  float* dbias[DW_GROUP_MAX];
+};
+__global__ __launch_bounds__(256) void dwconv_bwd_w_reduce_grouped_kernel(const DwReduceGroup G, int C, int K) {
+  __shared__ float red[4][64];
+  const int p = blockIdx.z;
+  const int nblk = G.rows[p], slices = nblk >= 1024 ? 4 : 1;
+  if ((int)blockIdx.y >= slices) return;
+  const float* __restrict__ part = G.part[p];
+  float* __restrict__ dw = G.dw[p];
+  float* __restrict__ dbias = G.dbias[p];
+  const int lane = threadIdx.x & 63, wave = threadIdx.x >> 6;
+  const int i = blockIdx.x * 64 + lane;
+  const int n = (K + 1) * C;
+  const int per = (nblk + slices - 1) / slices;
+  const int b0 = blockIdx.y * per, b1 = min(nblk, b0 + per);
+  float s = 0.f;
+  if (i < n) {
+#pragma unroll 8
+    for (int b = b0 + wave; b < b1; b += 4) s += part[(long)b * n + i];
+  }
+  red[wave][lane] = s;
+  __syncthreads();
+  if (wave == 0 && i < n) {
+    s = red[0][lane] + red[1][lane] + red[2][lane] + red[3][lane];
+    const int j = i / C, c = i % C;
+    if (slices == 1) {
+      if (j < K) dw[c * K + j] += s;
+      else if (dbias) dbias[c] += s;
+    } else {
+      if (j < K) atomicAdd(&dw[c * K + j], s);
+      else if (dbias) atomicAdd(&dbias[c], s);
+    }
+  }
+}
+
 constexpr int BN_ROWS = 16;
 constexpr int BN_STAT_ROWS = 64;
 template <typename T>
@@ -477,6 +517,28 @@
   return 0;
 }
 
+extern "C" int emoasr_dwconv_bwd_w_reduce_grouped(int n, const int* rows, int C, int K, const float* const* part, float* const* dw,
+                                                  float* const* dbias, void* stream) {
+  EMO_CHECK(n >= 0 && C > 0 && K > 0 && (n == 0 || (rows && part && dw)), "dwconv_bwd_w_reduce_grouped: bad arguments");
+  for (int i0 = 0; i0 < n;) {
+    DwReduceGroup G{};
+    int m = 0, slices = 1;
+    for (; i0 + m < n && m < DW_GROUP_MAX; ++m) {
+      const int i = i0 + m;
+      EMO_CHECK(rows[i] >= 0 && part[i] && dw[i], "dwconv_bwd_w_reduce_grouped: problem %d has no table / output", i);
+      bool repeat = false;
+      for (int k = 0; k < m; ++k) repeat = repeat || G.dw[k] == dw[i];
+      if (repeat) break;
+      G.rows[m] = rows[i]; G.part[m] = part[i]; G.dw[m] = dw[i]; G.dbias[m] = dbias ? dbias[i] : nullptr;
+      if (rows[i] >= 1024) slices = 4;
+    }
+    dwconv_bwd_w_reduce_grouped_kernel<<<dim3(cdiv((K + 1) * C, 64), slices, m), 256, 0, (hipStream_t)stream>>>(G, C, K);
+    EMO_LAUNCH_CHECK();
+    i0 += m;
+  }
+  return 0;
+}
+
 extern "C" int emoasr_dwconv_fwd(int dtype, int B, int Tn, int C, int K, const void* x, const float* w,
                                  const float* bias, void* y, void* stream) {
   EMO_CHECK(K <= DW_MAXK && (K & 1), "dwconv: K=%d unsupported (odd, <= %d)", K, DW_MAXK);
diff --git a/emoasr_amd/csrc/gemm.hip b/emoasr_amd/csrc/gemm.hip
--- a/emoasr_amd/csrc/gemm.hip
+++ b/emoasr_amd/csrc/gemm.hip
@@ -712,9 +712,10 @@
 }
 
 template <typename T, int AMODE, bool BKM, bool TR, bool SP = false>
-int launch_nt_(const NtArgs& a_in, hipStream_t s, int nz = 1) {
+int launch_nt_(const NtArgs& a_in, hipStream_t s, int nz = 1, int gz = 0) {
   NtArgs a = a_in;
   a.xcd = g_opt.gemm_xcd;
+  if (gz <= 0) gz = nz;
   if constexpr (SP) {
     const long t12864 = (long)cdiv(a.M, 128) * cdiv(a.N, 64) * nz, t128 = (long)cdiv(a.M, 128) * cdiv(a.N, 128) * nz;
     (void)t12864;
@@ -741,7 +742,7 @@
   const int kb = sizeof(T) == 2 ? (g_opt.gemm_kb ? g_opt.gemm_kb : (a.K >= 512 ? 2 : 1)) : 1;
 #define EMO_NT_LAUNCH(BM_, BN_)                                                           \
   do {                                                                                    \
-    dim3 grid(cdiv(a.N, BN_), cdiv(a.M, BM_), nz);                                        \
+    dim3 grid(cdiv(a.N, BN_), cdiv(a.M, BM_), gz);                                        \
     if constexpr (sizeof(T) == 2) {                                                       \
       if (kb == 2) gemm_nt_kernel<T, BM_, BN_, AMODE, BKM, TR, 2><<<grid, 256, 0, s>>>(a); \
       else gemm_nt_kernel<T, BM_, BN_, AMODE, BKM, TR, 1><<<grid, 256, 0, s>>>(a);         \
@@ -751,7 +752,7 @@
   } while (0)
   if constexpr (sizeof(T) == 2 && AMODE == 0 && !BKM) {
     if (g_opt.gemm_wholek && a.M <= 2048 && a.K % 256 == 0 && nz == 1) {
-      dim3 grid(cdiv(a.N, 64), cdiv(a.M, 64), 1);
+      dim3 grid(cdiv(a.N, 64), cdiv(a.M, 64), gz);
       gemm_nt_kernel<T, 64, 64, AMODE, BKM, TR, 8><<<grid, 256, 0, s>>>(a);
       EMO_LAUNCH_CHECK();
       return 0;
@@ -858,6 +859,32 @@
   EMO_DISPATCH(dtype, return (launch_nt<T, 0>(a, (hipStream_t)stream)));
 }
 
+extern "C" int emoasr_conformer_pos_proj(int dtype, int nl, int R, int d, const void* pos_t, const void* const* wpos,
+                                         void* const* pp, void* stream) {
+  EMO_CHECK(nl >= 0 && R > 0 && d > 0 && pos_t && (nl == 0 || (wpos && pp)), "conformer_pos_proj: bad arguments");
+  for (int l = 0; l < nl; ++l) EMO_CHECK(wpos[l] && pp[l], "conformer_pos_proj: layer %d has no weight / output", l);
+  if (nl == 0) return 0;
+  emoasr_epilogue_t ep{};
+  ep.alpha = 1.f; ep.res_scale = 1.f;
+  const long sb = nl > 1 ? (const char*)wpos[1] - (const char*)wpos[0] : 0, sc = nl > 1 ? (char*)pp[1] - (char*)pp[0] : 0;
+  bool strided = dtype == EMO_BF16 && nl > 1 && sb % 16 == 0 && sc % 16 == 0 && d % 8 == 0 &&
+                 !emo_gemm_nt_big_wants(R, d, d, d, d, d, ep);
+  for (int l = 2; l < nl && strided; ++l)
+    strided = (const char*)wpos[l] - (const char*)wpos[0] == l * sb && (char*)pp[l] - (char*)pp[0] == l * sc;
+  if (strided && (sc < 0 ? -sc : sc) < (long)R * d * 2) strided = false;
+  if (!strided) {
+    for (int l = 0; l < nl; ++l)
+      if (emoasr_gemm_nt(dtype, R, d, d, pos_t, d, wpos[l], d, pp[l], d, &ep, stream)) return 1;
+    return 0;
+  }
+  NtArgs a{};
+  a.M = R; a.N = d; a.K = d; a.A = pos_t; a.lda = d; a.B = wpos[0]; a.ldb = d; a.C = pp[0]; a.ldc = d;
+  a.ep = ep;
+  a.nh = 1; a.sa_b = 0; a.sb_b = sb / 2; a.sc_b = sc / 2;
+  EmoTimerScope timer_(EMO_TIMER_GEMM_NT_NN, (hipStream_t)stream, 2.0 * nl * R * d * d, ((double)R * d + nl * ((double)d * d + (double)R * d)) * 2.0);
+  return launch_nt_<bf16, 0, false, true>(a, (hipStream_t)stream, 1, nl);
+}
+
 extern "C" int emoasr_gemm_nn(int dtype, int M, int N, int K, const void* A, long lda, const void* B,
                               long ldb, void* C, long ldc, const emoasr_epilogue_t* ep, void* stream) {
   SplitScope split_scope(dtype);
diff --git a/emoasr_amd/csrc/layer.hip b/emoasr_amd/csrc/layer.hip
--- a/emoasr_amd/csrc/layer.hip
+++ b/emoasr_amd/csrc/layer.hip
@@ -24,6 +24,10 @@
                    int flip, float* part, hipStream_t s);
 int emo_dwconv_bwd_w_seg(int dtype, const RowSegs& sg, int tmax, int C, int K, const void* dy, const void* x, float* dw, float* dbias,
                          float* scratch, hipStream_t s);
+int emo_conv_module_bwd_seg(int dtype, const emoasr_segments_t* seg, int C, int K, const void* dz, const void* c, const float* bmean,
+                            const float* bvar, const float* gamma, const float* beta, float eps, float* dgamma, float* dbeta,
+                            const void* g, const float* w, void* dg, float* dw, float* dbias, float* bn_scratch, float* dw_scratch,
+                            int defer_reduce, void* stream);
 
 namespace {
 
@@ -203,7 +207,7 @@
     e.bias = L->bqkv;
     if (emoasr_gemm_nt(dtype, M, 3 * d, d, io->at_h, d, L->wqkv, d, io->qkv, 3 * d, &e, stream)) return 1;
     emoasr_epilogue_t ep = plain_ep();
-    if (emoasr_gemm_nt(dtype, R, d, d, io->pos_t, d, L->wpos, d, io->pp, d, &ep, stream)) return 1;
+    if (!io->pp_ready && emoasr_gemm_nt(dtype, R, d, d, io->pos_t, d, L->wpos, d, io->pp, d, &ep, stream)) return 1;
     const int astep = g_opt.stack_launch ? sv.n : 1;
     for (int si = 0; si < sv.n; si += astep) {
       const size_t ro = (size_t)sv.row[si];
@@ -345,6 +349,11 @@
   SegView sv;
   if (seg->n < 1 || !seg_view(&io, d, &sv)) return 0;
   return bwd_layout(dtype, sv, d, H, 4 * d, 1).img[sv.n];
+}
+
+extern "C" long emoasr_conformer_layer_bwd_dw_rows(int dtype, const emoasr_segments_t* seg, int d) {
+  if (!seg || seg->n < 2 || !g_opt.stack_launch || !conv_fused_ok(dtype, d)) return 0;
+  return emoasr_conv_module_bwd_seg_rows(seg, d);
 }
 
 extern "C" size_t emoasr_conformer_layer_bwd_ws_bytes(int dtype, int B, int T, int d, int H, int F, int K) {
@@ -428,10 +437,11 @@
                  : emoasr_gemm_nn(dtype, M, d, d, dy, d, L->pw2, d, ws + bb.dz, d, &e, stream)) return 1;
     if (conv_fused_ok(dtype, d)) {
       const bool conv_one_launch = sv.n > 1 && g_opt.stack_launch;
+      const bool dw_defer = conv_one_launch && io->dw_defer && io->dw_part;
       if (conv_one_launch &&
-          emoasr_conv_module_bwd_seg(dtype, &st->seg, d, K, ws + bb.dz, st->c, st->bmean, st->bvar, L->bn_g, L->bn_b, 1e-5f,
-                                     (float*)G->bn_g, (float*)G->bn_b, st->g, L->dw_w, ws + bb.dg, (float*)G->dw_w, (float*)G->dw_b,
-                                     (float*)(ws + bb.bn_scr), (float*)(ws + bb.dw_scr), stream))
+          emo_conv_module_bwd_seg(dtype, &st->seg, d, K, ws + bb.dz, st->c, st->bmean, st->bvar, L->bn_g, L->bn_b, 1e-5f,
+                                  (float*)G->bn_g, (float*)G->bn_b, st->g, L->dw_w, ws + bb.dg, (float*)G->dw_w, (float*)G->dw_b,
+                                  (float*)(ws + bb.bn_scr), dw_defer ? io->dw_part : (float*)(ws + bb.dw_scr), dw_defer, stream))
         return 1;
       for (int si = 0; si < sv.n && !conv_one_launch; ++si) {
         const size_t ro = (size_t)sv.row[si];
diff --git a/emoasr_amd/engine/encoder.py b/emoasr_amd/engine/encoder.py
--- a/emoasr_amd/engine/encoder.py
+++ b/emoasr_amd/engine/encoder.py
@@ -49,6 +49,9 @@
         self._layer_lo = None
         self._cpp_layers = os.environ.get("EMOASR_CPP_LAYER", "1") != "0"
         self._layer_rt = None
+        self.pos_group = os.environ.get("EMOASR_POS_GROUP", "1") != "0"
+        self.dw_reduce_defer = os.environ.get("EMOASR_DW_REDUCE_DEFER", "1") != "0"
+        self._dw_deferred = []
         self.mask_padding = False
         self._conv_lens = None
         self._side_wgrads = os.environ.get("EMOASR_WGRAD_SIDE", "0") != "0"
@@ -365,6 +368,7 @@
             self._defer_wgrads = False
             self._wq = []
             self._ln_deferred = []
+            self._dw_deferred = []
 
     def _stack_dtype_ok(self, single=False):
         if self.dtype == torch.bfloat16:
@@ -429,10 +433,11 @@
         pos_t = ops.strided_copy(tab, out_dtype=dt)
         if p_enc > 0:
             pos_t = ops.scale_dropout(pos_t, 1.0, p_enc, self._seed(2))
+        pps = self._layer_rt.pos_proj(self.nl, pos_t) if self.pos_group and dt == torch.bfloat16 else None
         cur, layers = x, []
         for li in range(self.nl):
             cur = self._layer_rt.forward(li, cur, Btot, Tmax, elens, pos_t, p_enc, p_att, True, True, segs=tuple(segs),
-                                         att_mask=None if masks is None else masks[li])
+                                         att_mask=None if masks is None else masks[li], pp=None if pps is None else pps[li])
             layers.append(cur)
         x_final = cur.tv("y")
         eouts, fin_mean, fin_rstd = ops.layernorm_fwd(x_final, A.p("encoder.norm.weight"), A.p("encoder.norm.bias"), 1e-12, True)
@@ -453,17 +458,20 @@
         lnf = ops.lib.size_query("emoasr_layernorm_bwd_scratch_floats", d)
         ln_parts = torch.empty(self.nl, 5, lnf, device=dev, dtype=torch.float32)
         dx_bufs = [torch.empty(M, d, device=dev, dtype=dt) for _ in range(2)]
+        dw_deferred = self._dw_deferred if self.dw_reduce_defer and dt == torch.bfloat16 else None
         for li in reversed(range(self.nl)):
             out = dx_bufs[li & 1]
-            self._layer_rt.backward(li, st.layers[li], dx, out, ln_parts[li], self._ln_deferred)
+            self._layer_rt.backward(li, st.layers[li], dx, out, ln_parts[li], self._ln_deferred, dw_deferred)
             dx = out
             if self.grad_hook is not None:
                 self._flush_wgrads()
                 ops.layernorm_bwd_finalize(self._ln_deferred)
+                ops.dwconv_bwd_w_reduce_grouped(self._dw_deferred)
                 self._hook_after_layer(li)
         self._flush_wgrads()
         self._layer_rt.join_wgrads()
         ops.layernorm_bwd_finalize(self._ln_deferred)
+        ops.dwconv_bwd_w_reduce_grouped(self._dw_deferred)
         if self.grad_hook is not None and self._layer_rt.wgrad_side:
             self.grad_hook(self._layer_offset(0))
         dlin = ops.scale_dropout(dx, math.sqrt(d), self.p_enc, st.s_pe)
@@ -507,6 +515,7 @@
             self._defer_wgrads = False
             self._wq = []
             self._ln_deferred = []
+            self._dw_deferred = []
 
     def _ctc_train_stacked(self, batches, blank, scales, head):
         A = self.arena
diff --git a/emoasr_amd/layer_rt.py b/emoasr_amd/layer_rt.py
--- a/emoasr_amd/layer_rt.py
+++ b/emoasr_amd/layer_rt.py
@@ -55,11 +55,15 @@
 
 
 class LayerStash:
-    __slots__ = ("wt", "wf", "lay", "x_in", "seeds", "_tup", "io", "B", "T", "sweep")
+    __slots__ = ("wt", "wf", "lay", "x_in", "seeds", "_tup", "io", "B", "T", "sweep", "pp_ext")
 
     def __init__(self, wt, wf, lay, x_in, seeds):
         self.wt, self.wf, self.lay, self.x_in, self.seeds, self._tup = wt, wf, lay, x_in, seeds, None
         self.io = None
+        self.pp_ext = None
+
+    def pp(self):
+        return self.pp_ext if self.pp_ext is not None else self.tv("pp")
 
     def tv(self, name):
         o, n, shape = self.lay.t[name]
@@ -107,6 +111,15 @@
         self.calls = 0
         self.attn_img, self.attn_img_key = None, None
         self.sweeps = 0
+
+    def pos_proj(self, nl, pos_t):
+        eng = self.eng
+        R = pos_t.shape[0]
+        pp = torch.empty(nl, R, eng.d, device=pos_t.device, dtype=pos_t.dtype)
+        wpos = (ctypes.c_void_p * nl)(*[self._layer_params(li).wpos for li in range(nl)])
+        out = (ctypes.c_void_p * nl)(*[pp[li].data_ptr() for li in range(nl)])
+        lib.call("emoasr_conformer_pos_proj", ops.dt(pos_t), nl, R, eng.d, pos_t.data_ptr(), wpos, out, ops._stream())
+        return pp
 
     def _layer_params(self, li):
         eng, A = self.eng, self.eng.arena
@@ -183,7 +196,7 @@
             lay = self.layouts[key] = _Layout(B, T, self.eng.d, self.eng.h, F, segs)
         return lay
 
-    def forward(self, li, x, B, T, elens, pos_t, p_enc, p_att, training, keep, segs=None, att_mask=None):
+    def forward(self, li, x, B, T, elens, pos_t, p_enc, p_att, training, keep, segs=None, att_mask=None, pp=None):
         eng = self.eng
         L = self._layer_params(li)
         lay = self._layout(B, T, L.F, segs)
@@ -231,6 +244,9 @@
             io.at_mean, io.at_rstd = fb + f["at_mean"][0] * 4, fb + f["at_rstd"][0] * 4
             io.cv_mean, io.cv_rstd = fb + f["cv_mean"][0] * 4, fb + f["cv_rstd"][0] * 4
             io.fin_mean, io.fin_rstd = fb + f["fin_mean"][0] * 4, fb + f["fin_rstd"][0] * 4
+        if pp is not None:
+            assert pp.shape == (lay.R, eng.d) and pp.is_contiguous() and pp.dtype == wt.dtype
+            io.pp, io.pp_ready, st.pp_ext = pp.data_ptr(), 1, pp
         lib.call("emoasr_conformer_layer_fwd", ops.dt(wt), ctypes.byref(L), ctypes.byref(io), ops._stream())
         st.io, st.B, st.T = io, B, T
         return st
@@ -270,7 +286,7 @@
         self.grads[li] = (G, guard)
         return G
 
-    def backward(self, li, st, dy, dx, ln_part, deferred):
+    def backward(self, li, st, dy, dx, ln_part, deferred, dw_deferred=None):
         eng, A = self.eng, self.eng.arena
         L, G = self._layer_params(li), self._layer_grads(li)
         B, T = st.B, st.T
@@ -300,9 +316,15 @@
                 self.attn_img_key = key
             io.attn_img, io.attn_img_bytes = self.attn_img.data_ptr(), self.attn_img.numel()
         io.ln_part, io.ln_part_stride = ln_part.data_ptr(), ln_part.stride(0)
+        name = f"encoder.transformers.{li}"
+        if dw_deferred is not None and st.lay.segs is not None:
+            rows = lib.dw_rows_seg(ops.dt(st.wt), st.io.seg, eng.d)
+            if rows > 0:
+                table = torch.empty(rows * (L.K + 1) * eng.d, device=dy.device, dtype=torch.float32)
+                io.dw_part, io.dw_defer = table.data_ptr(), 1
+                dw_deferred.append((rows, table, A.g(name + ".conv.depthwise_conv.weight"), A.g(name + ".conv.depthwise_conv.bias")))
         lib.call("emoasr_conformer_layer_bwd", ops.dt(st.wt), ctypes.byref(L), ctypes.byref(G), ctypes.byref(st.io),
                  ctypes.byref(io), ops._stream())
-        name = f"encoder.transformers.{li}"
         M = st.lay.M
         for k, norm in enumerate(("norm_final", "norm_ff", "norm_conv", "norm_self_attn", "norm_ff_macaron")):
             deferred.append((M, eng.d, ln_part[k], A.g(f"{name}.{norm}.weight"), A.g(f"{name}.{norm}.bias")))
diff --git a/emoasr_amd/lib.py b/emoasr_amd/lib.py
--- a/emoasr_amd/lib.py
+++ b/emoasr_amd/lib.py
@@ -194,11 +194,12 @@
                 ("cv_y", c_void_p), ("bmean", c_void_p), ("bvar", c_void_p), ("bn_part", c_void_p),
                 ("cv_mean", c_void_p), ("cv_rstd", c_void_p),
                 ("y", c_void_p), ("fin_mean", c_void_p), ("fin_rstd", c_void_p), ("seg", Segments),
-                ("att_mask", c_void_p), ("att_mask_nw", c_int), ("att_mask_ready", c_int)]
+                ("att_mask", c_void_p), ("att_mask_nw", c_int), ("att_mask_ready", c_int), ("pp_ready", c_int)]
 
 class ConformerBwd(Structure):
     _fields_ = [("dy", c_void_p), ("dx", c_void_p), ("ws", c_void_p), ("ws_bytes", ctypes.c_size_t),
-                ("ln_part", c_void_p), ("ln_part_stride", c_long), ("attn_img", c_void_p), ("attn_img_bytes", ctypes.c_size_t)]
+                ("ln_part", c_void_p), ("ln_part_stride", c_long), ("attn_img", c_void_p), ("attn_img_bytes", ctypes.c_size_t),
+                ("dw_part", c_void_p), ("dw_defer", c_int)]
 
 
 class LasAttend(Structure):
@@ -257,6 +258,8 @@
     "emoasr_layernorm_bwd": [I, I, I, P, P, P, P, P, P, P, P, P, P, P],
     "emoasr_layernorm_bwd_ex": [I, I, I, P, P, P, P, P, P, P, P, P, P, POINTER(LnBwdOpts), P],
     "emoasr_layernorm_bwd_finalize": [I, POINTER(LnFinalizeItem), P],
+    "emoasr_conformer_pos_proj": [I, I, I, I, P, POINTER(c_void_p), POINTER(c_void_p), P],
+    "emoasr_dwconv_bwd_w_reduce_grouped": [I, POINTER(c_int), I, I, POINTER(c_void_p), POINTER(c_void_p), POINTER(c_void_p), P],
     "emoasr_conformer_layer_fwd": [I, POINTER(ConformerLayer), POINTER(ConformerFwd), P],
     "emoasr_conformer_attn_masks": [I, I, POINTER(Segments), I, I, I, I, P, F, P, P, L, I, P],
     "emoasr_conformer_layer_bwd": [I, POINTER(ConformerLayer), POINTER(ConformerLayer), POINTER(ConformerFwd),
@@ -490,6 +493,13 @@
     return n
 
 
+def dw_rows_seg(dtype_code, seg, d):
+    fn = load().emoasr_conformer_layer_bwd_dw_rows
+    fn.restype = ctypes.c_long
+    fn.argtypes = [c_int, POINTER(Segments), c_int]
+    return int(fn(dtype_code, ctypes.byref(seg), d))
+
+
 def img_bytes_seg(dtype_code, seg, d, H):
     fn = load().emoasr_conformer_layer_bwd_img_bytes_seg
     fn.restype = ctypes.c_size_t
diff --git a/emoasr_amd/ops.py b/emoasr_amd/ops.py
--- a/emoasr_amd/ops.py
+++ b/emoasr_amd/ops.py
@@ -270,6 +270,21 @@
     lib.call("emoasr_layernorm_fwd", dt(x), M, N, _p(x), _p(gamma), _p(beta), eps, _p(y), _p(mean), _p(rstd),
              _stream())
     return y, mean, rstd
+
+
+def dwconv_bwd_w_reduce_grouped(deferred):
+    n = len(deferred)
+    if n == 0:
+        return
+    C, K = deferred[0][2].shape[0], deferred[0][2].numel() // deferred[0][2].shape[0]
+    rows = (ctypes.c_int * n)(*[r for r, _, _, _ in deferred])
+    part = (ctypes.c_void_p * n)(*[t.data_ptr() for _, t, _, _ in deferred])
+    dw = (ctypes.c_void_p * n)(*[w.data_ptr() for _, _, w, _ in deferred])
+    db = (ctypes.c_void_p * n)(*[b.data_ptr() for _, _, _, b in deferred])
+    for r, t, w, b in deferred:
+        assert t.dtype == torch.float32 and t.numel() >= r * (K + 1) * C and w.numel() == C * K and b.numel() == C
+    lib.call("emoasr_dwconv_bwd_w_reduce_grouped", n, rows, C, K, part, dw, db, _stream())
+    del deferred[:]
 
 
 def layernorm_bwd(dy, x, gamma, mean, rstd, dres, dgamma, dbeta, branch=None, deferred=None):
diff --git a/include/emoasr_hip.h b/include/emoasr_hip.h
--- a/include/emoasr_hip.h
+++ b/include/emoasr_hip.h
@@ -464,7 +464,10 @@
   emoasr_segments_t seg;
   unsigned* att_mask; int att_mask_nw;
   int att_mask_ready;
+  int pp_ready;
 } emoasr_conformer_fwd_t;
+int emoasr_conformer_pos_proj(int dtype, int nl, int R, int d, const void* pos_t, const void* const* wpos, void* const* pp,
+                              void* stream);
 int emoasr_conformer_attn_masks(int dtype, int nl, const emoasr_segments_t* seg, int B, int T, int H, int d, const int* klens,
                                 float p_att, const uint64_t* seeds, unsigned* masks, long layer_stride_words, int nw, void* stream);
 int emoasr_conformer_layer_fwd(int dtype, const emoasr_conformer_layer_t* layer,
@@ -475,7 +478,12 @@
   void* ws; size_t ws_bytes;
   float* ln_part; long ln_part_stride;
   void* attn_img; size_t attn_img_bytes;
+  float* dw_part; int dw_defer;
 } emoasr_conformer_bwd_t;
+long emoasr_conv_module_bwd_seg_rows(const emoasr_segments_t* seg, int C);
+long emoasr_conformer_layer_bwd_dw_rows(int dtype, const emoasr_segments_t* seg, int d);
+int emoasr_dwconv_bwd_w_reduce_grouped(int n, const int* rows, int C, int K, const float* const* part, float* const* dw,
+                                       float* const* dbias, void* stream);
 size_t emoasr_conformer_layer_bwd_ws_bytes(int dtype, int B, int T, int d, int H, int F, int K);
 int emoasr_conv_module_fwd_seg(int dtype, const emoasr_segments_t* seg, int C, int K, const void* g, const float* w,
                                const float* bias, void* c, float* part, float* bmean, float* bvar, float* running_mean,
```

Result: slower. 5.898 million frames/s (-3.0%).
